# geopolars/geopolars

Measured on AMD Instinct MI355X. Metric: predicate evals/sec (10M pts x 1k polys point-in-polygon), higher is better.
Workload: dtype f64

## Files before the change

### geopolars_amd/_abi.py

```python
from __future__ import annotations

import ctypes as C
import os

HERE = os.path.dirname(os.path.abspath(__file__))
LIB_PATH = os.environ.get("GPK_LIB_PATH") or os.path.join(HERE, "libgeopolars_hip.so")

GPK_OK = 0
GPK_ERR_MISMATCHED_GEOMETRY = 1
GPK_ERR_INVALID_OFFSETS = 2
GPK_ERR_NULL_UNSUPPORTED = 3
GPK_ERR_DEVICE = 4
GPK_ERR_OOM = 5
GPK_ERR_INVALID_ARGUMENT = 6
GPK_ERR_CAPACITY = 7

GEOM_POINT = 0
GEOM_LINESTRING = 1
GEOM_POLYGON = 3
GEOM_MULTIPOINT = 4
GEOM_MULTILINESTRING = 5
GEOM_MULTIPOLYGON = 6
ARROW_WKB, ARROW_INTERLEAVED, ARROW_STRUCT = 0, 1, 2

MEM_HOST = 0
MEM_DEVICE = 1

PRED_INTERSECTS = 0
PRED_CONTAINS = 1
PRED_WITHIN = 2
INDEX_BBOX_GRID = 1
INDEX_PIP = 2
INDEX_PIP_LIGHT = 4
INDEX_PIP_FULL = 8
QUERY_CONTAINED, QUERY_INTERSECTING = 0, 1
PREDICATES = {"intersects": PRED_INTERSECTS, "contains": PRED_CONTAINS, "within": PRED_WITHIN}
LP_INTERIOR, LP_BOUNDARY, LP_EXTERIOR = 1, 2, 4
LP_PRED_INTERSECTS, LP_PRED_WITHIN, LP_PRED_COVERED_BY, LP_PRED_CROSSES, LP_PRED_TOUCHES = 0, 1, 2, 3, 4
TRI_OK, TRI_EMPTY, TRI_FAILED = 0, 1, 2
CLIP_INSIDE, CLIP_OUTSIDE, CLIP_DROP_EMPTY = 0, 1, 1
PCLIP_INTERSECTION, PCLIP_DIFFERENCE = 0, 1
PCLIP_OK, PCLIP_TOUCH, PCLIP_EMPTY, PCLIP_NULL, PCLIP_UNRESOLVED = 0, 1, 2, 3, 4
GEODESIC_AREA_SIGNED = 1
PUNION_UNION = 0
PP_INTERIORS, PP_BOUNDARIES, PP_A_OUTSIDE, PP_B_OUTSIDE = 1, 2, 4, 8
(PP_PRED_INTERSECTS, PP_PRED_WITHIN, PP_PRED_CONTAINS, PP_PRED_TOUCHES, PP_PRED_OVERLAPS, PP_PRED_EQUALS,
 PP_PRED_CONTAINS_PROPERLY) = range(7)
LL_INTERIORS, LL_SHARED_PIECE, LL_INT_BND, LL_BND_INT, LL_BND_BND, LL_A_OUTSIDE, LL_B_OUTSIDE = 1, 2, 4, 8, 16, 32, 64
(LL_PRED_INTERSECTS, LL_PRED_WITHIN, LL_PRED_CONTAINS, LL_PRED_COVERED_BY, LL_PRED_COVERS, LL_PRED_CROSSES, LL_PRED_TOUCHES, LL_PRED_OVERLAPS,
 LL_PRED_EQUALS) = range(9)
PT_INTERIOR, PT_BOUNDARY, PT_EXTERIOR, PT_B_OUTSIDE = 1, 2, 4, 8
GPK_KNN_MAX_K, GPK_KNN_EXCLUDE_SELF = 64, 1
(PT_PRED_INTERSECTS, PT_PRED_WITHIN, PT_PRED_CONTAINS, PT_PRED_COVERED_BY, PT_PRED_COVERS, PT_PRED_CROSSES, PT_PRED_TOUCHES, PT_PRED_OVERLAPS,
 PT_PRED_EQUALS) = range(9)


class GeopolarsHipError(RuntimeError):

    def __init__(self, code: int, message: str):
        super().__init__(f"[gpk status {code}] {message}")
        self.code = code


class MismatchedGeometry(GeopolarsHipError):
    """GeopolarsError::MismatchedGeometry (error.rs:12-16)."""


class GeoArrowDesc(C.Structure):
    _fields_ = [
        ("geom_type", C.c_int32),
        ("mem_space", C.c_int32),
        ("n_geoms", C.c_int64),
        ("n_coords", C.c_int64),
        ("xy", C.c_void_p),
        ("geom_offsets", C.c_void_p),
        ("part_offsets", C.c_void_p),
        ("ring_offsets", C.c_void_p),
        ("n_parts", C.c_int64),
        ("n_rings", C.c_int64),
        ("validity", C.c_void_p),
        ("x", C.c_void_p),
        ("y", C.c_void_p),
    ]


class ArrowSchema(C.Structure):
    """Arrow C Data Interface (what `pyarrow.Array._export_to_c` fills: py-geopolars/src/ffi.rs:12-32)"""


ArrowSchema._fields_ = [
    ("format", C.c_char_p),
    ("name", C.c_char_p),
    ("metadata", C.c_void_p),
    ("flags", C.c_int64),
    ("n_children", C.c_int64),
    ("children", C.POINTER(C.POINTER(ArrowSchema))),
    ("dictionary", C.POINTER(ArrowSchema)),
    ("release", C.CFUNCTYPE(None, C.POINTER(ArrowSchema))),
    ("private_data", C.c_void_p),
]


class ArrowArray(C.Structure):
    pass


ArrowArray._fields_ = [
    ("length", C.c_int64),
    ("null_count", C.c_int64),
    ("offset", C.c_int64),
    ("n_buffers", C.c_int64),
    ("n_children", C.c_int64),
    ("buffers", C.POINTER(C.c_void_p)),
    ("children", C.POINTER(C.POINTER(ArrowArray))),
    ("dictionary", C.POINTER(ArrowArray)),
    ("release", C.CFUNCTYPE(None, C.POINTER(ArrowArray))),
    ("private_data", C.c_void_p),
]


_VP = C.c_void_p
_PROTOS = {
    "gpk_version": (C.c_char_p, []),
    "gpk_last_error": (C.c_int32, [C.c_char_p, C.c_size_t]),
    "gpk_device_count": (C.c_int32, [C.POINTER(C.c_int32)]),
    "gpk_device_info": (C.c_int32, [C.c_char_p, C.c_size_t, C.POINTER(C.c_int32)]),
    "gpk_geoarray_upload": (C.c_int32, [C.POINTER(GeoArrowDesc), _VP, C.POINTER(_VP)]),
    "gpk_geoarray_from_arrow": (C.c_int32, [_VP, _VP, C.c_int32, _VP, C.POINTER(_VP), C.POINTER(C.c_int32)]),
    "gpk_geoarray_to_arrow": (C.c_int32, [_VP, C.c_int32, _VP, _VP, _VP]),
    "gpk_geoarray_free": (C.c_int32, [_VP]),
    "gpk_geoarray_invalidate": (C.c_int32, [_VP]),
    "gpk_geoarray_nbytes": (C.c_int32, [_VP, C.POINTER(C.c_int64)]),
    "gpk_wkb_decode": (C.c_int32, [_VP, _VP, C.c_int64, _VP, C.POINTER(C.c_int64), _VP, _VP, _VP, _VP]),
    "gpk_geoarray_from_wkb": (C.c_int32, [_VP, _VP, C.c_int64, _VP, C.c_int32, _VP, C.POINTER(_VP), C.POINTER(C.c_int32)]),
    "gpk_geoarray_download": (C.c_int32, [_VP, C.POINTER(C.c_int64), _VP, _VP, _VP, _VP, _VP]),
    "gpk_area": (C.c_int32, [_VP, _VP, C.c_int32, _VP]),
    "gpk_signed_area": (C.c_int32, [_VP, _VP, C.c_int32, _VP]),
    "gpk_centroid": (C.c_int32, [_VP, _VP, _VP, C.c_int32, _VP]),
    "gpk_representative_point": (C.c_int32, [_VP, _VP, _VP, _VP, C.c_int32, _VP]),
    "gpk_bounds": (C.c_int32, [_VP, _VP, C.c_int32, _VP]),
    "gpk_euclidean_length": (C.c_int32, [_VP, _VP, C.c_int32, _VP]),
    "gpk_affine_transform": (C.c_int32, [_VP, C.POINTER(C.c_double), _VP, C.c_int32, _VP]),
    "gpk_affine_transform_rows": (C.c_int32, [_VP, _VP, _VP, C.c_int32, _VP]),
    "gpk_affine_about_origin": (C.c_int32, [_VP, C.c_int32, C.c_double, C.c_double, C.c_int32, C.c_double, C.c_double, _VP, C.c_int32, _VP]),
    "gpk_crs_supported": (C.c_int32, [C.c_int32]),
    "gpk_reproject": (C.c_int32, [_VP, C.c_int32, C.c_int32, _VP, C.POINTER(C.c_int64), C.c_int32, _VP]),
    "gpk_envelope": (C.c_int32, [_VP, _VP, _VP, C.c_int32, _VP]),
    "gpk_exterior": (C.c_int32, [_VP, _VP, _VP, C.POINTER(C.c_int64), C.c_int32, _VP]),
    "gpk_explode": (C.c_int32, [_VP, _VP, C.c_int32, _VP, C.POINTER(_VP)]),
    "gpk_geoarray_validity": (C.c_int32, [_VP, _VP, C.POINTER(C.c_int32), _VP]),
    "gpk_geoarray_len": (C.c_int32, [_VP, C.POINTER(C.c_int64)]),
    "gpk_geom_type": (C.c_int32, [_VP, _VP, C.c_int32, _VP]),
    "gpk_is_empty": (C.c_int32, [_VP, _VP, C.c_int32, _VP]),
    "gpk_is_ring": (C.c_int32, [_VP, _VP, C.c_int32, _VP]),
    "gpk_point_xy": (C.c_int32, [_VP, _VP, _VP, C.c_int32, _VP]),
    "gpk_geodesic_length": (C.c_int32, [_VP, C.c_int32, _VP, C.c_int32, _VP]),
    "gpk_geodesic_area": (C.c_int32, [_VP, C.c_uint32, _VP, _VP, C.c_int32, _VP]),
    "gpk_geodesic_inverse": (C.c_int32, [_VP, _VP, _VP, _VP, _VP, _VP, C.c_int32, _VP]),
    "gpk_geodesic_direct": (C.c_int32, [_VP, _VP, C.c_int64, _VP, C.c_int64, _VP, _VP, C.c_int32, _VP]),
    "gpk_simplify": (C.c_int32, [_VP, C.c_double, _VP, _VP, C.POINTER(C.c_int64), C.c_int32, _VP]),
    "gpk_convex_hull": (C.c_int32, [_VP, _VP, _VP, C.c_int32, _VP]),
    "gpk_minimum_rotated_rectangle": (C.c_int32, [_VP, _VP, _VP, C.c_int32, _VP]),
    "gpk_minimum_bounding_circle": (C.c_int32, [_VP, _VP, _VP, _VP, C.c_int32, _VP]),
    "gpk_distance_rowwise": (C.c_int32, [_VP, _VP, _VP, _VP, C.c_int32, _VP]),
    "gpk_rowmap_build": (C.c_int32, [_VP, _VP, C.c_int64, C.c_int32, _VP, C.POINTER(_VP)]),
    "gpk_rowmap_free": (C.c_int32, [_VP]),
    "gpk_rowmap_nbytes": (C.c_int32, [_VP, C.POINTER(C.c_int64)]),
    "gpk_distance_rowmap": (C.c_int32, [_VP, _VP, _VP, _VP, C.c_int32, _VP]),
    "gpk_hausdorff_distance": (C.c_int32, [_VP, _VP, _VP, C.c_int32, _VP, C.c_int32, _VP]),
    "gpk_frechet_distance": (C.c_int32, [_VP, _VP, _VP, C.c_int32, _VP, C.POINTER(C.c_int64), C.c_int32, _VP]),
    "gpk_predicate_rowwise": (C.c_int32, [_VP, _VP, _VP, C.c_int32, _VP, C.c_int32, _VP]),
    "gpk_index_build": (C.c_int32, [_VP, _VP, C.POINTER(_VP)]),
    "gpk_index_build_ex": (C.c_int32, [_VP, C.c_int32, _VP, _VP, C.POINTER(_VP)]),
    "gpk_index_free": (C.c_int32, [_VP]),
    "gpk_index_nbytes": (C.c_int32, [_VP, C.POINTER(C.c_int64)]),
    "gpk_index_describe": (C.c_int32, [_VP, C.POINTER(C.c_int64)]),
    "gpk_index_query_envelope": (C.c_int32, [_VP, _VP, C.c_int64, C.c_int32, _VP, _VP, C.c_int64, C.POINTER(C.c_int64), C.c_int32, _VP]),
    "gpk_spatial_join": (
        C.c_int32,
        [_VP, _VP, _VP, C.c_int32, C.c_uint32, _VP, _VP, C.c_int64, C.POINTER(C.c_int64), C.c_int32, _VP],
    ),
    "gpk_spatial_join_async": (C.c_int32, [_VP, _VP, _VP, C.c_int32, C.c_uint32, _VP, _VP, C.c_int64, _VP, _VP]),
    "gpk_nearest_join": (
        C.c_int32,
        [_VP, _VP, _VP, C.c_double, C.c_uint32, _VP, _VP, _VP, C.c_int64, C.POINTER(C.c_int64), C.c_int32, _VP],
    ),
    "gpk_nearest_join_any": (
        C.c_int32,
        [_VP, _VP, _VP, C.c_double, C.c_uint32, _VP, _VP, _VP, C.c_int64, C.POINTER(C.c_int64), C.c_int32, _VP],
    ),
    "gpk_knn_join": (
        C.c_int32,
        [_VP, _VP, _VP, C.c_int32, C.c_double, C.c_uint32, C.c_uint32, _VP, _VP, _VP, C.c_int64, C.POINTER(C.c_int64), C.c_int32, _VP],
    ),
    "gpk_dwithin_join": (
        C.c_int32,
        [_VP, _VP, _VP, C.c_double, C.c_uint32, _VP, _VP, _VP, C.c_int64, C.POINTER(C.c_int64), C.c_int32, _VP],
    ),
    "gpk_dwithin_rowwise": (C.c_int32, [_VP, _VP, _VP, C.c_double, _VP, C.c_int32, _VP]),
    "gpk_line_polygon_relation": (C.c_int32, [_VP, _VP, _VP, _VP, C.c_int32, _VP]),
    "gpk_line_polygon_join": (
        C.c_int32,
        [_VP, _VP, _VP, C.c_int32, C.c_uint32, _VP, _VP, _VP, C.c_int64, C.POINTER(C.c_int64), C.c_int32, _VP],
    ),
    "gpk_polygon_relation": (C.c_int32, [_VP, _VP, _VP, _VP, C.c_int32, _VP]),
    "gpk_polygon_relation_join": (
        C.c_int32,
        [_VP, _VP, _VP, C.c_int32, C.c_uint32, _VP, _VP, _VP, C.c_int64, C.POINTER(C.c_int64), C.c_int32, _VP],
    ),
    "gpk_intersection_measure": (C.c_int32, [_VP, _VP, _VP, _VP, C.c_int32, _VP]),
    "gpk_line_clip": (C.c_int32, [_VP, _VP, _VP, _VP, C.c_int64, C.c_int32, C.c_int32, C.c_int32, _VP, C.c_int32, _VP, C.POINTER(_VP)]),
    "gpk_polygon_clip": (C.c_int32, [_VP, _VP, _VP, _VP, C.c_int64, C.c_int32, C.c_int32, C.c_int32, _VP, C.c_int32, _VP, C.c_int32, _VP, C.POINTER(_VP)]),
    "gpk_polygon_union": (C.c_int32, [_VP, _VP, _VP, _VP, C.c_int64, C.c_int32, C.c_int32, C.c_int32, _VP, C.c_int32, _VP, C.c_int32, _VP, C.POINTER(_VP)]),
    "gpk_union_all_pairs": (C.c_int32, [_VP, _VP, C.c_int64, C.c_int64, _VP, _VP, _VP, _VP, C.POINTER(C.c_int64), _VP]),
    "gpk_intersection_measure_join": (
        C.c_int32,
        [_VP, _VP, _VP, C.c_double, C.c_uint32, _VP, _VP, _VP, C.c_int64, C.POINTER(C.c_int64), C.c_int32, _VP],
    ),
    "gpk_line_relation": (C.c_int32, [_VP, _VP, _VP, _VP, C.c_int32, _VP]),
    "gpk_line_relation_join": (
        C.c_int32,
        [_VP, _VP, _VP, C.c_int32, C.c_uint32, _VP, _VP, _VP, C.c_int64, C.POINTER(C.c_int64), C.c_int32, _VP],
    ),
    "gpk_point_relation": (C.c_int32, [_VP, _VP, _VP, _VP, C.c_int32, _VP]),
    "gpk_point_relation_join": (
        C.c_int32,
        [_VP, _VP, _VP, C.c_int32, C.c_uint32, _VP, _VP, _VP, C.c_int64, C.POINTER(C.c_int64), C.c_int32, _VP],
    ),
    "gpk_validity": (C.c_int32, [_VP, _VP, _VP, C.c_int32, _VP]),
    "gpk_is_simple": (C.c_int32, [_VP, _VP, C.c_int32, _VP]),
    "gpk_triangulate": (C.c_int32, [_VP, _VP, C.c_int64, _VP, _VP, C.POINTER(C.c_int64), C.c_int32, _VP]),
    "gpk_closest_point_rowwise": (C.c_int32, [_VP, _VP, _VP, _VP, _VP, C.c_int32, _VP]),
    "gpk_line_locate_point": (C.c_int32, [_VP, _VP, _VP, C.c_int32, _VP, C.c_int32, _VP]),
    "gpk_line_interpolate_point": (C.c_int32, [_VP, _VP, C.c_int64, C.c_int32, _VP, _VP, C.c_int32, _VP]),
    "gpk_wkb_encode": (C.c_int32, [_VP, _VP, _VP, C.c_int64, C.POINTER(C.c_int64)]),
    "gpk_geoarray_to_wkb": (C.c_int32, [_VP, _VP, _VP, C.c_int64, C.POINTER(C.c_int64), C.c_int32, _VP]),
    "gpk_join_indices": (C.c_int32, [_VP, _VP, C.c_int64, C.c_int64, C.c_uint32, C.c_int32, _VP, _VP, C.c_int64, C.POINTER(C.c_int64), C.c_int32, _VP]),
    "gpk_take_fixed": (C.c_int32, [_VP, C.c_int32, _VP, C.c_int64, _VP, C.c_int64, _VP, _VP, C.c_int32, _VP]),
    "gpk_take_binary": (C.c_int32, [_VP, _VP, _VP, C.c_int64, _VP, C.c_int64, _VP, _VP, C.c_int64, C.POINTER(C.c_int64), _VP, C.c_int32, _VP]),
    "gpk_geoarray_take": (C.c_int32, [_VP, _VP, C.c_int64, C.c_int32, _VP, C.POINTER(_VP)]),
    "gpk_geoarray_filter": (C.c_int32, [_VP, _VP, C.c_int32, C.c_int32, _VP, C.POINTER(_VP), C.POINTER(C.c_int64)]),
    "gpk_segmentize": (C.c_int32, [_VP, C.c_double, _VP, C.c_int32, _VP, C.POINTER(_VP)]),
    "gpk_remove_repeated_points": (C.c_int32, [_VP, C.c_double, _VP, C.POINTER(_VP)]),
    "gpk_reverse": (C.c_int32, [_VP, _VP, C.POINTER(_VP)]),
    "gpk_orient_polygons": (C.c_int32, [_VP, C.c_int32, _VP, C.POINTER(_VP)]),
    "gpk_comm_unique_id":(C.c_int32, [C.POINTER(C.c_uint8)]),
    "gpk_comm_init": (C.c_int32, [C.c_int32, C.c_int32, C.POINTER(C.c_uint8), C.POINTER(_VP)]),
    "gpk_comm_free": (C.c_int32, [_VP]),
    "gpk_comm_mock_world": (C.c_int32, [C.c_int32, C.POINTER(_VP)]),
    "gpk_comm_init_mock": (C.c_int32, [C.c_int32, _VP, C.POINTER(_VP)]),
    "gpk_comm_mock_world_free": (C.c_int32, [_VP]),
    "gpk_comm_info": (C.c_int32, [_VP, C.POINTER(C.c_int32), C.POINTER(C.c_int32)]),
    "gpk_allgatherv_geoarray": (C.c_int32, [_VP, _VP, _VP, C.POINTER(_VP), C.POINTER(C.c_int64), C.POINTER(C.c_int64)]),
    "gpk_geoarray_concat": (C.c_int32, [C.POINTER(_VP), C.c_int32, _VP, C.POINTER(_VP), C.POINTER(C.c_int64), C.POINTER(C.c_int64)]),
    "gpk_allgatherv_rows_f64": (C.c_int32, [_VP, _VP, C.c_int64, C.c_int32, _VP, C.c_int64, C.POINTER(C.c_int64), C.POINTER(C.c_int64), _VP]),
    "gpk_device_cache_release": (C.c_int32, []),
    "gpk_join_stats_enable": (C.c_int32, [C.c_int32]),
    "gpk_join_stats": (C.c_int32, [C.POINTER(C.c_int64), C.c_int32]),
    "gpk_profile_enable": (C.c_int32, [C.c_int32]),
    "gpk_profile_filter": (C.c_int32, [C.c_char_p]),
    "gpk_profile_reset": (C.c_int32, []),
    "gpk_profile_query": (C.c_int32, [C.c_char_p, C.POINTER(C.c_double), C.POINTER(C.c_int64)]),
}
EXPORTED_SYMBOLS = tuple(_PROTOS)

_lib = None


def lib() -> C.CDLL:
    global _lib
    if _lib is not None:
        return _lib
    if not os.path.exists(LIB_PATH):
        raise GeopolarsHipError(
            GPK_ERR_DEVICE,
            f"{LIB_PATH} is missing: build it with `python -m geopolars_amd.build` "
            "(hipcc, gfx950).  geopolars_amd has no CPU fallback.",
        )
    try:
        import torch
    except Exception:
        pass
    handle = C.CDLL(LIB_PATH, mode=C.RTLD_GLOBAL)
    for name, (res, args) in _PROTOS.items():
        fn = getattr(handle, name)
        fn.restype = res
        fn.argtypes = args
    _lib = handle
    return _lib


def last_error() -> str:
    buf = C.create_string_buffer(512)
    lib().gpk_last_error(buf, 512)
    return buf.value.decode("utf-8", "replace")


def check(status: int) -> None:
    if status == GPK_OK:
        return
    msg = last_error()
    if status == GPK_ERR_MISMATCHED_GEOMETRY:
        raise MismatchedGeometry(status, msg)
    raise GeopolarsHipError(status, msg)


def device_count() -> int:
    n = C.c_int32(0)
    rc = lib().gpk_device_count(C.byref(n))
    return int(n.value) if rc == GPK_OK else 0


def device_info() -> tuple[str, int]:
    buf = C.create_string_buffer(256)
    cus = C.c_int32(0)
    check(lib().gpk_device_info(buf, 256, C.byref(cus)))
    return buf.value.decode(), int(cus.value)
```

### geopolars_amd/csrc/gpk_gridindex.hip

```cpp
#include <atomic>
#include <chrono>
#include <cmath>
#include <cstdlib>

#include "gpk_device.h"
#include "gpk_index.h"
#include "gpk_scan.h"

namespace gpk {

__global__ __launch_bounds__(256) void extent_partial_kernel(const double4* __restrict__ bbox, int64_t n, double4* __restrict__ part) {
    __shared__ double red[4][4];
    double mnx = INFINITY, mny = INFINITY, mxx = -INFINITY, mxy = -INFINITY;
    for (int64_t i = (int64_t)blockIdx.x * 256 + threadIdx.x; i < n; i += (int64_t)gridDim.x * 256) {
        const double4 b = bbox[i];
        if (b.x == b.x) {
            mnx = fmin(mnx, b.x);
            mny = fmin(mny, b.y);
            mxx = fmax(mxx, b.z);
            mxy = fmax(mxy, b.w);
        }
    }
    mnx = dev::wave_min(mnx);
    mny = dev::wave_min(mny);
    mxx = dev::wave_max(mxx);
    mxy = dev::wave_max(mxy);
    const int lane = threadIdx.x & 63, wave = threadIdx.x >> 6;
    if (lane == 0) {
        red[0][wave] = mnx;
        red[1][wave] = mny;
        red[2][wave] = mxx;
        red[3][wave] = mxy;
    }
    __syncthreads();
    if (threadIdx.x == 0) {
        for (int w = 1; w < 4; ++w) {
            mnx = fmin(mnx, red[0][w]);
            mny = fmin(mny, red[1][w]);
            mxx = fmax(mxx, red[2][w]);
            mxy = fmax(mxy, red[3][w]);
        }
        part[blockIdx.x] = mnx <= mxx ? make_double4(mnx, mny, mxx, mxy) : make_double4(NAN, NAN, NAN, NAN);
    }
}
__global__ __launch_bounds__(1024) void extent_kernel(const double4* __restrict__ bbox, int64_t n,
                                                      int gx, int gy, GridParams* __restrict__ out) {
    __shared__ double red[4][16];
    double mnx = INFINITY, mny = INFINITY, mxx = -INFINITY, mxy = -INFINITY;
    for (int64_t i = threadIdx.x; i < n; i += 1024) {
        const double4 b = bbox[i];
        if (b.x == b.x) {
            mnx = fmin(mnx, b.x);
            mny = fmin(mny, b.y);
            mxx = fmax(mxx, b.z);
            mxy = fmax(mxy, b.w);
        }
    }
    mnx = dev::wave_min(mnx);
    mny = dev::wave_min(mny);
    mxx = dev::wave_max(mxx);
    mxy = dev::wave_max(mxy);
    const int lane = threadIdx.x & 63, wave = threadIdx.x >> 6;
    if (lane == 0) {
        red[0][wave] = mnx;
        red[1][wave] = mny;
        red[2][wave] = mxx;
        red[3][wave] = mxy;
    }
    __syncthreads();
    if (threadIdx.x == 0) {
        for (int w = 1; w < 16; ++w) {
            mnx = fmin(mnx, red[0][w]);
            mny = fmin(mny, red[1][w]);
            mxx = fmax(mxx, red[2][w]);
            mxy = fmax(mxy, red[3][w]);
        }
        GridParams g;
        const bool any = mnx <= mxx;
        g.x0 = any ? mnx : 0.0;
        g.y0 = any ? mny : 0.0;
        const double w = any ? mxx - mnx : 0.0, h = any ? mxy - mny : 0.0;
        g.inv_w = w > 0.0 ? (double)gx / w : 0.0;
        g.inv_h = h > 0.0 ? (double)gy / h : 0.0;
        g.gx = gx;
        g.gy = gy;
        *out = g;
    }
}

template <bool FILL>
__global__ void grid_register_kernel(const double4* __restrict__ bbox, int64_t n,
                                     const GridParams* __restrict__ gp, int32_t* __restrict__ cell_cnt,
                                     int32_t* __restrict__ items) {
    const int64_t j = (int64_t)blockIdx.x * blockDim.x + threadIdx.x;
    if (j >= n) return;
    const double4 b = bbox[j];
    if (!(b.x == b.x)) return;
    const GridParams g = *gp;
    const int cx0 = dev::cell_of(b.x, g.x0, g.inv_w, g.gx), cx1 = dev::cell_of(b.z, g.x0, g.inv_w, g.gx);
    const int cy0 = dev::cell_of(b.y, g.y0, g.inv_h, g.gy), cy1 = dev::cell_of(b.w, g.y0, g.inv_h, g.gy);
    for (int cy = cy0; cy <= cy1; ++cy)
        for (int cx = cx0; cx <= cx1; ++cx) {
            const int c = cy * g.gx + cx;
            const int slot = atomicAdd(&cell_cnt[c], 1);
            if (FILL) items[slot] = (int32_t)j;
        }
}

__global__ void cell_sort_kernel(const int32_t* __restrict__ cell_off, int64_t n_cells, int32_t* __restrict__ items) {
    const int64_t c = (int64_t)blockIdx.x * blockDim.x + threadIdx.x;
    if (c >= n_cells) return;
    const int b = cell_off[c], e = cell_off[c + 1];
    for (int i = b + 1; i < e; ++i) {
        const int32_t key = items[i];
        int k = i - 1;
        while (k >= b && items[k] > key) {
            items[k + 1] = items[k];
            --k;
        }
        items[k + 1] = key;
    }
}

static inline dim3 grid_for(int64_t n, int block) {
    int64_t b = (n + block - 1) / block;
    return dim3((unsigned)(b > 0 ? b : 1));
}

}

using namespace gpk;

extern "C" {

int32_t gpk_index_free(gpk_index* idx) {
    if (!idx) return GPK_OK;
    (void)sync_device(idx->device);
    for (int i = 0; i < 24; ++i)
        if (idx->owned[i]) cached_free(idx->owned[i]);
    delete idx;
    return GPK_OK;
}

int32_t gpk_index_describe(const gpk_index* idx, int64_t out[8]) {
    if (!idx || !out) return fail(GPK_ERR_INVALID_ARGUMENT, "NULL argument");
    for (int i = 0; i < 8; ++i) out[i] = 0;
    out[0] = idx->pip.R;
    out[1] = idx->pip_lean;
    out[2] = idx->pip.chain_xy != nullptr;
    out[3] = idx->pip.route != nullptr;
    out[4] = idx->pip_list_heavy;
    out[5] = idx->route_own;
    out[6] = idx->route_single;
    return GPK_OK;
}

int32_t gpk_index_nbytes(const gpk_index* idx, int64_t* out_bytes) {
    if (!idx || !out_bytes) return fail(GPK_ERR_INVALID_ARGUMENT, "NULL argument");
    *out_bytes = idx->nbytes;
    return GPK_OK;
}

int32_t gpk_index_build(const gpk_geoarray* a, void* stream, gpk_index** out) {
    return gpk_index_build_ex(a, GPK_INDEX_BBOX_GRID | GPK_INDEX_PIP, nullptr, stream, out);
}

int32_t gpk_index_build_ex(const gpk_geoarray* a, int32_t parts, const double* bbox4_dev, void* stream, gpk_index** out) {
    if (!a || !out) return fail(GPK_ERR_INVALID_ARGUMENT, "NULL argument");
    *out = nullptr;
    GPK_TRY(require_device());
    hipStream_t s = (hipStream_t)stream;
    const int64_t n = a->d.n_geoms;

    gpk_index* ix = new gpk_index;
    memset(ix, 0, sizeof *ix);
    ix->device = a->device;
    ix->n_geoms = n;
    ix->geom_type = a->d.type;
    ix->n_coords = a->d.n_coords;
    ix->n_rings = a->d.n_rings;
    {
        static std::atomic<uint64_t> next_serial{1};
        ix->serial = next_serial.fetch_add(1);
    }

    int gdim = (int)ceil(2.0 * sqrt((double)(n > 0 ? n : 1)));
    if (gdim < 1) gdim = 1;
    if (gdim > 2048) gdim = 2048;
    const int64_t n_cells = (int64_t)gdim * gdim;

    auto cleanup = [&](int32_t rc) {
        gpk_index_free(ix);
        return rc;
    };
#define IX_HIP(expr)                                                                              \
    do {                                                                                          \
        hipError_t _e = (expr);                                                                   \
        if (_e != hipSuccess)                                                                     \
            return cleanup(fail(_e == hipErrorOutOfMemory ? GPK_ERR_OOM : GPK_ERR_DEVICE,         \
                                "%s failed: %s", #expr, hipGetErrorString(_e)));                  \
    } while (0)
#define IX_TRY(expr)                             \
    do {                                         \
        int32_t _rc = (expr);                    \
        if (_rc != GPK_OK) return cleanup(_rc);  \
    } while (0)

    const bool dbg_time = getenv("GPK_DEBUG_INDEX") != nullptr;
    auto t_last = std::chrono::steady_clock::now();
    auto stamp = [&](const char* what) {
        if (!dbg_time) return;
        (void)hipStreamSynchronize(s);
        const auto now = std::chrono::steady_clock::now();
        fprintf(stderr, "[gpk] index build: %-28s %8.3f ms\n", what, std::chrono::duration<double, std::milli>(now - t_last).count());
        t_last = now;
    };
    double4* bbox = nullptr;
    GridParams* grid = nullptr;
    int32_t* cell_off = nullptr;
    IX_HIP(cached_malloc((void**)&bbox, sizeof(double4) * (size_t)(n > 0 ? n : 1)));
    ix->owned[0] = bbox;
    IX_HIP(cached_malloc((void**)&grid, sizeof(GridParams)));
    ix->owned[1] = grid;
    IX_HIP(cached_malloc((void**)&cell_off, sizeof(int32_t) * (size_t)(n_cells + 1)));
    ix->owned[2] = cell_off;

    if (bbox4_dev)
        IX_HIP(hipMemcpyAsync(bbox, bbox4_dev, sizeof(double4) * (size_t)n, hipMemcpyDeviceToDevice, s));
    else
        IX_TRY(gpk_bounds(a, (double*)bbox, GPK_MEM_DEVICE, stream));

    stamp("boxes (gpk_bounds)");
    const int64_t n_blocks = (n_cells + 255) / 256;
    const int64_t ext_blocks = n > 65536 ? 1024 : 0;
    Scratch sc(workspace());
    int32_t *cell_cnt, *cursor;
    unsigned long long* btot;
    double4* ext_part;
    sc.add_n((size_t)(n_cells + 1), cell_cnt, cursor);
    sc.add(btot, (size_t)(n_blocks + 1));
    sc.add(ext_part, 1024);
    IX_TRY(sc.commit());
    if (ext_blocks) {
        GPK_LAUNCH_OR(cleanup, "gpk_index_extent_partial", extent_partial_kernel, dim3((unsigned)ext_blocks), dim3(256), 0, s, bbox, n, ext_part);
        GPK_LAUNCH_OR(cleanup, "gpk_index_extent", extent_kernel, dim3(1), dim3(1024), 0, s, (const double4*)ext_part, ext_blocks, gdim, gdim, grid);
    } else {
        GPK_LAUNCH_OR(cleanup, "gpk_index_extent", extent_kernel, dim3(1), dim3(1024), 0, s, bbox, n, gdim, gdim, grid);
    }

    stamp("extent");
    IX_HIP(hipMemsetAsync(cell_cnt, 0, sizeof(int32_t) * (size_t)(n_cells + 1), s));
    if (n > 0)
        GPK_LAUNCH_OR(cleanup, "gpk_index_count", grid_register_kernel<false>, grid_for(n, 256), dim3(256), 0, s, bbox, n, grid, cell_cnt, (int32_t*)nullptr);
    IX_TRY(exclusive_scan_i32(cell_cnt, n_cells, cell_off, cursor, btot, s));
    unsigned long long total = 0;
    IX_HIP(d2h_small(&total, btot + n_blocks, sizeof total, s));
    IX_HIP(d2h_small(&ix->host_grid, grid, sizeof(GridParams), s));
    IX_HIP(sync_small(s));
    if (total > (unsigned long long)INT32_MAX)
        return cleanup(fail(GPK_ERR_INVALID_OFFSETS, "spatial index directory overflows i32 (%llu entries)", total));
    int32_t* items = nullptr;
    IX_HIP(cached_malloc((void**)&items, sizeof(int32_t) * (size_t)(total > 0 ? total : 1)));
    ix->owned[3] = items;
    if (n > 0) {
        GPK_LAUNCH_OR(cleanup, "gpk_index_fill", grid_register_kernel<true>, grid_for(n, 256), dim3(256), 0, s, bbox, n, grid, cursor, items);
        GPK_LAUNCH_OR(cleanup, "gpk_index_sort", cell_sort_kernel, grid_for(n_cells, 256), dim3(256), 0, s, cell_off, n_cells, items);
    }
    IX_HIP(hipStreamSynchronize(s));
    stamp("directory");
#undef IX_HIP
#undef IX_TRY

    ix->v.bbox = bbox;
    ix->v.grid = grid;
    ix->v.cell_off = cell_off;
    ix->v.items = items;
    ix->v.gx = gdim;
    ix->v.gy = gdim;
    ix->nbytes = (int64_t)(sizeof(double4) * (size_t)n + sizeof(GridParams) + sizeof(int32_t) * (size_t)(n_cells + 1) +
                           sizeof(int32_t) * (size_t)total);
    if (parts & GPK_INDEX_PIP) {
        const int32_t rc = build_pip_index(a, ix, s, (parts & GPK_INDEX_PIP_LIGHT) ? 0 : ((parts & GPK_INDEX_PIP_FULL) ? 2 : 1));
        if (rc != GPK_OK) {
            gpk_index_free(ix);
            return rc;
        }
    }
    *out = ix;
    return GPK_OK;
}

}
```

### geopolars_amd/csrc/gpk_index.h

```cpp
#pragma once

#include "gpk_common.h"
#include "gpk_route.h"

namespace gpk {

struct GridParams {
    double x0, y0, inv_w, inv_h;
    int32_t gx, gy;
};

struct IndexView {
    const double4* bbox;
    const GridParams* grid;
    const int32_t* cell_off;
    const int32_t* items;
    int32_t gx, gy;
};

struct PartInfo {
    int32_t slab_base, row0 , nrows, n_rings;
};
constexpr int PIP_SUB = 8;
constexpr int PIP_SLAB_MUL = 2;
constexpr int PIP_FINE_LOG2 = 6;
__host__ __device__ inline int slab_row0_of(int32_t packed) { return packed & 0xFFFFFF; }
__host__ __device__ inline int slab_shift_of(int32_t packed) { return packed >> 24; }
constexpr uint32_t SUB_INDIRECT = 1u << 30;
struct SubCell {
    uint32_t part_flags;
    uint32_t e0, e1, e2;
    uint32_t labels[4];
};
struct SubCell2 {
    SubCell a;
    uint32_t b_part_flags;
    uint32_t b_e0, b_e1, b_e2;
    uint32_t pad[4];
};
constexpr uint32_t SUB2_BIT = 1u << 29;
constexpr int CHAIN_MAX = 12;
constexpr uint32_t HCHAIN_COUNT_MASK = 0xFu;
constexpr int HCHAIN_BASE_SHIFT = 4;
constexpr int HCHAIN_START_SHIFT = 8;
struct HalfCell {
    uint32_t lw[2];
    uint32_t part_flags;
    uint32_t aux_base;
};
static_assert(sizeof(HalfCell) * 2 == sizeof(SubCell), "two half-cell records overlay one SubCell");
static_assert(CHAIN_MAX <= (int)HCHAIN_COUNT_MASK, "the edge count of a chain is a 4-bit field");
struct PipView {
    int32_t R;
    double rx0, ry0, fw, fh, inv_fw, inv_fh;
    const uint32_t* cell;
    const uint32_t* list;
    const SubCell* sub;
    const SubCell2* sub2;
    const double2* chain_xy;
    const RouteWord* route;
    const SubCell* lrec;
    const uint32_t* part_geom;
    const PartInfo* part_info;
    const float4* part_box;
    const int32_t* ring_row0;
    const int32_t* ring_slab_base;
    const int32_t* slab_off;
    const double4* slab_edges;
    const int32_t* slab_vidx;
    const double2* slab_xy;
};
constexpr uint32_t CELL_TAG_EMPTY = 0u, CELL_TAG_SINGLE = 1u, CELL_TAG_LIST = 2u, CELL_TAG_SUB = 3u;

namespace dev {
__device__ __forceinline__ int cell_of(double v, double v0, double inv, int g) {
    return (int)fmin(fmax((v - v0) * inv, 0.0), (double)(g - 1));
}
}

}

struct gpk_index {
    gpk::IndexView v;
    gpk::PipView pip;
    gpk::GridParams host_grid;
    int device;
    int64_t n_geoms, n_coords, n_rings;
    int32_t geom_type;
    void* owned[24];
    int64_t nbytes;
    int32_t pip_lean;
    uint64_t serial;
    int32_t pip_list_heavy;
    int32_t route_own, route_single;
};

namespace gpk {
int32_t build_pip_index(const gpk_geoarray* a, gpk_index* ix, hipStream_t s, int list_records_mode = 1);
int32_t ring_bboxes(const gpk_geoarray* a, double4* out_dev, hipStream_t s);
int32_t affine_rows_impl(const gpk_geoarray* a, const double* matrices, int32_t mat_space, double* out_xy, int32_t out_space, hipStream_t s);
}
```

### geopolars_amd/csrc/gpk_pipindex.hip

```cpp
#include <cstdio>
#include <cstdlib>
#include <cstring>

#include <rocprim/rocprim.hpp>

#include <chrono>

#include "gpk_device.h"
#include "gpk_index.h"
#include "gpk_pip.h"
#include "gpk_scan.h"

namespace gpk {

struct FineGrid {
    int R;
    double rx0, ry0, fw, fh, inv_fw, inv_fh, pad_x, pad_y;
};
__device__ __forceinline__ int fcol(const FineGrid& f, double x) { return dev::cell_of(x, f.rx0, f.inv_fw, f.R); }
__device__ __forceinline__ int frow(const FineGrid& f, double y) { return dev::cell_of(y, f.ry0, f.inv_fh, f.R); }

__global__ void part_geom_kernel(DevGeo a, uint32_t* __restrict__ part_geom) {
    const int64_t g = (int64_t)blockIdx.x * blockDim.x + threadIdx.x;
    if (g >= a.n_geoms) return;
    for (int p = a.geom_off[g]; p < a.geom_off[g + 1]; ++p) part_geom[p] = (uint32_t)g;
}
__global__ void ring_part_kernel(DevGeo a, int64_t n_parts, int32_t* __restrict__ ring_part) {
    const int64_t p = (int64_t)blockIdx.x * blockDim.x + threadIdx.x;
    if (p >= n_parts) return;
    int r0, r1;
    dev::part_rings(a, (int)p, r0, r1);
    for (int r = r0; r < r1; ++r) ring_part[r] = (int32_t)p;
}

__global__ void part_info_kernel(DevGeo a, int64_t n_parts, const int32_t* __restrict__ row0, const int32_t* __restrict__ slab_base,
                                 PartInfo* __restrict__ info) {
    const int64_t p = (int64_t)blockIdx.x * blockDim.x + threadIdx.x;
    if (p >= n_parts) return;
    int r0, r1;
    dev::part_rings(a, (int)p, r0, r1);
    PartInfo pi{0, 0, 0, r1 - r0};
    if (r1 > r0) {
        pi.slab_base = slab_base[r0];
        pi.row0 = row0[r0];
        pi.nrows = slab_base[r0 + 1] - slab_base[r0];
    }
    info[p] = pi;
}

__global__ void part_box_kernel(DevGeo a, int64_t n_parts, const double4* __restrict__ ring_bbox, float4* __restrict__ box) {
    const int64_t p = (int64_t)blockIdx.x * blockDim.x + threadIdx.x;
    if (p >= n_parts) return;
    int r0, r1;
    dev::part_rings(a, (int)p, r0, r1);
    const float nan = __builtin_nanf("");
    float4 b = make_float4(nan, nan, nan, nan);
    if (r1 > r0) {
        const double4 d = ring_bbox[r0];
        auto down = [](double v) {
            float f = (float)v;
            return (double)f > v ? nextafterf(f, -INFINITY) : f;
        };
        auto up = [](double v) {
            float f = (float)v;
            return (double)f < v ? nextafterf(f, INFINITY) : f;
        };
        b = make_float4(down(d.x), down(d.y), up(d.z), up(d.w));
    }
    box[p] = b;
}

constexpr int SLAB_TARGET = 12;
__global__ void ring_rows_kernel(const double4* __restrict__ ring_bbox, int64_t n_rings, const int32_t* __restrict__ ring_off, FineGrid f,
                                 int max_shift, int32_t* __restrict__ row0, int32_t* __restrict__ nrows, int32_t* __restrict__ n_refined) {
    const int64_t r = (int64_t)blockIdx.x * blockDim.x + threadIdx.x;
    if (r >= n_rings) return;
    const double4 b = ring_bbox[r];
    if (!(b.x == b.x) || !(b.y == b.y) || !(b.w == b.w)) {
        row0[r] = 0;
        nrows[r] = 0;
        return;
    }
    const int f0 = frow(f, b.y), f1 = frow(f, b.w);
    const int64_t n_edges = (int64_t)ring_off[r + 1] - ring_off[r] - 1;
    const int64_t base_rows = (f1 >> PIP_FINE_LOG2) - (f0 >> PIP_FINE_LOG2) + 1;
    int sh = 0;
    while (sh < max_shift && n_edges > (int64_t)SLAB_TARGET * (base_rows << sh)) ++sh;
    const int j0 = f0 >> (PIP_FINE_LOG2 - sh), j1 = f1 >> (PIP_FINE_LOG2 - sh);
    if (sh > 0 && (int)(threadIdx.x & 63) == __ffsll((long long)__ballot(sh > 0)) - 1) *n_refined = 1;
    row0[r] = j0 | (sh << 24);
    nrows[r] = j1 - j0 + 1;
}

__device__ __forceinline__ bool edge_at(const DevGeo& a, const int32_t* __restrict__ coord_ring, int i, int& r, double2& s, double2& e) {
    r = coord_ring[i];
    const int c0 = a.ring_off[r], c1 = a.ring_off[r + 1];
    if (i >= c1) return false;
    s = a.xy[i];
    if (i + 1 < c1) {
        e = a.xy[i + 1];
        return true;
    }
    if (c1 - c0 == 1) {
        e = s;
        return true;
    }
    return false;
}

__global__ void ring_start_kernel(const int32_t* __restrict__ ring_off, int64_t n_rings, int64_t n_coords, int32_t* __restrict__ flag) {
    const int64_t r = (int64_t)blockIdx.x * blockDim.x + threadIdx.x;
    if (r < 1 || r >= n_rings) return;
    const int32_t o = ring_off[r];
    if (o >= 0 && (int64_t)o < n_coords) atomicAdd(&flag[o], 1);
}

template <bool FILL>
__global__ void slab_register_kernel(DevGeo a, const int32_t* __restrict__ coord_ring, FineGrid f, const int32_t* __restrict__ row0,
                                     const int32_t* __restrict__ slab_base, int32_t* __restrict__ cnt_or_cursor,
                                     double4* __restrict__ edges, int32_t* __restrict__ vidx = nullptr) {
    const int64_t i = (int64_t)blockIdx.x * blockDim.x + threadIdx.x;
    const int lane = (int)(threadIdx.x & 63);
    int r = 0;
    double2 s = make_double2(0, 0), e = s;
    bool live = i < a.n_coords && edge_at(a, coord_ring, (int)i, r, s, e);
    if (live) live = slab_base[r + 1] != slab_base[r];
    const double ylo = s.y < e.y ? s.y : e.y, yhi = s.y > e.y ? s.y : e.y;
    if (!(ylo == ylo) || !(yhi == yhi)) live = false;
    int j0 = 0, j1 = -1, sl0 = -1 - lane;
    int rr = 0;
    if (live) {
        rr = row0[r];
        const int down = PIP_FINE_LOG2 - slab_shift_of(rr);
        j0 = frow(f, ylo) >> down;
        j1 = frow(f, yhi) >> down;
        sl0 = slab_base[r] + (j0 - slab_row0_of(rr));
    }
    const int prev = __shfl_up(sl0, 1, 64);
    const unsigned long long heads = __ballot(lane == 0 || sl0 != prev);
    const int head = 63 - __clzll((long long)(heads & (~0ull >> (63 - lane))));
    const unsigned long long above = lane == 63 ? 0ull : heads >> (lane + 1);
    const int run = above ? __ffsll((long long)above) : 64 - lane;
    int base = 0;
    if (live && head == lane) base = atomicAdd(&cnt_or_cursor[sl0], run);
    base = __shfl(base, head, 64);
    if (!live) return;
    const bool degenerate = FILL && a.ring_off[r + 1] - a.ring_off[r] == 1;
    auto put = [&](int slot) {
        if (edges) edges[slot] = make_double4(s.x, s.y, e.x, e.y);
        if (vidx) vidx[slot] = degenerate ? ~(int32_t)i : (int32_t)i;
    };
    if (FILL) put(base + (lane - head));
    for (int j = j0 + 1; j <= j1; ++j) {
        const int sl = slab_base[r] + (j - slab_row0_of(rr));
        const int slot = atomicAdd(&cnt_or_cursor[sl], 1);
        if (FILL) put(slot);
    }
}

__device__ __forceinline__ bool line_clear_of_rect(double sx, double sy, double ex, double ey, double xl, double yl, double xh, double yh) {
    const bool x_up = sy > ey, y_up = ex > sx;
    const double max_x = x_up ? xh : xl, min_x = x_up ? xl : xh, max_y = y_up ? yh : yl, min_y = y_up ? yl : yh;
    return dev::orient2d(sx, sy, ex, ey, min_x, min_y) > 0 || dev::orient2d(sx, sy, ex, ey, max_x, max_y) < 0;
}
template <typename F>
__device__ __forceinline__ void for_each_touched_cell(const FineGrid& g, double2 s, double2 e, F&& f) {
    const double xlo = s.x < e.x ? s.x : e.x, xhi = s.x > e.x ? s.x : e.x;
    const double ylo = s.y < e.y ? s.y : e.y, yhi = s.y > e.y ? s.y : e.y;
    if (!(xlo == xlo) || !(xhi == xhi) || !(ylo == ylo) || !(yhi == yhi)) return;
    const int i0 = fcol(g, xlo - g.pad_x), i1 = fcol(g, xhi + g.pad_x);
    const int j0 = frow(g, ylo - g.pad_y), j1 = frow(g, yhi + g.pad_y);
    if (i0 == i1 && j0 == j1) {
        f(i0, j0);
        return;
    }
    for (int j = j0; j <= j1; ++j)
        for (int i = i0; i <= i1; ++i) {
            if (i == 0 || j == 0 || i == g.R - 1 || j == g.R - 1) {
                f(i, j);
                continue;
            }
            const double xl = g.rx0 + (double)i * g.fw - g.pad_x, xh = g.rx0 + (double)(i + 1) * g.fw + g.pad_x;
            const double yl = g.ry0 + (double)j * g.fh - g.pad_y, yh = g.ry0 + (double)(j + 1) * g.fh + g.pad_y;
            if (!line_clear_of_rect(s.x, s.y, e.x, e.y, xl, yl, xh, yh)) f(i, j);
        }
}

template <bool FILL>
__global__ void mark_kernel(DevGeo a, const int32_t* __restrict__ coord_ring, FineGrid g, const int32_t* __restrict__ ring_part,
                            int32_t* __restrict__ cnt_or_off, unsigned long long* __restrict__ keys) {
    const int64_t i = (int64_t)blockIdx.x * blockDim.x + threadIdx.x;
    const int lane = (int)(threadIdx.x & 63);
    int r = 0;
    double2 s = make_double2(0, 0), e = s;
    const bool live = i < a.n_coords && edge_at(a, coord_ring, (int)i, r, s, e);
    const unsigned long long none = ~0ull;
    unsigned long long first = none;
    const int64_t o0 = FILL && i < a.n_coords ? (int64_t)cnt_or_off[i] : 0;
    int64_t n = 0;
    if (live) {
        const unsigned long long part = (unsigned long long)ring_part[r];
        for_each_touched_cell(g, s, e, [&](int ci, int cj) {
            const unsigned long long key = ((unsigned long long)(cj * g.R + ci) << 32) | part;
            if (n == 0) {
                first = key;
            } else if (FILL) {
                if (n == 1) keys[o0] = first;
                keys[o0 + n] = key;
            }
            ++n;
        });
    }
    const unsigned long long single = n == 1 ? first : none;
    const unsigned long long prev = __shfl_up(single, 1, 64);
    const bool repeat = lane > 0 && single != none && single == prev;
    if (i >= a.n_coords) return;
    if (!FILL) {
        cnt_or_off[i] = repeat ? 0 : (int32_t)(n < 0x7FFFFFFF ? n : 0x7FFFFFFF);
    } else if (n == 1 && !repeat) {
        keys[o0] = first;
    }
}

__global__ void unique_flags_kernel(const unsigned long long* __restrict__ sorted, int64_t n, int32_t* __restrict__ flag) {
    const int64_t i = (int64_t)blockIdx.x * blockDim.x + threadIdx.x;
    if (i >= n) return;
    flag[i] = (i == 0 || sorted[i] != sorted[i - 1]) ? 1 : 0;
}
__global__ void unique_compact_kernel(const unsigned long long* __restrict__ sorted, int64_t n, const int32_t* __restrict__ pos,
                                      unsigned long long* __restrict__ out, int32_t* __restrict__ cell_marks) {
    const int64_t i = (int64_t)blockIdx.x * blockDim.x + threadIdx.x;
    if (i >= n) return;
    const unsigned long long key = sorted[i];
    if (i == 0 || key != sorted[i - 1]) {
        out[pos[i]] = key;
        atomicAdd(&cell_marks[key >> 32], 1);
    }
}

constexpr int CELL_SCRATCH = 8;
template <bool FILL>
__global__ void cell_build_kernel(DevGeo a, IndexView ix, PipView pv, FineGrid g,
                                  const unsigned long long* __restrict__ marks, const int32_t* __restrict__ mark_start,
                                  int32_t* __restrict__ need, const int32_t* __restrict__ list_off,
                                  uint32_t* __restrict__ cell, uint32_t* __restrict__ list, uint32_t* __restrict__ scratch,
                                  const double4* __restrict__ ring_bbox) {
    const int64_t c = (int64_t)blockIdx.x * blockDim.x + threadIdx.x;
    const int64_t n_cells = (int64_t)g.R * g.R;
    if (c >= n_cells) return;
    if (FILL && need[c] == 0) return;
    if (FILL && scratch && need[c] - 1 <= CELL_SCRATCH) {
        const int m = need[c] - 1;
        uint32_t* out = list + list_off[c];
        out[0] = (uint32_t)m;
        for (int k = 0; k < m; ++k) out[1 + k] = scratch[(int64_t)k * n_cells + c];
        cell[c] = (CELL_TAG_LIST << 30) | (uint32_t)list_off[c];
        return;
    }
    const int ci = (int)(c % g.R), cj = (int)(c / g.R);
    const double cx = g.rx0 + ((double)ci + 0.5) * g.fw, cy = g.ry0 + ((double)cj + 0.5) * g.fh;
    const bool border = ci == 0 || cj == 0 || ci == g.R - 1 || cj == g.R - 1;
    const bool centre_ok = !border && fcol(g, cx) == ci && frow(g, cy) == cj;
    int64_t m = mark_start[c];
    const int64_t m_end = mark_start[c + 1];

    int n = 0;
    uint32_t first_entry = 0;
    uint32_t* out = nullptr;
    if (FILL && need[c] > 0) {
        out = list + list_off[c];
        out[0] = (uint32_t)(need[c] - 1);
        ++out;
    }
    auto emit = [&](uint32_t part, uint32_t boundary) {
        const uint32_t e = (part << 1) | boundary;
        if (n == 0) first_entry = e;
        if (out) out[n] = e;
        if (!FILL && scratch && n < CELL_SCRATCH) scratch[(int64_t)n * n_cells + c] = e;
        ++n;
    };
    auto flush_marks_below = [&](unsigned long long part_limit) {
        while (m < m_end && (marks[m] & 0xFFFFFFFFull) < part_limit) {
            emit((uint32_t)(marks[m] & 0xFFFFFFFFull), 1u);
            ++m;
        }
    };

    const GridParams cg = *ix.grid;
    const int gx = dev::cell_of(cx, cg.x0, cg.inv_w, cg.gx), gy = dev::cell_of(cy, cg.y0, cg.inv_h, cg.gy);
    const int gc = gy * cg.gx + gx;
    for (int k = ix.cell_off[gc]; k < ix.cell_off[gc + 1]; ++k) {
        const int j = ix.items[k];
        const double4 bb = ix.bbox[j];
        if (!(cx >= bb.x && cx <= bb.z && cy >= bb.y && cy <= bb.w)) continue;
        if (!dev::valid_row(a.validity, j)) continue;
        int p0, p1;
        dev::geom_parts(a, j, p0, p1);
        for (int p = p0; p < p1; ++p) {
            flush_marks_below((unsigned long long)p);
            if (m < m_end && (marks[m] & 0xFFFFFFFFull) == (unsigned long long)p) {
                emit((uint32_t)p, 1u);
                ++m;
                continue;
            }
            if (p1 - p0 > 1) {
                int r0, r1;
                dev::part_rings(a, p, r0, r1);
                if (r1 <= r0) continue;
                const double4 rb = ring_bbox[r0];
                if (!(cx >= rb.x && cx <= rb.z && cy >= rb.y && cy <= rb.w)) continue;
            }
            const int pos = pip::part_pos_single(pv, a, p, cx, cy);
            if (pos == dev::POS_OUTSIDE) continue;
            emit((uint32_t)p, (centre_ok && pos == dev::POS_INSIDE) ? 0u : 1u);
        }
    }
    flush_marks_below(~0ull);

    if (!FILL) {
        need[c] = n >= 2 ? n + 1 : 0;
        if (n <= 1) cell[c] = n == 1 ? ((CELL_TAG_SINGLE << 30) | first_entry) : 0u;
        return;
    }
    cell[c] = (CELL_TAG_LIST << 30) | (uint32_t)list_off[c];
}

__device__ __forceinline__ int64_t sub_slot(int64_t c, int route_logR) { return route_logR ? (int64_t)route_order((uint32_t)c, route_logR) : c; }
__global__ void sub_flag_kernel(const uint32_t* __restrict__ cell, const uint32_t* __restrict__ list, int64_t n_cells, int route_logR,
                                int32_t* __restrict__ flag, int32_t* __restrict__ flag2) {
    const int64_t c = (int64_t)blockIdx.x * blockDim.x + threadIdx.x;
    if (c >= n_cells) return;
    const uint32_t w = cell[c];
    const uint32_t tag = w >> 30;
    flag[sub_slot(c, route_logR)] = (tag == CELL_TAG_SINGLE && (w & 1u)) ? 1 : 0;
    int f2 = 0;
    if (tag == CELL_TAG_LIST) {
        const uint32_t off = w & 0x3FFFFFFFu;
        if (list[off] == 2u) f2 = (list[off + 1] & list[off + 2] & 1u) ? 1 : 0;
    }
    flag2[c] = f2;
}

__device__ __forceinline__ void record_slabs(const PipView& pv, int p, int cj, uint32_t& flags, uint32_t& e0, uint32_t& e1, uint32_t& e2) {
    const PartInfo pi = pv.part_info[p];
    e0 = e1 = e2 = 0;
    flags = (uint32_t)p | (pi.n_rings > 1 ? 0x80000000u : 0u);
    if (slab_shift_of(pi.row0) != 0) {
        flags |= SUB_INDIRECT;
        return;
    }
    const int j0 = PIP_SLAB_MUL * cj - slab_row0_of(pi.row0), j1 = j0 + 1;
    const bool lo_ok = j0 >= 0 && j0 < pi.nrows, hi_ok = j1 >= 0 && j1 < pi.nrows;
    if (lo_ok) {
        e0 = (uint32_t)pv.slab_off[pi.slab_base + j0];
        e1 = (uint32_t)pv.slab_off[pi.slab_base + j0 + 1];
        e2 = e1;
    }
    if (hi_ok) {
        if (!lo_ok) e0 = e1 = (uint32_t)pv.slab_off[pi.slab_base + j1];
        e2 = (uint32_t)pv.slab_off[pi.slab_base + j1 + 1];
    }
}
__global__ void sub_head_kernel(PipView pv, FineGrid g, const int32_t* __restrict__ work_cell, const uint32_t* __restrict__ work_part,
                                int64_t n_work, SubCell* __restrict__ sub) {
    const int64_t i = (int64_t)blockIdx.x * blockDim.x + threadIdx.x;
    if (i >= n_work) return;
    uint32_t flags, e0, e1, e2;
    record_slabs(pv, (int)work_part[i], (int)(work_cell[i] / g.R), flags, e0, e1, e2);
    *reinterpret_cast<uint4*>(&sub[i].part_flags) = make_uint4(flags, e0, e1, e2);
}

constexpr int SUB_EDGE_CAP = 48;
template <int NP, bool WORK = false, int MODE = 0>
__global__ __launch_bounds__(256) __attribute__((amdgpu_waves_per_eu(MODE == 1 ? 8 : 5))) void sub_build_kernel(DevGeo a, PipView pv, FineGrid g, const int32_t* __restrict__ flag,
                                                        const int32_t* __restrict__ pos, int64_t n_cells, const uint32_t* __restrict__ cell,
                                                        const uint32_t* __restrict__ list, SubCell* __restrict__ sub,
                                                        SubCell2* __restrict__ sub2, const int32_t* __restrict__ work_cell = nullptr,
                                                        const uint32_t* __restrict__ work_part = nullptr, int64_t n_work = 0) {
    static_assert(!WORK || NP == 1, "work items carry one part");
    constexpr int S = PIP_SUB, SS = PIP_SUB * PIP_SUB;
    const int64_t t = (int64_t)blockIdx.x * blockDim.x + threadIdx.x;
    const int64_t item = t / SS;
    const int k = (int)(t % SS);
    if (WORK ? item >= n_work : (item >= n_cells || !flag[item])) return;
    const int64_t c = WORK ? (int64_t)work_cell[item] : item;
    const uint32_t w = cell[c];
    int part[2] = {0, 0};
    bool crosses[2] = {true, true};
    if (WORK) {
        part[0] = (int)work_part[item];
    } else if (NP == 1) {
        part[0] = (int)((w & 0x3FFFFFFFu) >> 1);
    } else {
        const uint32_t off = w & 0x3FFFFFFFu;
        const uint32_t ea = list[off + 1], eb = list[off + 2];
        part[0] = (int)(ea >> 1);
        part[1] = (int)(eb >> 1);
    }
    const int ci = (int)(c % g.R), cj = (int)(c / g.R);
    const int si = S * ci + (k % S), sj = S * cj + (k / S);
    const double fw2 = g.fw / S, fh2 = g.fh / S, px2 = g.pad_x / S, py2 = g.pad_y / S;
    const double xl = g.rx0 + (double)si * fw2 - px2, xh = g.rx0 + (double)(si + 1) * fw2 + px2;
    const double yl = g.ry0 + (double)sj * fh2 - py2, yh = g.ry0 + (double)(sj + 1) * fh2 + py2;
    __shared__ double4 s_edges[256 / 64][SUB_EDGE_CAP];
    __shared__ double4 s_edges_all[WORK ? 256 / 64 : 1][WORK ? 64 : 1];
    const int wave = threadIdx.x >> 6, lane64 = threadIdx.x & 63;
    const double cxl = g.rx0 + (double)(S * ci) * fw2 - px2, cxh = g.rx0 + (double)(S * ci + S) * fw2 + px2;
    const double cyl = g.ry0 + (double)(S * cj) * fh2 - py2, cyh = g.ry0 + (double)(S * cj + S) * fh2 + py2;
    auto edge_touches = [&](const double4 ed) {
        if (fmax(ed.x, ed.z) < xl || fmin(ed.x, ed.z) > xh || fmax(ed.y, ed.w) < yl || fmin(ed.y, ed.w) > yh) return false;
        return !line_clear_of_rect(ed.x, ed.y, ed.z, ed.w, xl, yl, xh, yh);
    };
    auto store_labels = [&](SubCell* rec, uint32_t label) {
        const unsigned long long lo = __ballot((label & 1u) != 0), hi = __ballot((label & 2u) != 0);
        if (k < 4) {
            auto spread16 = [](uint32_t x) {
                x = (x | (x << 8)) & 0x00FF00FFu;
                x = (x | (x << 4)) & 0x0F0F0F0Fu;
                x = (x | (x << 2)) & 0x33333333u;
                x = (x | (x << 1)) & 0x55555555u;
                return x;
            };
            rec->labels[k] = spread16((uint32_t)(lo >> (16 * k)) & 0xFFFFu) | (spread16((uint32_t)(hi >> (16 * k)) & 0xFFFFu) << 1);
        }
    };
    if (WORK) {
        const uint4 head = *reinterpret_cast<const uint4*>(&sub[item].part_flags);
        const uint32_t n_all = head.w - head.y;
        const bool fast = !(head.x & (SUB_INDIRECT | 0x80000000u)) && n_all <= 64u;
        if (MODE == 1 && !fast) return;
        if (MODE == 2 && fast) return;
        if (MODE != 2 && fast) {
            if ((uint32_t)lane64 < n_all) s_edges_all[wave][lane64] = pip::slab_edge(pv, (int)(head.y + (uint32_t)lane64));
            __builtin_amdgcn_fence(__ATOMIC_RELEASE, "wavefront");
            __builtin_amdgcn_wave_barrier();
            __builtin_amdgcn_fence(__ATOMIC_ACQUIRE, "wavefront");
            bool touched = false;
            for (uint32_t e = 0; e < n_all && !touched; ++e) touched = edge_touches(s_edges_all[wave][e]);
            uint32_t label = 2u;
            if (!touched) {
                const double cx = g.rx0 + ((double)si + 0.5) * fw2, cy = g.ry0 + ((double)sj + 0.5) * fh2;
                const bool ok = dev::cell_of(cx, g.rx0, g.inv_fw * S, g.R * S) == si && dev::cell_of(cy, g.ry0, g.inv_fh * S, g.R * S) == sj;
                if (ok) {
                    const uint32_t mid = head.z - head.y;
                    const uint32_t a0 = (k / S) >= S / 2 ? mid : 0u, a1 = (k / S) >= S / 2 ? n_all : mid;
                    int wn = 0;
                    bool on = false;
                    for (uint32_t e = a0; e < a1; ++e) {
                        const double4 ed = s_edges_all[wave][e];
                        on |= dev::ring_edge(ed.x, ed.y, ed.z, ed.w, cx, cy, wn);
                    }
                    label = on ? 2u : (wn != 0 ? 1u : 0u);
                }
            }
            store_labels(sub + item, label);
            return;
        }
        if (MODE == 1) return;
    }
    __shared__ int s_span_e0[256 / 64][64], s_span_at[256 / 64][64];
    int n_list = 0;
    bool touched = false;
    auto wave_min = [&](double v) {
#pragma unroll
        for (int o = 1; o < 64; o <<= 1) v = fmin(v, __shfl_xor(v, o, 64));
        return v;
    };
    auto drain = [&](bool boxed = false) {
        __builtin_amdgcn_fence(__ATOMIC_RELEASE, "wavefront");
        __builtin_amdgcn_wave_barrier();
        __builtin_amdgcn_fence(__ATOMIC_ACQUIRE, "wavefront");
        bool skip = false;
        if (boxed) {
            const double inf = __builtin_inf();
            double4 b = make_double4(inf, inf, inf, inf);
            bool odd = false;
            if (lane64 < n_list) {
                const double4 ed = s_edges[wave][lane64];
                b = make_double4(fmin(ed.x, ed.z), fmin(ed.y, ed.w), -fmax(ed.x, ed.z), -fmax(ed.y, ed.w));
                odd = !(ed.x == ed.x) || !(ed.y == ed.y) || !(ed.z == ed.z) || !(ed.w == ed.w);
            }
            if (!__ballot(odd)) {
                const double bx0 = wave_min(b.x), by0 = wave_min(b.y), bx1 = -wave_min(b.z), by1 = -wave_min(b.w);
                skip = bx1 < xl || bx0 > xh || by1 < yl || by0 > yh;
            }
        }
        for (int e = 0; e < n_list && !touched && !skip; ++e) touched = edge_touches(s_edges[wave][e]);
        __builtin_amdgcn_fence(__ATOMIC_RELEASE, "wavefront");
        __builtin_amdgcn_wave_barrier();
        __builtin_amdgcn_fence(__ATOMIC_ACQUIRE, "wavefront");
        n_list = 0;
    };
    for (int q = 0; q < NP; ++q) {
        if (!crosses[q]) continue;
        int r0, r1;
        dev::part_rings(a, part[q], r0, r1);
        for (int rb = r0; rb < r1; rb += 64) {
            const int n_r = r1 - rb < 64 ? r1 - rb : 64;
            int e0 = 0, cnt = 0;
            if (lane64 < n_r) {
                int a0, a1;
                if (pip::slab_span_of_raster_row(pv, rb + lane64, cj, a0, a1)) {
                    e0 = a0;
                    cnt = a1 - a0;
                }
            }
            const int incl = dev::wave_inclusive_scan(cnt);
            const int total = __shfl(incl, 63, 64);
            s_span_e0[wave][lane64] = e0;
            s_span_at[wave][lane64] = incl - cnt;
            __builtin_amdgcn_fence(__ATOMIC_RELEASE, "wavefront");
            __builtin_amdgcn_wave_barrier();
            __builtin_amdgcn_fence(__ATOMIC_ACQUIRE, "wavefront");
            for (int base = 0; base < total; base += 64) {
                const int t = base + lane64;
                bool keep = false;
                double4 ed = make_double4(0, 0, 0, 0);
                if (t < total) {
                    int lo = 0, hi = n_r;
                    while (hi - lo > 1) {
                        const int mid = (lo + hi) >> 1;
                        if (s_span_at[wave][mid] <= t)
                            lo = mid;
                        else
                            hi = mid;
                    }
                    ed = pip::slab_edge(pv, s_span_e0[wave][lo] + (t - s_span_at[wave][lo]));
                    keep = !(fmax(ed.x, ed.z) < cxl || fmin(ed.x, ed.z) > cxh || fmax(ed.y, ed.w) < cyl || fmin(ed.y, ed.w) > cyh);
                }
                unsigned long long pending = __ballot(keep);
                while (pending) {
                    const int rank = __popcll(pending & ((1ull << lane64) - 1ull));
                    const bool put = keep && rank < SUB_EDGE_CAP - n_list;
                    if (put) {
                        s_edges[wave][n_list + rank] = ed;
                        keep = false;
                    }
                    const unsigned long long taken = __ballot(put);
                    n_list += __popcll(taken);
                    pending &= ~taken;
                    if (pending) drain(true);
                }
            }
            __builtin_amdgcn_fence(__ATOMIC_RELEASE, "wavefront");
            __builtin_amdgcn_wave_barrier();
            __builtin_amdgcn_fence(__ATOMIC_ACQUIRE, "wavefront");
        }
    }
    drain();
    const uint32_t test_label = NP == 2 ? 3u : 2u;
    uint32_t label = test_label;
    if (!touched) {
        const double cx = g.rx0 + ((double)si + 0.5) * fw2, cy = g.ry0 + ((double)sj + 0.5) * fh2;
        const bool ok = dev::cell_of(cx, g.rx0, g.inv_fw * S, g.R * S) == si && dev::cell_of(cy, g.ry0, g.inv_fh * S, g.R * S) == sj;
        if (ok) {
            if (NP == 1) {
                const int p = pip::part_pos_single(pv, a, part[0], cx, cy);
                label = p == dev::POS_INSIDE ? 1u : (p == dev::POS_OUTSIDE ? 0u : 2u);
            } else {
                const int pa = pip::part_pos_single(pv, a, part[0], cx, cy), pb = pip::part_pos_single(pv, a, part[1], cx, cy);
                if (pa == dev::POS_BOUNDARY || pb == dev::POS_BOUNDARY)
                    label = 3u;
                else if (pa == dev::POS_INSIDE && pb == dev::POS_INSIDE)
                    label = 3u;
                else
                    label = pa == dev::POS_INSIDE ? 1u : (pb == dev::POS_INSIDE ? 2u : 0u);
            }
        }
    }
    auto slabs_of = [&](int p, uint32_t& flags, uint32_t& e0, uint32_t& e1, uint32_t& e2) { record_slabs(pv, p, cj, flags, e0, e1, e2); };
    SubCell* rec = WORK ? sub + item : (NP == 1 ? sub + pos[c] : &sub2[pos[c]].a);
    if (k == 0) {
        slabs_of(part[0], rec->part_flags, rec->e0, rec->e1, rec->e2);
        if (NP == 2) {
            SubCell2* r2 = sub2 + pos[c];
            slabs_of(part[1], r2->b_part_flags, r2->b_e0, r2->b_e1, r2->b_e2);
        }
    }
    store_labels(rec, label);
}
__global__ void sub_commit_kernel(const int32_t* __restrict__ flag, const int32_t* __restrict__ pos, const int32_t* __restrict__ flag2,
                                  const int32_t* __restrict__ pos2, int64_t n_cells, int route_logR, uint32_t* __restrict__ cell) {
    const int64_t c = (int64_t)blockIdx.x * blockDim.x + threadIdx.x;
    if (c >= n_cells) return;
    const int64_t o = sub_slot(c, route_logR);
    if (flag[o])
        cell[c] = (CELL_TAG_SUB << 30) | (uint32_t)pos[o];
    else if (flag2 && flag2[c])
        cell[c] = (CELL_TAG_SUB << 30) | SUB2_BIT | (uint32_t)pos2[c];
}

__global__ void lrec_count_kernel(const uint32_t* __restrict__ cell, const uint32_t* __restrict__ list, int64_t n_cells,
                                  int32_t* __restrict__ cnt) {
    const int64_t c = (int64_t)blockIdx.x * blockDim.x + threadIdx.x;
    if (c >= n_cells) return;
    const uint32_t w = cell[c];
    int n = 0;
    if ((w >> 30) == CELL_TAG_LIST) {
        const uint32_t off = w & 0x3FFFFFFFu, m = list[off];
        for (uint32_t t = 0; t < m; ++t) n += (int)(list[off + 1 + t] & 1u);
    }
    cnt[c] = n;
}
__device__ __forceinline__ int test_labels_of(uint32_t w) { return __popc((w >> 1) & ~w & 0x55555555u); }
__global__ void chain_xy_kernel(DevGeo a, double2* __restrict__ ext) {
    const int64_t k = (int64_t)blockIdx.x * blockDim.x + threadIdx.x;
    const int64_t n_ext = a.n_coords + a.n_rings * CHAIN_MAX;
    if (k >= n_ext) return;
    int lo = 0, hi = (int)a.n_rings - 1;
    while (lo < hi) {
        const int mid = (lo + hi + 1) >> 1;
        if ((int64_t)a.ring_off[mid] + (int64_t)mid * CHAIN_MAX <= k)
            lo = mid;
        else
            hi = mid - 1;
    }
    const int c0 = a.ring_off[lo], n = a.ring_off[lo + 1] - c0;
    const int j = (int)(k - ((int64_t)c0 + (int64_t)lo * CHAIN_MAX));
    const int ne = n - 1;
    ext[k] = n <= 0 ? make_double2(0.0, 0.0) : (ne >= 1 ? a.xy[c0 + j % ne] : a.xy[c0]);
}
__global__ __launch_bounds__(256) void half_chain_kernel(DevGeo a, PipView pv, FineGrid g, const int32_t* __restrict__ work_cell,
                                                         const uint32_t* __restrict__ work_part, int64_t n_work,
                                                         const int32_t* __restrict__ slab_vidx, const SubCell* __restrict__ sub,
                                                         uint32_t* __restrict__ hword) {
    constexpr int S = PIP_SUB;
    static_assert(S == 8 && PIP_SLAB_MUL == 2, "a record is two halves of four sub-cell rows, one base slab row each");
    const int64_t t = (int64_t)blockIdx.x * blockDim.x + threadIdx.x;
    const int64_t item = t >> 1;
    const int half = (int)(t & 1);
    if (item >= n_work) return;
    const int64_t c = work_cell[item];
    const int part = (int)work_part[item];
    const uint32_t lw0 = sub[item].labels[2 * half], lw1 = sub[item].labels[2 * half + 1];
    uint32_t word = 0u;
    int r0, r1;
    dev::part_rings(a, part, r0, r1);
    if (test_labels_of(lw0) + test_labels_of(lw1) > 0 && r1 - r0 == 1) {
        const int ci = (int)(c % g.R), cj = (int)(c / g.R);
        const double fw2 = g.fw / S, fh2 = g.fh / S, px2 = g.pad_x / S, py2 = g.pad_y / S;
        const int sj0 = S * cj + (S / 2) * half;
        const double xl = g.rx0 + (double)(S * ci) * fw2 - px2, xh = g.rx0 + (double)(S * ci + S) * fw2 + px2;
        const double yl = g.ry0 + (double)sj0 * fh2 - py2, yh = g.ry0 + (double)(sj0 + S / 2) * fh2 + py2;
        const int c0 = a.ring_off[r0], ne = a.ring_off[r0 + 1] - c0 - 1;
        bool closed = false;
        if (ne >= 1) {
            const double2 f = a.xy[c0], l = a.xy[c0 + ne];
            closed = f.x == l.x && f.y == l.y;
        }
        const double cy = g.ry0 + ((double)sj0 + 0.25 * S) * fh2;
        const int row_c = pip::row_of(pv, cy);
        const int step = 1 << PIP_FINE_LOG2;
        int e0 = 0, e1 = 0;
        bool have = false;
        int lo = 0, len = 0;
        bool ok = closed;
        int n_touched = 0;
        int touched[CHAIN_MAX + 1];
        for (int dr = -1; dr <= 1 && ok; ++dr) {
            if (!pip::slab_range(pv, r0, row_c + dr * step, e0, e1)) continue;
            have = true;
            for (int e = e0; e < e1 && ok; ++e) {
                const double4 ed = pip::slab_edge(pv, e);
                if (fmax(ed.x, ed.z) < xl || fmin(ed.x, ed.z) > xh || fmax(ed.y, ed.w) < yl || fmin(ed.y, ed.w) > yh) continue;
                if (line_clear_of_rect(ed.x, ed.y, ed.z, ed.w, xl, yl, xh, yh)) continue;
                const int ei = pip::slab_vertex(slab_vidx[e]) - c0;
                bool seen = false;
                for (int q = 0; q < n_touched; ++q) seen = seen || touched[q] == ei;
                if (seen) continue;
                if (n_touched >= CHAIN_MAX) {
                    ok = false;
                    break;
                }
                touched[n_touched++] = ei;
            }
        }
        ok = ok && have && n_touched > 0;
        if (ok) {
            int best_gap = -1, best_next = 0;
            for (int p = 0; p < n_touched; ++p) {
                const int ea = touched[p];
                int nd = ne, nb = ea;
                for (int q = 0; q < n_touched; ++q) {
                    int dd = touched[q] - ea;
                    if (dd < 0) dd += ne;
                    if (dd > 0 && dd < nd) {
                        nd = dd;
                        nb = touched[q];
                    }
                }
                if (nd > best_gap) {
                    best_gap = nd;
                    best_next = nb;
                }
            }
            lo = best_next;
            len = ne - best_gap + 1;
            ok = len >= 1 && len <= CHAIN_MAX;
        }
        while (ok && len < ne) {
            int hv = lo + len;
            if (hv >= ne) hv -= ne;
            const double y = a.xy[c0 + hv].y;
            if (!(y >= yl && y <= yh)) break;
            ++len;
            ok = len <= CHAIN_MAX;
        }
        while (ok && len < ne) {
            const double y = a.xy[c0 + lo].y;
            if (!(y >= yl && y <= yh)) break;
            lo = lo == 0 ? ne - 1 : lo - 1;
            ++len;
            ok = len <= CHAIN_MAX;
        }
        if (ok) {
            const double cx = g.rx0 + ((double)(S * ci) + 0.5 * S) * fw2;
            int wn = 0;
            bool on = false;
            if (pip::slab_range(pv, r0, row_c, e0, e1)) {
                for (int e = e0; e < e1; ++e) {
                    int dd = pip::slab_vertex(slab_vidx[e]) - c0 - lo;
                    if (dd < 0) dd += ne;
                    if (dd < len) continue;
                    const double4 ed = pip::slab_edge(pv, e);
                    on |= dev::ring_edge(ed.x, ed.y, ed.z, ed.w, cx, cy, wn);
                }
            }
            const int64_t start = (int64_t)c0 + (int64_t)r0 * CHAIN_MAX + lo;
            if (!on && wn >= -8 && wn <= 7 && start < ((int64_t)1 << (32 - HCHAIN_START_SHIFT)))
                word = (uint32_t)len | ((uint32_t)(wn & 15) << HCHAIN_BASE_SHIFT) | ((uint32_t)start << HCHAIN_START_SHIFT);
        }
    }
    hword[2 * item + half] = word;
}
__global__ void half_chain_commit_kernel(SubCell* __restrict__ sub, int64_t n_sub, const uint32_t* __restrict__ hword) {
    const int64_t i = (int64_t)blockIdx.x * blockDim.x + threadIdx.x;
    if (i >= n_sub) return;
    const SubCell rc = sub[i];
    HalfCell* h = reinterpret_cast<HalfCell*>(sub + i);
    h[0] = HalfCell{{rc.labels[0], rc.labels[1]}, rc.part_flags & ~SUB_INDIRECT, hword[2 * i]};
    h[1] = HalfCell{{rc.labels[2], rc.labels[3]}, rc.part_flags & ~SUB_INDIRECT, hword[2 * i + 1]};
}
__global__ void route_build_kernel(const uint32_t* __restrict__ cell, int64_t n_words, int logR, RouteWord* __restrict__ route,
                                   uint32_t* __restrict__ counters) {
    const int64_t w = (int64_t)blockIdx.x * blockDim.x + threadIdx.x;
    if (w >= n_words) return;
    const uint32_t bx = (uint32_t)w & ((1u << (logR - 3)) - 1u), by = (uint32_t)w >> (logR - 3);
    uint32_t cw[32];
#pragma unroll
    for (int i = 0; i < 32; ++i) cw[i] = cell[((int64_t)((by << 2) | (uint32_t)(i >> 3)) << logR) + ((bx << 3) | (uint32_t)(i & 7))];
    uint32_t rec = 0u, other = 0u, inside = 0u, rec0 = 0u;
#pragma unroll
    for (int i = 31; i >= 0; --i) {
        const uint32_t tag = cw[i] >> 30, payload = cw[i] & 0x3FFFFFFFu;
        if (tag == CELL_TAG_SUB && !(payload & SUB2_BIT)) {
            rec |= 1u << i;
            rec0 = payload;
        } else if ((cw[i] & 0xC0000001u) == (CELL_TAG_SINGLE << 30)) {
            inside |= 1u << i;
        } else if (cw[i] != 0u) {
            other |= 1u << i;
        }
    }
    uint32_t owner = ROUTE_NO_OWNER, own = 0u;
    if (inside) {
        uint32_t left = inside;
#pragma unroll
        for (int i = 0; i < 32; ++i) {
            if (!((left >> i) & 1u)) continue;
            const uint32_t p = (cw[i] >> 1) & 0x1FFFFFFFu;
            uint32_t m = 0u;
#pragma unroll
            for (int j = i; j < 32; ++j) m |= (uint32_t)(((cw[j] >> 1) & 0x1FFFFFFFu) == p) << j;
            m &= left;
            left &= ~m;
            if (p < ROUTE_OWNER_MAX && (__popc(m) > __popc(own) || (__popc(m) == __popc(own) && p < owner))) {
                owner = p;
                own = m;
            }
        }
    }
    route[w] = RouteWord{rec | own, other | inside, route_pack(rec0, owner), 0u};
    if (inside) {
        if (own) atomicAdd(&counters[0], (uint32_t)__popc(own));
        atomicAdd(&counters[1], (uint32_t)__popc(inside));
    }
}

__global__ void sub_work_kernel(const uint32_t* __restrict__ cell, const int32_t* __restrict__ flag, const int32_t* __restrict__ pos,
                                int64_t n_cells, int route_logR, int32_t* __restrict__ work_cell, uint32_t* __restrict__ work_part) {
    const int64_t c = (int64_t)blockIdx.x * blockDim.x + threadIdx.x;
    if (c >= n_cells) return;
    const int64_t o = sub_slot(c, route_logR);
    if (!flag[o]) return;
    work_cell[pos[o]] = (int32_t)c;
    work_part[pos[o]] = (cell[c] & 0x3FFFFFFFu) >> 1;
}
__global__ void lrec_assign_kernel(const uint32_t* __restrict__ cell, uint32_t* __restrict__ list, int64_t n_cells,
                                   const int32_t* __restrict__ pos, int32_t* __restrict__ work_cell, uint32_t* __restrict__ work_part) {
    const int64_t c = (int64_t)blockIdx.x * blockDim.x + threadIdx.x;
    if (c >= n_cells) return;
    const uint32_t w = cell[c];
    if ((w >> 30) != CELL_TAG_LIST) return;
    const uint32_t off = w & 0x3FFFFFFFu, m = list[off];
    int32_t o = pos[c];
    for (uint32_t t = 0; t < m; ++t) {
        const uint32_t e = list[off + 1 + t];
        if (!(e & 1u)) continue;
        work_cell[o] = (int32_t)c;
        work_part[o] = e >> 1;
        list[off + 1 + t] = ((uint32_t)o << 1) | 1u;
        ++o;
    }
}

}

using namespace gpk;

namespace {
struct Temps {
    void* p[48] = {nullptr};
    int n = 0;
    double malloc_ms = 0.0;
    size_t malloc_bytes = 0;
    template <typename T>
    int32_t alloc(T** out, size_t count) {
        const size_t bytes = sizeof(T) * (count ? count : 1);
        void* q = gpk::ScratchEstimate::try_carve(gpk::workspace_aux(1), bytes);
        if (!q) {
            const auto t0 = std::chrono::steady_clock::now();
            hipError_t e = cached_malloc(&q, bytes);
            malloc_ms += std::chrono::duration<double, std::milli>(std::chrono::steady_clock::now() - t0).count();
            malloc_bytes += bytes;
            if (e != hipSuccess) return fail(GPK_ERR_OOM, "index build: device_malloc(%zu) failed: %s", bytes, hipGetErrorString(e));
            if (n < 48) p[n++] = q;
        }
        *out = (T*)q;
        return GPK_OK;
    }
    ~Temps() {
        const auto t0 = std::chrono::steady_clock::now();
        if (n) (void)hipDeviceSynchronize();
        for (int i = 0; i < n; ++i) cached_free(p[i]);
        if (getenv("GPK_DEBUG_INDEX"))
            fprintf(stderr, "[gpk] index build: %d temporaries beyond the arena (%.2f GB): hipMalloc %.3f ms, hipFree %.3f ms\n", n, (double)malloc_bytes / 1e9,
                    malloc_ms, std::chrono::duration<double, std::milli>(std::chrono::steady_clock::now() - t0).count());
    }
};
inline dim3 blocks_for(int64_t n) { return dim3((unsigned)((n + 255) / 256 > 0 ? (n + 255) / 256 : 1)); }
}

namespace gpk {

int32_t build_pip_index(const gpk_geoarray* a, gpk_index* ix, hipStream_t s, int list_records_mode) {
    memset(&ix->pip, 0, sizeof ix->pip);
    const DevGeo& d = a->d;
    if (!is_polygonal(d.type) || d.n_geoms == 0 || d.n_coords == 0 || d.n_rings == 0) return GPK_OK;
    const GridParams hg = ix->host_grid;
    const double w = hg.inv_w > 0.0 ? (double)hg.gx / hg.inv_w : 0.0, h = hg.inv_h > 0.0 ? (double)hg.gy / hg.inv_h : 0.0;
    if (!(w > 0.0) || !(h > 0.0) || !std::isfinite(w) || !std::isfinite(h)) return GPK_OK;

    int R = 64;
    while (R < 2048 && (double)R < 2.0 * sqrt((double)d.n_coords)) R <<= 1;
    bool many_parts = false;
    if (R == 2048 && d.n_parts > (int64_t)R * R / 2) {
        R = 4096;
        many_parts = true;
    }
    const bool list_records = list_records_mode == 2 || (list_records_mode == 1 && !many_parts);
    FineGrid g;
    g.R = R;
    g.fw = w / (double)(R - 3);
    g.fh = h / (double)(R - 3);
    g.rx0 = hg.x0 - 1.5 * g.fw;
    g.ry0 = hg.y0 - 1.5 * g.fh;
    g.inv_fw = 1.0 / g.fw;
    g.inv_fh = 1.0 / g.fh;
    g.pad_x = g.fw * (1.0 / 65536.0);
    g.pad_y = g.fh * (1.0 / 65536.0);
    const double max_abs = fmax(fmax(fabs(hg.x0), fabs(hg.x0 + w)), fmax(fabs(hg.y0), fabs(hg.y0 + h)));
    const double ulp64 = max_abs * 1.4210854715202004e-14;
    if (!(g.pad_x > ulp64) || !(g.pad_y > ulp64)) return GPK_OK;

    const int64_t n_rings = d.n_rings, n_parts = d.n_parts, n_cells = (int64_t)R * R;
    {
        size_t est = (size_t)n_rings * 64 + (size_t)n_cells * 96 + (size_t)d.n_coords * 168 + (8u << 20);
        if (est > (size_t(256) << 20)) est = size_t(256) << 20;
        ScratchEstimate::reserve(workspace_aux(1), est);
    }
    Temps t;
    const bool dbg_time = getenv("GPK_DEBUG_INDEX") != nullptr;
    auto t_last = std::chrono::steady_clock::now();
    auto stamp = [&](const char* what) {
        if (!dbg_time) return;
        (void)hipStreamSynchronize(s);
        const auto now = std::chrono::steady_clock::now();
        fprintf(stderr, "[gpk] index build: %-28s %8.3f ms\n", what, std::chrono::duration<double, std::milli>(now - t_last).count());
        t_last = now;
    };
    int slot = 4;
    auto keep = [&](void* p) {
        if (slot < 24) ix->owned[slot++] = p;
    };

    uint32_t* part_geom = nullptr;
    if (d.type == GPK_GEOM_MULTIPOLYGON) {
        GPK_HIP(cached_malloc((void**)&part_geom, sizeof(uint32_t) * (size_t)(n_parts ? n_parts : 1)));
        keep(part_geom);
        GPK_LAUNCH("gpk_pipidx_part_geom", part_geom_kernel, blocks_for(d.n_geoms), dim3(256), 0, s, d, part_geom);
    }
    int32_t* ring_part;
    GPK_TRY(t.alloc(&ring_part, (size_t)n_rings));
    GPK_LAUNCH("gpk_pipidx_ring_part", ring_part_kernel, blocks_for(n_parts), dim3(256), 0, s, d, n_parts, ring_part);

    double4* ring_bbox;
    GPK_TRY(t.alloc(&ring_bbox, (size_t)n_rings));
    GPK_TRY(ring_bboxes(a, ring_bbox, s));
    stamp("ring maps + ring boxes");
    int32_t *row0 = nullptr, *nrows, *slab_base = nullptr;
    GPK_HIP(cached_malloc((void**)&row0, sizeof(int32_t) * (size_t)n_rings));
    keep(row0);
    GPK_HIP(cached_malloc((void**)&slab_base, sizeof(int32_t) * (size_t)(n_rings + 1)));
    keep(slab_base);
    GPK_TRY(t.alloc(&nrows, (size_t)n_rings));
    unsigned long long* btot;
    int64_t max_scan = n_cells > d.n_coords ? n_cells : d.n_coords;
    if (n_rings > max_scan) max_scan = n_rings;
    GPK_TRY(t.alloc(&btot, (size_t)((max_scan + 255) / 256 + 4)));
    int32_t* ring_starts;
    GPK_TRY(t.alloc(&ring_starts, (size_t)d.n_coords + 2));
    GPK_HIP(hipMemsetAsync(ring_starts, 0, sizeof(int32_t) * (size_t)(d.n_coords + 2), s));
    GPK_LAUNCH("gpk_pipidx_ring_start", ring_start_kernel, blocks_for(n_rings), dim3(256), 0, s, d.ring_off, n_rings, d.n_coords, ring_starts);
    GPK_TRY(exclusive_scan_i32(ring_starts, d.n_coords + 1, ring_starts, nullptr, btot, s));
    const int32_t* coord_ring = ring_starts + 1;
    FineGrid gs = g;
    gs.R = g.R * (PIP_SLAB_MUL << PIP_FINE_LOG2);
    gs.fw = g.fw / (PIP_SLAB_MUL << PIP_FINE_LOG2);
    gs.fh = g.fh / (PIP_SLAB_MUL << PIP_FINE_LOG2);
    gs.inv_fw = g.inv_fw * (double)(PIP_SLAB_MUL << PIP_FINE_LOG2);
    gs.inv_fh = g.inv_fh * (double)(PIP_SLAB_MUL << PIP_FINE_LOG2);
    int32_t n_slabs = 0, n_edges = 0;
    int32_t *slab_cnt = nullptr, *slab_off = nullptr, *cursor = nullptr;
    const int slab_off_slot = slot++;
    int32_t n_refined = 0, *n_refined_dev;
    GPK_TRY(t.alloc(&n_refined_dev, 64));
    for (int max_shift = PIP_FINE_LOG2;; max_shift = 0) {
        GPK_HIP(hipMemsetAsync(n_refined_dev, 0, sizeof(int32_t), s));
        GPK_LAUNCH("gpk_pipidx_ring_rows", ring_rows_kernel, blocks_for(n_rings), dim3(256), 0, s, ring_bbox, n_rings, d.ring_off, gs, max_shift,
                   row0, nrows, n_refined_dev);
        GPK_TRY(exclusive_scan_i32(nrows, n_rings, slab_base, nullptr, btot, s));
        GPK_HIP(d2h_small(&n_slabs, slab_base + n_rings, sizeof n_slabs, s));
        GPK_HIP(d2h_small(&n_refined, n_refined_dev, sizeof n_refined, s));
        GPK_HIP(sync_small(s));
        if ((int64_t)n_slabs > max_scan) {
            max_scan = n_slabs;
            GPK_TRY(t.alloc(&btot, (size_t)((max_scan + 255) / 256 + 4)));
        }
        GPK_TRY(t.alloc(&slab_cnt, (size_t)n_slabs + 1));
        GPK_TRY(t.alloc(&cursor, (size_t)n_slabs + 1));
        if (slab_off) cached_free(slab_off);
        ix->owned[slab_off_slot] = slab_off = nullptr;
        GPK_HIP(cached_malloc((void**)&slab_off, sizeof(int32_t) * (size_t)(n_slabs + 1)));
        ix->owned[slab_off_slot] = slab_off;
        GPK_HIP(hipMemsetAsync(slab_cnt, 0, sizeof(int32_t) * (size_t)(n_slabs + 1), s));
        GPK_HIP(hipMemsetAsync(slab_off, 0, sizeof(int32_t) * (size_t)(n_slabs + 1), s));
        GPK_LAUNCH("gpk_pipidx_slab_count", slab_register_kernel<false>, blocks_for(d.n_coords), dim3(256), 0, s, d, coord_ring, gs, row0, slab_base,
                   slab_cnt, (double4*)nullptr);
        n_edges = 0;
        if (n_slabs > 0) {
            GPK_TRY(exclusive_scan_i32(slab_cnt, n_slabs, slab_off, cursor, btot, s));
            GPK_HIP(d2h_small(&n_edges, slab_off + n_slabs, sizeof n_edges, s));
            GPK_HIP(sync_small(s));
        }
        if (max_shift == 0 || (int64_t)n_edges <= 8 * d.n_coords + (1 << 20)) break;
    }
    stamp("slab rows + counts");
    double4* edges = nullptr;
    int32_t* slab_vidx = nullptr;
    const bool edge_copies = sizeof(double4) * (size_t)n_edges <= (size_t(256) << 20);
    if (edge_copies) {
        GPK_HIP(cached_malloc((void**)&edges, sizeof(double4) * (size_t)(n_edges ? n_edges : 1)));
        keep(edges);
        if ((int64_t)n_edges <= ((int64_t)64 << 20)) GPK_TRY(t.alloc(&slab_vidx, (size_t)(n_edges ? n_edges : 1)));
    } else {
        GPK_HIP(cached_malloc((void**)&slab_vidx, sizeof(int32_t) * (size_t)n_edges));
        keep(slab_vidx);
    }
    GPK_LAUNCH("gpk_pipidx_slab_fill", slab_register_kernel<true>, blocks_for(d.n_coords), dim3(256), 0, s, d, coord_ring, gs, row0, slab_base,
               cursor, edges, slab_vidx);

    stamp("slab fill (+ edges malloc)");
    PartInfo* part_info = nullptr;
    GPK_HIP(cached_malloc((void**)&part_info, sizeof(PartInfo) * (size_t)(n_parts ? n_parts : 1)));
    keep(part_info);
    GPK_LAUNCH("gpk_pipidx_part_info", part_info_kernel, blocks_for(n_parts), dim3(256), 0, s, d, n_parts, row0, slab_base, part_info);

    PipView pv;
    memset(&pv, 0, sizeof pv);
    pv.R = R;
    pv.rx0 = g.rx0;
    pv.ry0 = g.ry0;
    pv.fw = g.fw;
    pv.fh = g.fh;
    pv.inv_fw = g.inv_fw;
    pv.inv_fh = g.inv_fh;
    pv.part_geom = part_geom;
    pv.part_info = part_info;
    pv.ring_row0 = row0;
    pv.ring_slab_base = slab_base;
    pv.slab_off = slab_off;
    pv.slab_edges = edges;
    pv.slab_vidx = edge_copies ? nullptr : slab_vidx;
    pv.slab_xy = d.xy;

    stamp("part info");
    int32_t *mark_cnt, *mark_off;
    GPK_TRY(t.alloc(&mark_cnt, (size_t)d.n_coords + 1));
    GPK_TRY(t.alloc(&mark_off, (size_t)d.n_coords + 1));
    GPK_LAUNCH("gpk_pipidx_mark_count", mark_kernel<false>, blocks_for(d.n_coords), dim3(256), 0, s, d, coord_ring, g, ring_part, mark_cnt,
               (unsigned long long*)nullptr);
    GPK_TRY(exclusive_scan_i32(mark_cnt, d.n_coords, mark_off, nullptr, btot, s));
    unsigned long long n_marks_raw = 0;
    GPK_HIP(d2h_small(&n_marks_raw, btot + (d.n_coords + 255) / 256, sizeof n_marks_raw, s));
    GPK_HIP(sync_small(s));
    if (n_marks_raw >= (1ull << 31))
        return GPK_OK;
    stamp("mark count + scan");
    unsigned long long *keys, *sorted, *marks;
    GPK_TRY(t.alloc(&keys, (size_t)n_marks_raw));
    GPK_TRY(t.alloc(&sorted, (size_t)n_marks_raw));
    marks = keys;
    int64_t n_marks = 0;
    int32_t* mark_start;
    GPK_TRY(t.alloc(&mark_start, (size_t)n_cells + 2));
    GPK_HIP(hipMemsetAsync(mark_start, 0, sizeof(int32_t) * (size_t)(n_cells + 2), s));
    if (n_marks_raw > 0) {
        GPK_LAUNCH("gpk_pipidx_mark_fill", mark_kernel<true>, blocks_for(d.n_coords), dim3(256), 0, s, d, coord_ring, g, ring_part, mark_off, keys);
        size_t tmp_bytes = 0;
        unsigned cell_bits = 1;
        while (cell_bits < 32 && (1ll << cell_bits) < n_cells) ++cell_bits;
        const unsigned sort_end = 32 + cell_bits;
        GPK_HIP(rocprim::radix_sort_keys(nullptr, tmp_bytes, keys, sorted, (size_t)n_marks_raw, 0, sort_end, s));
        char* tmp;
        GPK_TRY(t.alloc(&tmp, tmp_bytes));
        GPK_HIP(rocprim::radix_sort_keys(tmp, tmp_bytes, keys, sorted, (size_t)n_marks_raw, 0, sort_end, s));
        int32_t *flag, *pos;
        GPK_TRY(t.alloc(&flag, (size_t)n_marks_raw + 1));
        GPK_TRY(t.alloc(&pos, (size_t)n_marks_raw + 1));
        unsigned long long* btot2;
        GPK_TRY(t.alloc(&btot2, (size_t)((n_marks_raw + 255) / 256 + 4)));
        GPK_LAUNCH("gpk_pipidx_unique_flags", unique_flags_kernel, blocks_for((int64_t)n_marks_raw), dim3(256), 0, s, sorted,
                   (int64_t)n_marks_raw, flag);
        GPK_TRY(exclusive_scan_i32(flag, (int64_t)n_marks_raw, pos, nullptr, btot2, s));
        GPK_LAUNCH("gpk_pipidx_unique_compact", unique_compact_kernel, blocks_for((int64_t)n_marks_raw), dim3(256), 0, s, sorted,
                   (int64_t)n_marks_raw, pos, marks, mark_start);
        GPK_TRY(exclusive_scan_i32(mark_start, n_cells, mark_start, nullptr, btot, s));
        int32_t nu = 0;
        GPK_HIP(d2h_small(&nu, pos + n_marks_raw, sizeof nu, s));
        GPK_HIP(sync_small(s));
        n_marks = nu;
    }

    stamp("mark fill + sort + unique");
    uint32_t* cell = nullptr;
    GPK_HIP(cached_malloc((void**)&cell, sizeof(uint32_t) * (size_t)n_cells));
    keep(cell);
    int32_t *need, *list_off;
    GPK_TRY(t.alloc(&need, (size_t)n_cells + 1));
    GPK_TRY(t.alloc(&list_off, (size_t)n_cells + 1));
    uint32_t* cell_scratch = nullptr;
    GPK_TRY(t.alloc(&cell_scratch, (size_t)n_cells * CELL_SCRATCH));
    GPK_LAUNCH("gpk_pipidx_cell_count", cell_build_kernel<false>, blocks_for(n_cells), dim3(256), 0, s, d, ix->v, pv, g, marks, mark_start,
               need, (const int32_t*)nullptr, cell, (uint32_t*)nullptr, cell_scratch, (const double4*)ring_bbox);
    GPK_TRY(exclusive_scan_i32(need, n_cells, list_off, nullptr, btot, s));
    int32_t list_len = 0;
    GPK_HIP(d2h_small(&list_len, list_off + n_cells, sizeof list_len, s));
    GPK_HIP(sync_small(s));
    if ((unsigned)list_len >= (1u << 30)) return GPK_OK;
    uint32_t* list = nullptr;
    GPK_HIP(cached_malloc((void**)&list, sizeof(uint32_t) * (size_t)(list_len ? list_len : 1)));
    keep(list);
    GPK_LAUNCH("gpk_pipidx_cell_fill", cell_build_kernel<true>, blocks_for(n_cells), dim3(256), 0, s, d, ix->v, pv, g, marks, mark_start,
               need, list_off, cell, list, cell_scratch, (const double4*)ring_bbox);
    GPK_HIP(hipStreamSynchronize(s));
    pv.cell = cell;
    pv.list = list;
    ix->pip_list_heavy = (int64_t)list_len * 4 > n_cells ? 1 : 0;

    stamp("cells");
    int32_t n_sub = 0, n_sub2 = 0;
    bool sub_overflow = false;
    int32_t* swork_cell = nullptr;
    uint32_t* swork_part = nullptr;
    SubCell* sub = nullptr;
    SubCell2* sub2 = nullptr;
    static_assert(PIP_SLAB_MUL == 2, "SubCell stores exactly two adjacent slab ranges");
    int route_logR = 0;
    if (R <= PIP_ROUTE_RMAX)
        while ((1 << route_logR) < R) ++route_logR;
    const bool level2_ok = g.pad_x / PIP_SUB > ulp64 && g.pad_y / PIP_SUB > ulp64 && R * PIP_SUB <= 32768;
    if (level2_ok) {
        int32_t *sflag, *spos, *sflag2, *spos2;
        GPK_TRY(t.alloc(&sflag, (size_t)n_cells + 1));
        GPK_TRY(t.alloc(&spos, (size_t)n_cells + 1));
        GPK_TRY(t.alloc(&sflag2, (size_t)n_cells + 1));
        GPK_TRY(t.alloc(&spos2, (size_t)n_cells + 1));
        GPK_LAUNCH("gpk_pipidx_sub_flag", sub_flag_kernel, blocks_for(n_cells), dim3(256), 0, s, cell, (const uint32_t*)list, n_cells, route_logR, sflag,
                   sflag2);
        GPK_TRY(exclusive_scan_i32(sflag, n_cells, spos, nullptr, btot, s));
        GPK_TRY(exclusive_scan_i32(sflag2, n_cells, spos2, nullptr, btot, s));
        GPK_HIP(d2h_small(&n_sub, spos + n_cells, sizeof n_sub, s));
        GPK_HIP(d2h_small(&n_sub2, spos2 + n_cells, sizeof n_sub2, s));
        GPK_HIP(sync_small(s));
        if ((unsigned)n_sub >= SUB2_BIT || (unsigned)n_sub2 >= SUB2_BIT) {
            n_sub = n_sub2 = 0;
            sub_overflow = true;
        }
        if (getenv("GPK_DEBUG_INDEX")) fprintf(stderr, "[gpk] level 2: %d one-part cells, %d two-part cells of %lld\n", n_sub, n_sub2, (long long)n_cells);
        if ((int64_t)n_sub2 < 4 * (int64_t)n_sub) n_sub2 = 0;
        if (n_sub > 0) {
            GPK_HIP(cached_malloc((void**)&sub, sizeof(SubCell) * (size_t)n_sub));
            keep(sub);
            GPK_HIP(hipMemsetAsync(sub, 0, sizeof(SubCell) * (size_t)n_sub, s));
            GPK_TRY(t.alloc(&swork_cell, (size_t)n_sub));
            GPK_TRY(t.alloc(&swork_part, (size_t)n_sub));
            GPK_LAUNCH("gpk_pipidx_sub_work", sub_work_kernel, blocks_for(n_cells), dim3(256), 0, s, (const uint32_t*)cell, (const int32_t*)sflag,
                       (const int32_t*)spos, n_cells, route_logR, swork_cell, swork_part);
            GPK_LAUNCH("gpk_pipidx_sub_head", sub_head_kernel, blocks_for(n_sub), dim3(256), 0, s, pv, g, (const int32_t*)swork_cell,
                       (const uint32_t*)swork_part, (int64_t)n_sub, sub);
            if (n_refined == 0) {
                GPK_LAUNCH("gpk_pipidx_sub_build_fast", (sub_build_kernel<1, true, 1>), blocks_for((int64_t)n_sub * PIP_SUB * PIP_SUB), dim3(256), 0, s, d, pv, g,
                           (const int32_t*)nullptr, (const int32_t*)nullptr, n_cells, (const uint32_t*)cell, (const uint32_t*)list, sub, (SubCell2*)nullptr,
                           (const int32_t*)swork_cell, (const uint32_t*)swork_part, (int64_t)n_sub);
                GPK_LAUNCH("gpk_pipidx_sub_build_rest", (sub_build_kernel<1, true, 2>), blocks_for((int64_t)n_sub * PIP_SUB * PIP_SUB), dim3(256), 0, s, d, pv, g,
                           (const int32_t*)nullptr, (const int32_t*)nullptr, n_cells, (const uint32_t*)cell, (const uint32_t*)list, sub, (SubCell2*)nullptr,
                           (const int32_t*)swork_cell, (const uint32_t*)swork_part, (int64_t)n_sub);
            } else {
                GPK_LAUNCH("gpk_pipidx_sub_build", (sub_build_kernel<1, true, 0>), blocks_for((int64_t)n_sub * PIP_SUB * PIP_SUB), dim3(256), 0, s, d, pv, g,
                           (const int32_t*)nullptr, (const int32_t*)nullptr, n_cells, (const uint32_t*)cell, (const uint32_t*)list, sub, (SubCell2*)nullptr,
                           (const int32_t*)swork_cell, (const uint32_t*)swork_part, (int64_t)n_sub);
            }
        }
        if (n_sub2 > 0) {
            GPK_HIP(cached_malloc((void**)&sub2, sizeof(SubCell2) * (size_t)n_sub2));
            keep(sub2);
            GPK_HIP(hipMemsetAsync(sub2, 0, sizeof(SubCell2) * (size_t)n_sub2, s));
            GPK_LAUNCH("gpk_pipidx_sub2_build", sub_build_kernel<2>, blocks_for(n_cells * PIP_SUB * PIP_SUB), dim3(256), 0, s, d, pv, g, sflag2, spos2,
                       n_cells, (const uint32_t*)cell, (const uint32_t*)list, (SubCell*)nullptr, sub2);
        }
        if (n_sub > 0 || n_sub2 > 0) {
            GPK_LAUNCH("gpk_pipidx_sub_commit", sub_commit_kernel, blocks_for(n_cells), dim3(256), 0, s, sflag, spos, n_sub2 > 0 ? sflag2 : nullptr,
                       spos2, n_cells, route_logR, cell);
            GPK_HIP(hipStreamSynchronize(s));
        }
    }
    stamp("level-2 records");
    pv.sub = sub;
    pv.sub2 = sub2;
    int32_t n_lrec = 0;
    SubCell* lrec = nullptr;
    if (level2_ok && list_len > 0 && list_records) {
        int32_t *lcnt, *lpos;
        GPK_TRY(t.alloc(&lcnt, (size_t)n_cells + 1));
        GPK_TRY(t.alloc(&lpos, (size_t)n_cells + 1));
        GPK_LAUNCH("gpk_pipidx_lrec_count", lrec_count_kernel, blocks_for(n_cells), dim3(256), 0, s, (const uint32_t*)cell, (const uint32_t*)list, n_cells,
                   lcnt);
        GPK_TRY(exclusive_scan_i32(lcnt, n_cells, lpos, nullptr, btot, s));
        GPK_HIP(d2h_small(&n_lrec, lpos + n_cells, sizeof n_lrec, s));
        GPK_HIP(sync_small(s));
        if (getenv("GPK_DEBUG_INDEX")) fprintf(stderr, "[gpk] level 2: %d boundary entries in list cells (list length %d)\n", n_lrec, list_len);
        if (n_lrec > 0 && (int64_t)n_lrec < (int64_t)1 << 28) {
            int32_t* work_cell;
            uint32_t* work_part;
            GPK_TRY(t.alloc(&work_cell, (size_t)n_lrec));
            GPK_TRY(t.alloc(&work_part, (size_t)n_lrec));
            GPK_HIP(cached_malloc((void**)&lrec, sizeof(SubCell) * (size_t)n_lrec));
            keep(lrec);
            GPK_HIP(hipMemsetAsync(lrec, 0, sizeof(SubCell) * (size_t)n_lrec, s));
            GPK_LAUNCH("gpk_pipidx_lrec_assign", lrec_assign_kernel, blocks_for(n_cells), dim3(256), 0, s, (const uint32_t*)cell, list, n_cells,
                       (const int32_t*)lpos, work_cell, work_part);
            GPK_LAUNCH("gpk_pipidx_lrec_head", sub_head_kernel, blocks_for(n_lrec), dim3(256), 0, s, pv, g, (const int32_t*)work_cell,
                       (const uint32_t*)work_part, (int64_t)n_lrec, lrec);
            if (n_refined == 0) {
                GPK_LAUNCH("gpk_pipidx_lrec_build", (sub_build_kernel<1, true, 1>), blocks_for((int64_t)n_lrec * PIP_SUB * PIP_SUB), dim3(256), 0, s, d, pv, g,
                           (const int32_t*)nullptr, (const int32_t*)nullptr, n_cells, (const uint32_t*)cell, (const uint32_t*)list, lrec, (SubCell2*)nullptr,
                           (const int32_t*)work_cell, (const uint32_t*)work_part, (int64_t)n_lrec);
                GPK_LAUNCH("gpk_pipidx_lrec_build", (sub_build_kernel<1, true, 2>), blocks_for((int64_t)n_lrec * PIP_SUB * PIP_SUB), dim3(256), 0, s, d, pv, g,
                           (const int32_t*)nullptr, (const int32_t*)nullptr, n_cells, (const uint32_t*)cell, (const uint32_t*)list, lrec, (SubCell2*)nullptr,
                           (const int32_t*)work_cell, (const uint32_t*)work_part, (int64_t)n_lrec);
            } else {
                GPK_LAUNCH("gpk_pipidx_lrec_build", (sub_build_kernel<1, true, 0>), blocks_for((int64_t)n_lrec * PIP_SUB * PIP_SUB), dim3(256), 0, s, d, pv, g,
                           (const int32_t*)nullptr, (const int32_t*)nullptr, n_cells, (const uint32_t*)cell, (const uint32_t*)list, lrec, (SubCell2*)nullptr,
                           (const int32_t*)work_cell, (const uint32_t*)work_part, (int64_t)n_lrec);
            }
            GPK_HIP(hipStreamSynchronize(s));
        } else {
            n_lrec = 0;
        }
    }
    stamp("list-cell records");
    pv.lrec = lrec;
    if (list_len > 0 && !lrec) {
        float4* part_box = nullptr;
        GPK_HIP(cached_malloc((void**)&part_box, sizeof(float4) * (size_t)(n_parts ? n_parts : 1)));
        keep(part_box);
        GPK_LAUNCH("gpk_pipidx_part_box", part_box_kernel, blocks_for(n_parts), dim3(256), 0, s, d, n_parts, (const double4*)ring_bbox, part_box);
        pv.part_box = part_box;
        ix->nbytes += (int64_t)(sizeof(float4) * (size_t)n_parts);
    }
    const bool boundary_cells_have_records = level2_ok && !sub_overflow && n_sub2 == 0;
    ix->pip_lean = (int64_t)list_len * 8 <= (int64_t)n_sub && n_refined == 0 && boundary_cells_have_records ? 1 : 0;
    if (getenv("GPK_DEBUG_INDEX")) fprintf(stderr, "[gpk] lean join kernel eligible: %d (list %d, refined rings: %s, one-part records %d)\n", ix->pip_lean, list_len, n_refined ? "some" : "none", n_sub);
    if (ix->pip_lean && slab_vidx && n_sub > 0 && swork_cell && d.n_coords + d.n_rings * CHAIN_MAX < ((int64_t)1 << (32 - HCHAIN_START_SHIFT))) {
        const int64_t n_ext = d.n_coords + d.n_rings * CHAIN_MAX;
        double2* cxy = nullptr;
        GPK_HIP(cached_malloc((void**)&cxy, sizeof(double2) * (size_t)n_ext));
        keep(cxy);
        uint32_t* hword;
        GPK_TRY(t.alloc(&hword, (size_t)n_sub * 2 + 2));
        pv.sub = sub;
        GPK_LAUNCH("gpk_pipidx_chain_xy", chain_xy_kernel, blocks_for(n_ext), dim3(256), 0, s, d, cxy);
        GPK_LAUNCH("gpk_pipidx_half_chain", half_chain_kernel, blocks_for((int64_t)n_sub * 2), dim3(256), 0, s, d, pv, g,
                   (const int32_t*)swork_cell, (const uint32_t*)swork_part, (int64_t)n_sub, (const int32_t*)slab_vidx, (const SubCell*)sub, hword);
        GPK_LAUNCH("gpk_pipidx_chain_commit", half_chain_commit_kernel, blocks_for(n_sub), dim3(256), 0, s, sub, (int64_t)n_sub, (const uint32_t*)hword);
        pv.chain_xy = cxy;
        ix->nbytes += (int64_t)(sizeof(double2) * (size_t)n_ext);
        uint32_t route_host[2] = {0u, 0u};
        if (R <= PIP_ROUTE_RMAX) {
            RouteWord* route = nullptr;
            const int64_t n_words = n_cells / 32;
            GPK_HIP(cached_malloc((void**)&route, sizeof(RouteWord) * (size_t)n_words));
            keep(route);
            uint32_t* route_counts;
            GPK_TRY(t.alloc(&route_counts, 2));
            GPK_HIP(hipMemsetAsync(route_counts, 0, 2 * sizeof(uint32_t), s));
            GPK_LAUNCH("gpk_pipidx_route", route_build_kernel, blocks_for(n_words), dim3(256), 0, s, (const uint32_t*)cell, n_words, route_logR, route,
                       route_counts);
            GPK_HIP(d2h_small(route_host, route_counts, sizeof route_host, s));
            pv.route = route;
            ix->nbytes += (int64_t)(sizeof(RouteWord) * (size_t)n_words);
        }
        GPK_HIP(sync_small(s));
        ix->route_own = (int32_t)route_host[0];
        ix->route_single = (int32_t)route_host[1];
        if (getenv("GPK_DEBUG_INDEX")) fprintf(stderr, "[gpk] half-cell chains: %d records, %lld extended coordinates%s\n", n_sub, (long long)n_ext, pv.route ? ", routing image" : "");
        stamp("local chains");
    }
    ix->nbytes += (int64_t)(sizeof(SubCell) * (size_t)n_sub + sizeof(SubCell2) * (size_t)n_sub2 + sizeof(SubCell) * (size_t)n_lrec);
    ix->pip = pv;
    ix->nbytes += (int64_t)(sizeof(uint32_t) * (size_t)n_cells + sizeof(uint32_t) * (size_t)list_len + (pv.slab_edges ? sizeof(double4) : sizeof(int32_t)) * (size_t)n_edges +
                            sizeof(int32_t) * (size_t)(n_slabs + 1) + sizeof(int32_t) * (size_t)(2 * n_rings + 1) +
                            (part_geom ? sizeof(uint32_t) * (size_t)n_parts : 0) + sizeof(PartInfo) * (size_t)n_parts);
    return GPK_OK;
}

}
```

### geopolars_amd/spatial_index.py

```python
from __future__ import annotations

import ctypes as C
from dataclasses import dataclass
from typing import Optional

import numpy as np

from . import _abi
from ._abi import MEM_DEVICE, MEM_HOST, PREDICATES
from .geoarrow import DeviceGeoArray, GeoArrowArray
from .geoseries import (
    LINEAL,
    POLYGONAL,
    GeoSeries,
    _abi_name,
    _mismatch,
    dwithin_distance_arg,
    intersection_families_arg,
    intersection_min_measure_arg,
    line_clip_call,
    point_relation_sides,
    polygon_clip_call,
    predicate_route,
    relation_sides,
)


def _ptr(t):
    return t.data_ptr() if t is not None else None


def _index_parts(for_points: bool, full: bool, light: bool) -> int:
    parts = _abi.INDEX_BBOX_GRID | (_abi.INDEX_PIP if for_points else 0) | (_abi.INDEX_PIP_FULL if for_points and full else 0)
    if for_points and light and not full:
        parts |= _abi.INDEX_PIP_LIGHT
    return parts


class SpatialIndex:

    def __init__(self, series: GeoSeries, stream: int = 0, for_points: bool = True, full: bool = False, light: bool = False):
        self.series = series
        h = C.c_void_p()
        parts = _index_parts(for_points, full, light)
        _abi.check(_abi.lib().gpk_index_build_ex(series.device().handle, parts, None, stream, C.byref(h)))
        self._h = h

    @staticmethod
    def from_device(dev: DeviceGeoArray, stream: int = 0, for_points: bool = True, bboxes=None, full: bool = False, light: bool = False) -> "SpatialIndex":
        self = SpatialIndex.__new__(SpatialIndex)
        self.series = None
        self._dev = dev
        h = C.c_void_p()
        parts = _index_parts(for_points, full, light)
        _abi.check(_abi.lib().gpk_index_build_ex(dev.handle, parts, _ptr(bboxes), stream, C.byref(h)))
        self._h = h
        return self

    @property
    def handle(self) -> C.c_void_p:
        return self._h

    def nbytes(self) -> int:
        n = C.c_int64(0)
        _abi.check(_abi.lib().gpk_index_nbytes(self._h, C.byref(n)))
        return int(n.value)

    def describe(self) -> dict:
        out = (C.c_int64 * 8)()
        _abi.check(_abi.lib().gpk_index_describe(self._h, out))
        return {"R": int(out[0]), "lean": bool(out[1]), "chains": bool(out[2]), "route": bool(out[3]), "list_heavy": bool(out[4])}

    def query_envelopes(self, boxes, mode: str = "contained", stream: int = 0) -> tuple[np.ndarray, np.ndarray]:
        lib = _abi.lib()
        b = np.ascontiguousarray(np.asarray(boxes, dtype=np.float64).reshape(-1, 4))
        n = len(b)
        m = {"contained": _abi.QUERY_CONTAINED, "intersecting": _abi.QUERY_INTERSECTING}[mode]
        counts = np.zeros(n, dtype=np.uint32)
        n_pairs = C.c_int64(0)
        _abi.check(lib.gpk_index_query_envelope(self._h, b.ctypes.data, n, m, counts.ctypes.data, None, 0, C.byref(n_pairs), MEM_HOST, stream))
        pairs = np.zeros((int(n_pairs.value), 2), dtype=np.uint32)
        if len(pairs):
            _abi.check(lib.gpk_index_query_envelope(self._h, b.ctypes.data, n, m, counts.ctypes.data, pairs.ctypes.data, len(pairs), C.byref(n_pairs), MEM_HOST, stream))
        return pairs, counts

    def locate_in_envelope(self, lower, upper) -> np.ndarray:
        pairs, _ = self.query_envelopes([[lower[0], lower[1], upper[0], upper[1]]], "contained")
        return pairs[:, 1].astype(np.int64)

    def locate_in_envelope_intersecting(self, lower, upper) -> np.ndarray:
        pairs, _ = self.query_envelopes([[lower[0], lower[1], upper[0], upper[1]]], "intersecting")
        return pairs[:, 1].astype(np.int64)

    def free(self) -> None:
        if self._h:
            _abi.lib().gpk_index_free(self._h)
            self._h = C.c_void_p()

    def __del__(self):
        try:
            self.free()
        except Exception:
            pass


@dataclass
class SpatialJoinArgs:

    join_type: str = "inner"
    predicate: str = "intersects"
    l_suffix: Optional[str] = "_left"
    r_suffix: Optional[str] = "_right"
    l_index: Optional[SpatialIndex] = None
    r_index: Optional[SpatialIndex] = None
    l_geom_type: int = -1
    r_geom_type: int = -1
    geometry_encoding: str = "wkb"


GEOMETRY_ENCODINGS = ("wkb", "geoarrow")


def _pairs_with_retry(n: int, call, want_dist: bool = False, payload=np.float64):
    n_pairs = C.c_int64(0)
    capacity = max(1024, 4 * n)
    while True:
        pairs = np.empty((capacity, 2), dtype=np.uint32)
        dist = np.empty(capacity, dtype=payload) if want_dist else None
        rc = call(pairs.ctypes.data, dist.ctypes.data if want_dist else None, capacity, C.byref(n_pairs))
        if rc == _abi.GPK_ERR_CAPACITY and int(n_pairs.value) > capacity:
            capacity = int(n_pairs.value)
            continue
        _abi.check(rc)
        h = int(n_pairs.value)
        return pairs[:h].copy(), (dist[:h].copy() if want_dist else None)


def join_pairs(
    left: GeoSeries,
    right: GeoSeries,
    predicate: str = "intersects",
    r_index: Optional[SpatialIndex] = None,
    left_row_base: int = 0,
) -> tuple[np.ndarray, np.ndarray]:
    lib = _abi.lib()
    n = len(left)
    counts = np.empty(n, dtype=np.uint32)
    rh = r_index.handle if r_index is not None else None
    pred = PREDICATES[predicate]
    call = lambda pairs_ptr, _dist, capacity, n_pairs: lib.gpk_spatial_join(
        left.device().handle, right.device().handle, rh, pred, left_row_base, counts.ctypes.data, pairs_ptr, capacity, n_pairs, MEM_HOST, None)
    return _pairs_with_retry(n, call)[0], counts


def join_pairs_device(left: DeviceGeoArray, right: DeviceGeoArray, r_index: SpatialIndex, predicate: str, out_counts, out_pairs, left_row_base: int = 0, stream: int = 0) -> int:
    n_pairs = C.c_int64(0)
    rh, cap = r_index.handle if r_index is not None else None, out_pairs.shape[0] if out_pairs is not None else 0
    _abi.check(_abi.lib().gpk_spatial_join(
        left.handle, right.handle, rh, PREDICATES[predicate], left_row_base, _ptr(out_counts), _ptr(out_pairs), cap, C.byref(n_pairs), MEM_DEVICE, stream))
    return int(n_pairs.value)


def join_pairs_enqueue(left: DeviceGeoArray, right: DeviceGeoArray, r_index: SpatialIndex, predicate: str, out_counts, out_pairs, n_pairs_out, left_row_base: int = 0, stream: int = 0) -> None:
    cap = out_pairs.shape[0] if out_pairs is not None else 0
    _abi.check(_abi.lib().gpk_spatial_join_async(
        left.handle, right.handle, r_index.handle, PREDICATES[predicate], left_row_base, _ptr(out_counts), _ptr(out_pairs), cap, _ptr(n_pairs_out), stream))


JOIN_TYPES = {"inner": 0, "left": 1}


def join_indices(counts: np.ndarray, pairs: np.ndarray, join_type: str = "inner", left_row_base: int = 0) -> tuple[np.ndarray, np.ndarray]:
    lib = _abi.lib()
    counts = np.ascontiguousarray(counts, dtype=np.uint32)
    pairs = np.ascontiguousarray(pairs, dtype=np.uint32).reshape(-1, 2)
    n_rows = C.c_int64(0)
    jt = JOIN_TYPES[join_type]
    args = (counts.ctypes.data, pairs.ctypes.data if len(pairs) else None, len(counts), len(pairs), left_row_base, jt)
    _abi.check(lib.gpk_join_indices(*args, None, None, 0, C.byref(n_rows), MEM_HOST, None))
    n = int(n_rows.value)
    li, ri = np.empty(n, dtype=np.int64), np.empty(n, dtype=np.int64)
    if n:
        _abi.check(lib.gpk_join_indices(*args, li.ctypes.data, ri.ctypes.data, n, C.byref(n_rows), MEM_HOST, None))
    return li, ri


def take_column(column, idx: np.ndarray):
    import pyarrow as pa

    lib = _abi.lib()
    arr = column.combine_chunks() if isinstance(column, pa.ChunkedArray) else column
    if arr.offset != 0:
        arr = pa.concat_arrays([arr])
    t = arr.type
    idx = np.ascontiguousarray(idx, dtype=np.int64)
    n_idx, n = len(idx), len(arr)
    bufs = arr.buffers()
    validity = np.frombuffer(bufs[0], dtype=np.uint8) if bufs[0] is not None else None
    vptr = validity.ctypes.data if validity is not None else None
    out_valid = np.zeros((n_idx + 7) // 8, dtype=np.uint8)
    if pa.types.is_binary(t) or pa.types.is_string(t):
        offsets = np.frombuffer(bufs[1], dtype=np.int32)[: n + 1] if bufs[1] is not None else np.zeros(1, np.int32)
        values = np.frombuffer(bufs[2], dtype=np.uint8) if bufs[2] is not None and bufs[2].size else np.zeros(1, np.uint8)
        n_bytes = C.c_int64(0)
        out_off = np.zeros(n_idx + 1, dtype=np.int32)
        args = (values.ctypes.data, offsets.ctypes.data, vptr, n, idx.ctypes.data, n_idx, out_off.ctypes.data)
        _abi.check(lib.gpk_take_binary(*args, None, 0, C.byref(n_bytes), out_valid.ctypes.data, MEM_HOST, None))
        out_vals = np.empty(max(int(n_bytes.value), 1), dtype=np.uint8)
        if n_bytes.value:
            _abi.check(lib.gpk_take_binary(*args, out_vals.ctypes.data, int(n_bytes.value), C.byref(n_bytes), out_valid.ctypes.data, MEM_HOST, None))
        return pa.Array.from_buffers(t, n_idx, [pa.py_buffer(out_valid.tobytes()), pa.py_buffer(out_off.tobytes()), pa.py_buffer(out_vals[: int(n_bytes.value)].tobytes())])
    if pa.types.is_boolean(t):
        bits = 1
    elif pa.types.is_primitive(t):
        bits = t.bit_width
    else:
        raise _abi.GeopolarsHipError(_abi.GPK_ERR_INVALID_ARGUMENT, f"join assembly: column type {t} is not supported")
    data = np.frombuffer(bufs[1], dtype=np.uint8) if bufs[1] is not None else np.zeros(16, np.uint8)
    out = np.zeros((n_idx + 7) // 8 if bits == 1 else n_idx * (bits // 8), dtype=np.uint8)
    _abi.check(lib.gpk_take_fixed(data.ctypes.data, bits, vptr, n, idx.ctypes.data, n_idx, out.ctypes.data if len(out) else None, out_valid.ctypes.data, MEM_HOST, None))
    return pa.Array.from_buffers(t, n_idx, [pa.py_buffer(out_valid.tobytes()), pa.py_buffer(out.tobytes())])


def _geometry_type_of(table, hint: int, hint_name: str) -> int:
    import pyarrow as pa

    if hint >= 0:
        return hint
    t = table.schema.field("geometry").type
    ext = (table.schema.field("geometry").metadata or {}).get(b"ARROW:extension:name")
    if isinstance(t, pa.BaseExtensionType):
        ext, t = t.extension_name.encode(), t.storage_type
    depth = 0
    while pa.types.is_list(t) or pa.types.is_large_list(t):
        depth, t = depth + 1, t.value_type
    if depth in (1, 2) and not ext:
        kinds = "LineString or MultiPoint" if depth == 1 else "Polygon or MultiLineString"
        raise _abi.GeopolarsHipError(
            _abi.GPK_ERR_INVALID_ARGUMENT,
            f"spatial_join: a GeoArrow geometry column of {depth} list level(s) without an ARROW:extension:name is a {kinds} column: "
            f"name the type in SpatialJoinArgs.{hint_name}",
        )
    return -1


def _as_wkb(column, geo: GeoSeries):
    import pyarrow as pa

    if pa.types.is_binary(column.type) or pa.types.is_large_binary(column.type):
        return column
    return geo.device().to_arrow("wkb")


def _assemble(lhs, rhs, lgeo: GeoSeries, rgeo: GeoSeries, li: np.ndarray, ri: np.ndarray, l_suffix, r_suffix, distance_col=None, dist=None,
              geometry_encoding: str = "wkb"):
    import pyarrow as pa

    cols, names = [], []
    for table, geo, idx, suffix in ((lhs, lgeo, li, l_suffix), (rhs, rgeo, ri, r_suffix)):
        for name in table.column_names:
            if name == "geometry" and geometry_encoding == "geoarrow":
                cols.append(geo.device().take(idx).to_arrow("struct"))
            else:
                cols.append(take_column(_as_wkb(table.column(name), geo) if name == "geometry" else table.column(name), idx))
            names.append(name + (suffix or ""))
    if distance_col is not None:
        matched = ri >= 0
        d = np.zeros(len(ri), dtype=np.float64)
        d[matched] = dist
        cols.append(pa.array(d, type=pa.float64(), mask=~matched))
        names.append(distance_col)
    return pa.table(cols, names=names)


def spatial_join(lhs, rhs, options: Optional[SpatialJoinArgs] = None):
    options = options or SpatialJoinArgs()
    if options.join_type not in ("inner", "left"):
        raise _abi.GeopolarsHipError(_abi.GPK_ERR_INVALID_ARGUMENT, "Failed to generate the spatial index for the left dataframe")
    if options.geometry_encoding not in GEOMETRY_ENCODINGS:
        raise _abi.GeopolarsHipError(
            _abi.GPK_ERR_INVALID_ARGUMENT, f"spatial_join: geometry_encoding {options.geometry_encoding!r}: one of {', '.join(GEOMETRY_ENCODINGS)}")
    lgeo = GeoSeries.from_arrow(lhs.column("geometry"), _geometry_type_of(lhs, options.l_geom_type, "l_geom_type"))
    rgeo = GeoSeries.from_arrow(rhs.column("geometry"), _geometry_type_of(rhs, options.r_geom_type, "r_geom_type"))
    r_index = options.r_index or SpatialIndex(rgeo)
    pairs, counts = join_pairs(lgeo, rgeo, options.predicate, r_index)
    li, ri = join_indices(counts, pairs, options.join_type)
    return _assemble(lhs, rhs, lgeo, rgeo, li, ri, options.l_suffix, options.r_suffix, geometry_encoding=options.geometry_encoding)




@dataclass
class SpatialJoinNearestArgs:

    join_type: str = "inner"
    max_distance: Optional[float] = None
    distance_col: Optional[str] = None
    l_suffix: Optional[str] = "_left"
    r_suffix: Optional[str] = "_right"
    r_index: Optional[SpatialIndex] = None
    l_geom_type: int = -1
    r_geom_type: int = -1


def _max_distance_arg(max_distance: Optional[float]) -> float:
    if max_distance is None:
        return float("inf")
    d = float(max_distance)
    if not d >= 0.0:
        raise _abi.GeopolarsHipError(_abi.GPK_ERR_INVALID_ARGUMENT, f"nearest join: max_distance must be >= 0 (None: no limit), got {max_distance!r}")
    return d


def _require_point_series(left: GeoSeries) -> None:
    t = left._array.geom_type if left._array is not None else left._dev.geom_type
    if t != _abi.GEOM_POINT:
        raise _abi.MismatchedGeometry(_abi.GPK_ERR_MISMATCHED_GEOMETRY, f"nearest join: the left side must be POINT (found type {t})")


def nearest_pairs(
    left: GeoSeries,
    right: GeoSeries,
    r_index: Optional[SpatialIndex] = None,
    max_distance: Optional[float] = None,
    left_row_base: int = 0,
) -> tuple[np.ndarray, np.ndarray, np.ndarray]:
    md = _max_distance_arg(max_distance)
    _require_point_series(left)
    lib = _abi.lib()
    n = len(left)
    counts = np.empty(n, dtype=np.uint32)
    rh = r_index.handle if r_index is not None else None
    call = lambda pairs_ptr, dist_ptr, capacity, n_pairs: lib.gpk_nearest_join(
        left.device().handle, right.device().handle, rh, md, left_row_base, counts.ctypes.data, pairs_ptr, dist_ptr, capacity, n_pairs, MEM_HOST, None)
    pairs, dist = _pairs_with_retry(n, call, want_dist=True)
    return pairs, counts, dist


def nearest_pairs_device(
    left: DeviceGeoArray,
    right: DeviceGeoArray,
    r_index: Optional[SpatialIndex],
    out_counts,
    out_pairs,
    out_dist=None,
    max_distance: Optional[float] = None,
    left_row_base: int = 0,
    stream: int = 0,
) -> int:
    md = _max_distance_arg(max_distance)
    if left.geom_type != _abi.GEOM_POINT:
        raise _abi.MismatchedGeometry(_abi.GPK_ERR_MISMATCHED_GEOMETRY, f"nearest join: the left side must be POINT (found type {left.geom_type})")
    n_pairs = C.c_int64(0)
    rh, cap = r_index.handle if r_index is not None else None, out_pairs.shape[0] if out_pairs is not None else 0
    _abi.check(_abi.lib().gpk_nearest_join(
        left.handle, right.handle, rh, md, left_row_base, _ptr(out_counts), _ptr(out_pairs), _ptr(out_dist), cap, C.byref(n_pairs), MEM_DEVICE, stream))
    return int(n_pairs.value)


NEAREST_FAMILIES = (_abi.GEOM_POINT, _abi.GEOM_MULTIPOINT, _abi.GEOM_LINESTRING, _abi.GEOM_MULTILINESTRING, _abi.GEOM_POLYGON, _abi.GEOM_MULTIPOLYGON)


def _require_nearest_families(left_family: int, right_family: int) -> None:
    for side, t in (("left", left_family), ("right", right_family)):
        if t not in NEAREST_FAMILIES:
            raise _mismatch(f"nearest join: the {side} side must be Point, MultiPoint, LineString, MultiLineString, Polygon or MultiPolygon (found {_abi_name(t)})")


def nearest_pairs_any(
    left: GeoSeries,
    right: GeoSeries,
    r_index: Optional[SpatialIndex] = None,
    max_distance: Optional[float] = None,
    left_row_base: int = 0,
# ... 691 lines not shown
```

### include/geopolars_hip.h

```cpp
#ifndef GEOPOLARS_HIP_H
#define GEOPOLARS_HIP_H

#include <stddef.h>
#include <stdint.h>

#ifdef __cplusplus
extern "C" {
#endif

#define GPK_OK                        0
#define GPK_ERR_MISMATCHED_GEOMETRY   1
#define GPK_ERR_INVALID_OFFSETS       2
#define GPK_ERR_NULL_UNSUPPORTED      3
#define GPK_ERR_DEVICE                4
#define GPK_ERR_OOM                   5
#define GPK_ERR_INVALID_ARGUMENT      6
#define GPK_ERR_CAPACITY              7

#define GPK_GEOM_POINT             0
#define GPK_GEOM_LINESTRING        1
#define GPK_GEOM_POLYGON           3
#define GPK_GEOM_MULTIPOINT        4
#define GPK_GEOM_MULTILINESTRING   5
#define GPK_GEOM_MULTIPOLYGON      6

#define GPK_MEM_HOST    0
#define GPK_MEM_DEVICE  1

#define GPK_PRED_INTERSECTS  0
#define GPK_PRED_CONTAINS    1
#define GPK_PRED_WITHIN      2

typedef struct gpk_geoarrow_desc {
    int32_t        geom_type;
    int32_t        mem_space;
    int64_t        n_geoms;
    int64_t        n_coords;
    const double*  xy;
    const int32_t* geom_offsets;
    const int32_t* part_offsets;
    const int32_t* ring_offsets;
    int64_t        n_parts;
    int64_t        n_rings;
    const uint8_t* validity;
    const double*  x;
    const double*  y;
} gpk_geoarrow_desc;

typedef struct gpk_geoarray gpk_geoarray;
typedef struct gpk_index    gpk_index;

const char* gpk_version(void);
int32_t gpk_last_error(char* buf, size_t cap);
int32_t gpk_device_count(int32_t* out_n);
int32_t gpk_device_info(char* name_buf, size_t cap, int32_t* out_cus);
int32_t gpk_device_cache_release(void);

int32_t gpk_geoarray_upload(const gpk_geoarrow_desc* desc, void* stream, gpk_geoarray** out);
int32_t gpk_geoarray_free(gpk_geoarray* a);
int32_t gpk_geoarray_invalidate(gpk_geoarray* a);
int32_t gpk_geoarray_nbytes(const gpk_geoarray* a, int64_t* out_bytes);

int32_t gpk_wkb_decode(const uint8_t* wkb_values, const int32_t* wkb_offsets, int64_t n_rows,
                       const uint8_t* validity, int64_t counts[5], double* xy,
                       int32_t* geom_offsets, int32_t* part_offsets, int32_t* ring_offsets);

int32_t gpk_geoarray_from_wkb(const uint8_t* wkb_values, const int32_t* wkb_offsets, int64_t n_rows,
                              const uint8_t* validity, int32_t mem_space, void* stream,
                              gpk_geoarray** out, int32_t* out_geom_type);
int32_t gpk_wkb_encode(const gpk_geoarrow_desc* desc, int32_t* out_offsets, uint8_t* out_values,
                       int64_t capacity, int64_t* n_bytes);
int32_t gpk_geoarray_to_wkb(const gpk_geoarray* a, int32_t* out_offsets, uint8_t* out_values,
                            int64_t capacity, int64_t* n_bytes, int32_t out_space, void* stream);
#ifndef ARROW_C_DATA_INTERFACE
#define ARROW_C_DATA_INTERFACE
struct ArrowSchema {
    const char* format;
    const char* name;
    const char* metadata;
    int64_t flags;
    int64_t n_children;
    struct ArrowSchema** children;
    struct ArrowSchema* dictionary;
    void (*release)(struct ArrowSchema*);
    void* private_data;
};
struct ArrowArray {
    int64_t length;
    int64_t null_count;
    int64_t offset;
    int64_t n_buffers;
    int64_t n_children;
    const void** buffers;
    struct ArrowArray** children;
    struct ArrowArray* dictionary;
    void (*release)(struct ArrowArray*);
    void* private_data;
};
#endif
int32_t gpk_geoarray_from_arrow(const struct ArrowArray* array, const struct ArrowSchema* schema, int32_t geom_type_hint,
                                void* stream, gpk_geoarray** out, int32_t* out_geom_type);
#define GPK_ARROW_WKB 0
#define GPK_ARROW_INTERLEAVED 1
#define GPK_ARROW_STRUCT 2
int32_t gpk_geoarray_to_arrow(const gpk_geoarray* a, int32_t layout, void* stream, struct ArrowArray* out_array, struct ArrowSchema* out_schema);
int32_t gpk_geoarray_download(const gpk_geoarray* a, int64_t sizes[4], double* xy, int32_t* geom_offsets,
                              int32_t* part_offsets, int32_t* ring_offsets, void* stream);

int32_t gpk_geoarray_validity(const gpk_geoarray* a, uint8_t* out_bitmap, int32_t* out_has_validity, void* stream);

int32_t gpk_area(const gpk_geoarray* a, double* out, int32_t out_space, void* stream);
int32_t gpk_signed_area(const gpk_geoarray* a, double* out, int32_t out_space, void* stream);
int32_t gpk_centroid(const gpk_geoarray* a, double* out_xy, uint8_t* out_valid, int32_t out_space,
                     void* stream);
int32_t gpk_representative_point(const gpk_geoarray* a, double* out_xy, uint8_t* out_valid, double* out_width, int32_t out_space, void* stream);
int32_t gpk_bounds(const gpk_geoarray* a, double* out4, int32_t out_space, void* stream);
int32_t gpk_euclidean_length(const gpk_geoarray* a, double* out, int32_t out_space, void* stream);
int32_t gpk_affine_transform(const gpk_geoarray* a, const double m[6], double* out_xy,
                             int32_t out_space, void* stream);
int32_t gpk_affine_transform_rows(const gpk_geoarray* a, const double* matrices, double* out_xy,
                                  int32_t out_space, void* stream);
#define GPK_AFFINE_ROTATE 0
#define GPK_AFFINE_SCALE  1
#define GPK_AFFINE_SKEW   2
#define GPK_ORIGIN_CENTROID 0
#define GPK_ORIGIN_CENTER   1
#define GPK_ORIGIN_POINT    2
int32_t gpk_affine_about_origin(const gpk_geoarray* a, int32_t kind, double p0, double p1, int32_t origin,
                                double ox, double oy, double* out_xy, int32_t out_space, void* stream);
int32_t gpk_crs_supported(int32_t epsg);
int32_t gpk_reproject(const gpk_geoarray* a, int32_t src_epsg, int32_t dst_epsg, double* out_xy, int64_t* n_failed,
                      int32_t out_space, void* stream);
int32_t gpk_envelope(const gpk_geoarray* a, double* out_xy, uint8_t* out_valid, int32_t out_space, void* stream);
int32_t gpk_exterior(const gpk_geoarray* a, double* out_xy, int32_t* out_geom_offsets, int64_t* n_out_coords,
                     int32_t out_space, void* stream);
int32_t gpk_explode(const gpk_geoarray* a, int32_t* out_parent, int32_t parent_space, void* stream, gpk_geoarray** out);
int32_t gpk_geoarray_len(const gpk_geoarray* a, int64_t* out_n);
int32_t gpk_geom_type(const gpk_geoarray* a, int8_t* out, int32_t out_space, void* stream);
int32_t gpk_is_empty(const gpk_geoarray* a, uint8_t* out, int32_t out_space, void* stream);
int32_t gpk_is_ring(const gpk_geoarray* a, uint8_t* out, int32_t out_space, void* stream);
int32_t gpk_point_xy(const gpk_geoarray* a, double* out_x, double* out_y, int32_t out_space, void* stream);
#define GPK_GEODESIC_KARNEY    0
#define GPK_GEODESIC_HAVERSINE 1
#define GPK_GEODESIC_VINCENTY  2
int32_t gpk_geodesic_length(const gpk_geoarray* a, int32_t method, double* out, int32_t out_space, void* stream);
#define GPK_GEODESIC_AREA_SIGNED 1u
int32_t gpk_geodesic_area(const gpk_geoarray* a, uint32_t flags, double* out_area, double* out_perimeter, int32_t out_space,
                          void* stream);
int32_t gpk_geodesic_inverse(const gpk_geoarray* a, const gpk_geoarray* b, const uint32_t* b_rows, double* out_s12, double* out_azi1,
                             double* out_azi2, int32_t out_space, void* stream);
int32_t gpk_geodesic_direct(const gpk_geoarray* a, const double* azi1, int64_t n_azi, const double* s12, int64_t n_s12, double* out_xy,
                            double* out_azi2, int32_t out_space, void* stream);
int32_t gpk_simplify(const gpk_geoarray* a, double epsilon, double* out_xy, int32_t* out_seq_offsets,
                     int64_t* n_out_coords, int32_t out_space, void* stream);
int32_t gpk_convex_hull(const gpk_geoarray* a, double* out_xy, int32_t* out_ring_offsets,
                        int32_t out_space, void* stream);
#define MBG_CIRCLE_ITERS 64
int32_t gpk_minimum_rotated_rectangle(const gpk_geoarray* a, double* out_xy, uint8_t* out_valid, int32_t out_space, void* stream);
int32_t gpk_minimum_bounding_circle(const gpk_geoarray* a, double* out_center_xy, double* out_radius, uint8_t* out_valid, int32_t out_space,
                                    void* stream);

int32_t gpk_distance_rowwise(const gpk_geoarray* a, const gpk_geoarray* b, const uint32_t* b_rows,
                             double* out, int32_t out_space, void* stream);
typedef struct gpk_rowmap gpk_rowmap;
int32_t gpk_rowmap_build(const gpk_geoarray* b, const uint32_t* b_rows, int64_t n_rows, int32_t rows_space,
                         void* stream, gpk_rowmap** out);
int32_t gpk_rowmap_free(gpk_rowmap* map);
int32_t gpk_rowmap_nbytes(const gpk_rowmap* map, int64_t* out_bytes);
int32_t gpk_distance_rowmap(const gpk_geoarray* a, const gpk_geoarray* b, const gpk_rowmap* map, double* out,
                            int32_t out_space, void* stream);
#define GPK_FRECHET_MAX_SHORT 16384
#define GPK_MAX_SUBDIVISIONS 4096
int32_t gpk_hausdorff_distance(const gpk_geoarray* a, const gpk_geoarray* b, const uint32_t* b_rows, int32_t subdivisions,
                               double* out, int32_t out_space, void* stream);
int32_t gpk_frechet_distance(const gpk_geoarray* a, const gpk_geoarray* b, const uint32_t* b_rows, int32_t subdivisions,
                             double* out, int64_t* n_over, int32_t out_space, void* stream);
int32_t gpk_predicate_rowwise(const gpk_geoarray* a, const gpk_geoarray* b, const uint32_t* b_rows,
                              int32_t predicate, uint8_t* out, int32_t out_space, void* stream);

int32_t gpk_index_build(const gpk_geoarray* a, void* stream, gpk_index** out);
#define GPK_INDEX_BBOX_GRID 1
#define GPK_INDEX_PIP       2
#define GPK_INDEX_PIP_LIGHT 4
#define GPK_INDEX_PIP_FULL  8
int32_t gpk_index_build_ex(const gpk_geoarray* a, int32_t parts, const double* bbox4_dev, void* stream,
                           gpk_index** out);
int32_t gpk_index_free(gpk_index* idx);
#define GPK_QUERY_CONTAINED    0
#define GPK_QUERY_INTERSECTING 1
int32_t gpk_index_query_envelope(const gpk_index* idx, const double* boxes4, int64_t n_boxes, int32_t mode,
                                 uint32_t* out_counts, uint32_t* out_pairs, int64_t pair_capacity, int64_t* n_pairs,
                                 int32_t space, void* stream);
int32_t gpk_index_nbytes(const gpk_index* idx, int64_t* out_bytes);
int32_t gpk_index_describe(const gpk_index* idx, int64_t out[8]);

int32_t gpk_spatial_join(const gpk_geoarray* left, const gpk_geoarray* right,
                         const gpk_index* right_index, int32_t predicate, uint32_t left_row_base,
                         uint32_t* out_counts, uint32_t* out_pairs, int64_t pair_capacity,
                         int64_t* n_pairs, int32_t out_space, void* stream);

int32_t gpk_nearest_join(const gpk_geoarray* left, const gpk_geoarray* right, const gpk_index* right_index, double max_distance,
                         uint32_t left_row_base, uint32_t* out_counts, uint32_t* out_pairs, double* out_dist, int64_t pair_capacity,
                         int64_t* n_pairs, int32_t out_space, void* stream);

int32_t gpk_nearest_join_any(const gpk_geoarray* left, const gpk_geoarray* right, const gpk_index* right_index, double max_distance,
                             uint32_t left_row_base, uint32_t* out_counts, uint32_t* out_pairs, double* out_dist, int64_t pair_capacity,
                             int64_t* n_pairs, int32_t out_space, void* stream);

#define GPK_KNN_MAX_K 64
#define GPK_KNN_EXCLUDE_SELF 1u
int32_t gpk_knn_join(const gpk_geoarray* left, const gpk_geoarray* right, const gpk_index* right_index, int32_t k, double max_distance,
                     uint32_t flags, uint32_t left_row_base, uint32_t* out_counts, uint32_t* out_pairs, double* out_dist,
                     int64_t pair_capacity, int64_t* n_pairs, int32_t out_space, void* stream);

int32_t gpk_dwithin_join(const gpk_geoarray* left, const gpk_geoarray* right, const gpk_index* right_index, double distance,
                         uint32_t left_row_base, uint32_t* out_counts, uint32_t* out_pairs, double* out_dist, int64_t pair_capacity,
                         int64_t* n_pairs, int32_t out_space, void* stream);
int32_t gpk_dwithin_rowwise(const gpk_geoarray* a, const gpk_geoarray* b, const uint32_t* b_rows, double distance, uint8_t* out,
                            int32_t out_space, void* stream);

#define GPK_LP_INTERIOR 1
#define GPK_LP_BOUNDARY 2
#define GPK_LP_EXTERIOR 4
int32_t gpk_line_polygon_relation(const gpk_geoarray* lines, const gpk_geoarray* polys, const uint32_t* poly_rows, uint8_t* out_mask,
                                  int32_t out_space, void* stream);
#define GPK_LP_PRED_INTERSECTS 0
#define GPK_LP_PRED_WITHIN 1
#define GPK_LP_PRED_COVERED_BY 2
#define GPK_LP_PRED_CROSSES 3
#define GPK_LP_PRED_TOUCHES 4
int32_t gpk_line_polygon_join(const gpk_geoarray* left, const gpk_geoarray* right, const gpk_index* right_index, int32_t predicate,
                              uint32_t left_row_base, uint32_t* out_counts, uint32_t* out_pairs, uint8_t* out_mask, int64_t pair_capacity,
                              int64_t* n_pairs, int32_t out_space, void* stream);

#define GPK_PP_INTERIORS 1
#define GPK_PP_BOUNDARIES 2
#define GPK_PP_A_OUTSIDE 4
#define GPK_PP_B_OUTSIDE 8
int32_t gpk_polygon_relation(const gpk_geoarray* a, const gpk_geoarray* b, const uint32_t* b_rows, uint8_t* out_mask, int32_t out_space,
                             void* stream);
#define GPK_PP_PRED_INTERSECTS 0
#define GPK_PP_PRED_WITHIN 1
#define GPK_PP_PRED_CONTAINS 2
#define GPK_PP_PRED_TOUCHES 3
#define GPK_PP_PRED_OVERLAPS 4
#define GPK_PP_PRED_EQUALS 5
#define GPK_PP_PRED_CONTAINS_PROPERLY 6
int32_t gpk_polygon_relation_join(const gpk_geoarray* left, const gpk_geoarray* right, const gpk_index* right_index, int32_t predicate,
                                  uint32_t left_row_base, uint32_t* out_counts, uint32_t* out_pairs, uint8_t* out_mask,
                                  int64_t pair_capacity, int64_t* n_pairs, int32_t out_space, void* stream);

int32_t gpk_intersection_measure(const gpk_geoarray* a, const gpk_geoarray* b, const uint32_t* b_rows, double* out, int32_t out_space,
                                 void* stream);
int32_t gpk_intersection_measure_join(const gpk_geoarray* left, const gpk_geoarray* right, const gpk_index* right_index, double min_measure,
                                      uint32_t left_row_base, uint32_t* out_counts, uint32_t* out_pairs, double* out_measure,
                                      int64_t pair_capacity, int64_t* n_pairs, int32_t out_space, void* stream);

#define GPK_CLIP_INSIDE  0
#define GPK_CLIP_OUTSIDE 1
#define GPK_CLIP_DROP_EMPTY 1
int32_t gpk_line_clip(const gpk_geoarray* lines, const gpk_geoarray* polys, const uint32_t* line_rows, const uint32_t* poly_rows,
                      int64_t n_rows, int32_t rows_space, int32_t mode, int32_t flags, int32_t* out_src, int32_t src_space, void* stream,
                      gpk_geoarray** out);

#define GPK_PCLIP_INTERSECTION 0
#define GPK_PCLIP_DIFFERENCE   1
int32_t gpk_polygon_clip(const gpk_geoarray* a, const gpk_geoarray* b, const uint32_t* a_rows, const uint32_t* b_rows, int64_t n_rows,
                         int32_t rows_space, int32_t mode, int32_t flags, int32_t* out_src, int32_t src_space, uint8_t* out_status,
                         int32_t status_space, void* stream, gpk_geoarray** out);

#define GPK_PUNION_UNION 0
int32_t gpk_polygon_union(const gpk_geoarray* a, const gpk_geoarray* b, const uint32_t* a_rows, const uint32_t* b_rows, int64_t n_rows,
                          int32_t rows_space, int32_t mode, int32_t flags, int32_t* out_src, int32_t src_space, uint8_t* out_status,
                          int32_t status_space, void* stream, gpk_geoarray** out);
int32_t gpk_union_all_pairs(const int32_t* group, const uint32_t* rows, int64_t n, int64_t base, uint32_t* a_rows, uint32_t* b_rows,
                            int32_t* next_group, uint32_t* next_rows, int64_t* out_counts, void* stream);

#define GPK_LL_INTERIORS 1
#define GPK_LL_SHARED_PIECE 2
#define GPK_LL_INT_BND 4
#define GPK_LL_BND_INT 8
#define GPK_LL_BND_BND 16
#define GPK_LL_A_OUTSIDE 32
#define GPK_LL_B_OUTSIDE 64
int32_t gpk_line_relation(const gpk_geoarray* a, const gpk_geoarray* b, const uint32_t* b_rows, uint8_t* out_mask, int32_t out_space,
                          void* stream);
#define GPK_LL_PRED_INTERSECTS 0
#define GPK_LL_PRED_WITHIN 1
#define GPK_LL_PRED_CONTAINS 2
#define GPK_LL_PRED_COVERED_BY 3
#define GPK_LL_PRED_COVERS 4
#define GPK_LL_PRED_CROSSES 5
#define GPK_LL_PRED_TOUCHES 6
#define GPK_LL_PRED_OVERLAPS 7
#define GPK_LL_PRED_EQUALS 8
int32_t gpk_line_relation_join(const gpk_geoarray* left, const gpk_geoarray* right, const gpk_index* right_index, int32_t predicate,
                               uint32_t left_row_base, uint32_t* out_counts, uint32_t* out_pairs, uint8_t* out_mask, int64_t pair_capacity,
                               int64_t* n_pairs, int32_t out_space, void* stream);

#define GPK_PT_INTERIOR 1
#define GPK_PT_BOUNDARY 2
#define GPK_PT_EXTERIOR 4
#define GPK_PT_B_OUTSIDE 8
int32_t gpk_point_relation(const gpk_geoarray* points, const gpk_geoarray* other, const uint32_t* other_rows, uint8_t* out_mask,
                           int32_t out_space, void* stream);
#define GPK_PT_PRED_INTERSECTS 0
#define GPK_PT_PRED_WITHIN 1
#define GPK_PT_PRED_CONTAINS 2
#define GPK_PT_PRED_COVERED_BY 3
#define GPK_PT_PRED_COVERS 4
#define GPK_PT_PRED_CROSSES 5
#define GPK_PT_PRED_TOUCHES 6
#define GPK_PT_PRED_OVERLAPS 7
#define GPK_PT_PRED_EQUALS 8
int32_t gpk_point_relation_join(const gpk_geoarray* left, const gpk_geoarray* right, const gpk_index* right_index, int32_t predicate,
                                uint32_t left_row_base, uint32_t* out_counts, uint32_t* out_pairs, uint8_t* out_mask, int64_t pair_capacity,
                                int64_t* n_pairs, int32_t out_space, void* stream);

#define GPK_VALID 0
#define GPK_INVALID_COORDINATE 1
#define GPK_INVALID_RING_SHAPE 2
#define GPK_INVALID_RING_SELF_INTERSECTION 3
#define GPK_INVALID_RINGS_CROSS 4
#define GPK_INVALID_HOLE_OUTSIDE_SHELL 5
#define GPK_INVALID_NESTED_HOLES 6
#define GPK_INVALID_NESTED_MEMBERS 7
#define GPK_INVALID_DISCONNECTED_INTERIOR 8
#define GPK_INVALID_NULL 9
int32_t gpk_validity(const gpk_geoarray* a, uint8_t* out_code, int32_t* out_where, int32_t out_space, void* stream);
int32_t gpk_is_simple(const gpk_geoarray* a, uint8_t* out, int32_t out_space, void* stream);

#define GPK_TRI_OK     0
#define GPK_TRI_EMPTY  1
#define GPK_TRI_FAILED 2
int32_t gpk_triangulate(const gpk_geoarray* a, uint32_t* out_index, int64_t tri_capacity, int32_t* out_tri_offsets, uint8_t* out_status,
                        int64_t* n_triangles, int32_t out_space, void* stream);

int32_t gpk_closest_point_rowwise(const gpk_geoarray* a, const gpk_geoarray* b, const uint32_t* b_rows, double* out_xy, int32_t* out_seg,
                                  int32_t out_space, void* stream);
int32_t gpk_line_locate_point(const gpk_geoarray* pts, const gpk_geoarray* lines, const uint32_t* line_rows, int32_t normalized, double* out,
                              int32_t out_space, void* stream);
int32_t gpk_line_interpolate_point(const gpk_geoarray* lines, const double* distances, int64_t n_distances, int32_t normalized,
                                   double* out_xy, uint8_t* out_valid, int32_t out_space, void* stream);

int32_t gpk_spatial_join_async(const gpk_geoarray* left, const gpk_geoarray* right,
                               const gpk_index* right_index, int32_t predicate, uint32_t left_row_base,
                               uint32_t* out_counts, uint32_t* out_pairs, int64_t pair_capacity,
                               int64_t* n_pairs_dev, void* stream);

#define GPK_JOIN_INNER 0
#define GPK_JOIN_LEFT  1
int32_t gpk_join_indices(const uint32_t* counts, const uint32_t* pairs, int64_t n_left, int64_t n_pairs,
                         uint32_t left_row_base, int32_t join_type, int64_t* out_l, int64_t* out_r,
                         int64_t capacity, int64_t* n_rows, int32_t space, void* stream);
int32_t gpk_take_fixed(const void* values, int32_t elem_bits, const uint8_t* validity, int64_t n_values,
                       const int64_t* idx, int64_t n_idx, void* out_values, uint8_t* out_validity,
                       int32_t space, void* stream);
int32_t gpk_take_binary(const uint8_t* values, const int32_t* offsets, const uint8_t* validity, int64_t n_values,
                        const int64_t* idx, int64_t n_idx, int32_t* out_offsets, uint8_t* out_values,
                        int64_t capacity, int64_t* n_bytes, uint8_t* out_validity, int32_t space, void* stream);

int32_t gpk_geoarray_take(const gpk_geoarray* a, const int64_t* idx, int64_t n_idx, int32_t idx_space, void* stream, gpk_geoarray** out);
int32_t gpk_geoarray_filter(const gpk_geoarray* a, const uint8_t* mask, int32_t mask_bits, int32_t mask_space, void* stream, gpk_geoarray** out, int64_t* n_kept);

int32_t gpk_segmentize(const gpk_geoarray* a, double max_segment_length, const double* per_row, int32_t per_row_space, void* stream, gpk_geoarray** out);
int32_t gpk_remove_repeated_points(const gpk_geoarray* a, double tolerance, void* stream, gpk_geoarray** out);
int32_t gpk_reverse(const gpk_geoarray* a, void* stream, gpk_geoarray** out);
int32_t gpk_orient_polygons(const gpk_geoarray* a, int32_t exterior_cw, void* stream, gpk_geoarray** out);

int32_t gpk_geoarray_concat(const gpk_geoarray* const* chunks, int32_t n_chunks, void* stream, gpk_geoarray** out,
                            int64_t* out_row_bases, int64_t* out_bytes);

typedef struct gpk_comm gpk_comm;
int32_t gpk_comm_unique_id(uint8_t out_id[128]);
int32_t gpk_comm_init(int32_t rank, int32_t world, const uint8_t id[128], gpk_comm** out);
int32_t gpk_comm_free(gpk_comm* comm);
int32_t gpk_comm_info(const gpk_comm* comm, int32_t* out_rank, int32_t* out_world);
int32_t gpk_comm_mock_world(int32_t world, void** out_world);
int32_t gpk_comm_init_mock(int32_t rank, void* world, gpk_comm** out);
int32_t gpk_comm_mock_world_free(void* world);
int32_t gpk_allgatherv_geoarray(gpk_comm* comm, const gpk_geoarray* shard, void* stream, gpk_geoarray** out,
                                int64_t* out_row_base, int64_t* out_bytes);
int32_t gpk_allgatherv_rows_f64(gpk_comm* comm, const double* local_dev, int64_t n_local, int32_t width, double* out_dev,
                                int64_t out_capacity_rows, int64_t* out_total_rows, int64_t* out_counts, void* stream);

int32_t gpk_join_stats_enable(int32_t on);
int32_t gpk_join_stats(int64_t out[4], int32_t reset);

int32_t gpk_profile_enable(int32_t on);
int32_t gpk_profile_filter(const char* substr);
int32_t gpk_profile_reset(void);
int32_t gpk_profile_query(const char* substr, double* out_ms, int64_t* out_launches);

#ifdef __cplusplus
}
#endif
#endif
```

Measured before the change: 127800 billion.

## Add speculative single-sync PIP index build path for small polygon sets

Adds a speculative build path for the point-in-polygon index, used when the coordinate count is small. Device-side capacity checks and stop flags let the kernels run back-to-back with preallocated buffers, replacing many host round-trips that read back sizes. Per-cell mark deduplication now uses bucket scatter and insertion sort instead of a global sort. If a capacity is exceeded the path aborts and falls back to the exact build, which adds redundant work in that case. It also adds debug table export and build-path reporting.

```diff
diff --git a/geopolars_amd/_abi.py b/geopolars_amd/_abi.py
--- a/geopolars_amd/_abi.py
+++ b/geopolars_amd/_abi.py
@@ -33,6 +33,10 @@
 INDEX_PIP = 2
 INDEX_PIP_LIGHT = 4
 INDEX_PIP_FULL = 8
+INDEX_PIP_EXACT_BUILD = 16
+INDEX_PIP_SMALL_BUILD = 32
+INDEX_TABLES = {"cell": 0, "list": 1, "sub": 2, "sub2": 3, "lrec": 4, "chain_xy": 5, "route": 6, "part_info": 7, "part_box": 8, "slab_off": 9,
+                "slab_edges": 10, "ring_row0": 11, "ring_slab_base": 12, "part_geom": 13}
 QUERY_CONTAINED, QUERY_INTERSECTING = 0, 1
 PREDICATES = {"intersects": PRED_INTERSECTS, "contains": PRED_CONTAINS, "within": PRED_WITHIN}
 LP_INTERIOR, LP_BOUNDARY, LP_EXTERIOR = 1, 2, 4
@@ -175,6 +179,7 @@
     "gpk_index_free": (C.c_int32, [_VP]),
     "gpk_index_nbytes": (C.c_int32, [_VP, C.POINTER(C.c_int64)]),
     "gpk_index_describe": (C.c_int32, [_VP, C.POINTER(C.c_int64)]),
+    "gpk_index_debug_table": (C.c_int32, [_VP, C.c_int32, _VP, C.c_int64, C.POINTER(C.c_int64), _VP]),
     "gpk_index_query_envelope": (C.c_int32, [_VP, _VP, C.c_int64, C.c_int32, _VP, _VP, C.c_int64, C.POINTER(C.c_int64), C.c_int32, _VP]),
     "gpk_spatial_join": (
         C.c_int32,
diff --git a/geopolars_amd/csrc/gpk_gridindex.hip b/geopolars_amd/csrc/gpk_gridindex.hip
--- a/geopolars_amd/csrc/gpk_gridindex.hip
+++ b/geopolars_amd/csrc/gpk_gridindex.hip
@@ -152,6 +152,43 @@
     out[4] = idx->pip_list_heavy;
     out[5] = idx->route_own;
     out[6] = idx->route_single;
+    out[7] = idx->pip_build_path;
+    return GPK_OK;
+}
+
+int32_t gpk_index_debug_table(const gpk_index* idx, int32_t which, void* dst_dev, int64_t capacity, int64_t* nbytes, void* stream) {
+    if (!idx || !nbytes) return fail(GPK_ERR_INVALID_ARGUMENT, "NULL argument");
+    const PipView& pv = idx->pip;
+    const int64_t* c = idx->pip_counts;
+    const int64_t n_cells = (int64_t)pv.R * pv.R;
+    const void* src = nullptr;
+    int64_t bytes = 0;
+    switch (which) {
+        case GPK_INDEX_TABLE_CELL: src = pv.cell, bytes = 4 * n_cells; break;
+        case GPK_INDEX_TABLE_LIST: src = pv.list, bytes = 4 * c[2]; break;
+        case GPK_INDEX_TABLE_SUB: src = pv.sub, bytes = (int64_t)sizeof(SubCell) * c[3]; break;
+        case GPK_INDEX_TABLE_SUB2: src = pv.sub2, bytes = (int64_t)sizeof(SubCell2) * c[4]; break;
+        case GPK_INDEX_TABLE_LREC: src = pv.lrec, bytes = (int64_t)sizeof(SubCell) * c[5]; break;
+        case GPK_INDEX_TABLE_CHAIN_XY: src = pv.chain_xy, bytes = (int64_t)sizeof(double2) * c[6]; break;
+        case GPK_INDEX_TABLE_ROUTE: src = pv.route, bytes = (int64_t)sizeof(RouteWord) * (n_cells / 32); break;
+        case GPK_INDEX_TABLE_PART_INFO: src = pv.part_info, bytes = (int64_t)sizeof(PartInfo) * c[7]; break;
+        case GPK_INDEX_TABLE_PART_BOX: src = pv.part_box, bytes = (int64_t)sizeof(float4) * c[7]; break;
+        case GPK_INDEX_TABLE_SLAB_OFF: src = pv.slab_off, bytes = 4 * (c[0] + 1); break;
+        case GPK_INDEX_TABLE_SLAB_EDGES:
+            src = pv.slab_edges ? (const void*)pv.slab_edges : (const void*)pv.slab_vidx;
+            bytes = (pv.slab_edges ? (int64_t)sizeof(double4) : 4) * c[1];
+            break;
+        case GPK_INDEX_TABLE_RING_ROW0: src = pv.ring_row0, bytes = 4 * idx->n_rings; break;
+        case GPK_INDEX_TABLE_RING_SLAB: src = pv.ring_slab_base, bytes = 4 * (idx->n_rings + 1); break;
+        case GPK_INDEX_TABLE_PART_GEOM: src = pv.part_geom, bytes = 4 * c[7]; break;
+        default: return fail(GPK_ERR_INVALID_ARGUMENT, "gpk_index_debug_table: no table %d", which);
+    }
+    if (!pv.R || !src) bytes = 0;
+    *nbytes = bytes;
+    if (!dst_dev || bytes == 0) return GPK_OK;
+    if (bytes > capacity) return fail(GPK_ERR_CAPACITY, "gpk_index_debug_table: table %d holds %lld bytes, capacity %lld", which, (long long)bytes, (long long)capacity);
+    const hipError_t e = hipMemcpyAsync(dst_dev, src, (size_t)bytes, hipMemcpyDeviceToDevice, (hipStream_t)stream);
+    if (e != hipSuccess) return fail(GPK_ERR_DEVICE, "gpk_index_debug_table: copy failed: %s", hipGetErrorString(e));
     return GPK_OK;
 }
 
@@ -280,7 +317,8 @@
     ix->nbytes = (int64_t)(sizeof(double4) * (size_t)n + sizeof(GridParams) + sizeof(int32_t) * (size_t)(n_cells + 1) +
                            sizeof(int32_t) * (size_t)total);
     if (parts & GPK_INDEX_PIP) {
-        const int32_t rc = build_pip_index(a, ix, s, (parts & GPK_INDEX_PIP_LIGHT) ? 0 : ((parts & GPK_INDEX_PIP_FULL) ? 2 : 1));
+        const int32_t rc = build_pip_index(a, ix, s, (parts & GPK_INDEX_PIP_LIGHT) ? 0 : ((parts & GPK_INDEX_PIP_FULL) ? 2 : 1),
+                                           (parts & GPK_INDEX_PIP_EXACT_BUILD) ? 1 : ((parts & GPK_INDEX_PIP_SMALL_BUILD) ? 2 : 0));
         if (rc != GPK_OK) {
             gpk_index_free(ix);
             return rc;
diff --git a/geopolars_amd/csrc/gpk_index.h b/geopolars_amd/csrc/gpk_index.h
--- a/geopolars_amd/csrc/gpk_index.h
+++ b/geopolars_amd/csrc/gpk_index.h
@@ -93,10 +93,12 @@
     uint64_t serial;
     int32_t pip_list_heavy;
     int32_t route_own, route_single;
+    int32_t pip_build_path;
+    int64_t pip_counts[8];
 };
 
 namespace gpk {
-int32_t build_pip_index(const gpk_geoarray* a, gpk_index* ix, hipStream_t s, int list_records_mode = 1);
+int32_t build_pip_index(const gpk_geoarray* a, gpk_index* ix, hipStream_t s, int list_records_mode = 1, int path_mode = 0);
 int32_t ring_bboxes(const gpk_geoarray* a, double4* out_dev, hipStream_t s);
 int32_t affine_rows_impl(const gpk_geoarray* a, const double* matrices, int32_t mat_space, double* out_xy, int32_t out_space, hipStream_t s);
 }
diff --git a/geopolars_amd/csrc/gpk_pipindex.hip b/geopolars_amd/csrc/gpk_pipindex.hip
--- a/geopolars_amd/csrc/gpk_pipindex.hip
+++ b/geopolars_amd/csrc/gpk_pipindex.hip
@@ -17,6 +17,30 @@
     int R;
     double rx0, ry0, fw, fh, inv_fw, inv_fh, pad_x, pad_y;
 };
+struct SpecCtl {
+    const unsigned long long* n64;
+    const int32_t* n32;
+    int64_t cap;
+    uint32_t* stop;
+    const uint32_t* go;
+};
+__device__ __forceinline__ bool spec_enter(const SpecCtl& sc, int64_t& n) {
+    if (!sc.stop) return true;
+    if (*sc.stop) return false;
+    if (sc.go && !*sc.go) return false;
+    if (sc.n64 || sc.n32) {
+        const unsigned long long v = sc.n64 ? *sc.n64 : (unsigned long long)(uint32_t)*sc.n32;
+        if (v > (unsigned long long)sc.cap) {
+            *sc.stop = 1u;
+            return false;
+        }
+        n = (int64_t)v;
+    }
+    return true;
+}
+enum { SC_STOP = 0, SC_GO_CHAIN, SC_GO_REST, SC_N_FLAG2, SC_N_SLABS, SC_N_EDGES, SC_N_MARKS_RAW, SC_LIST_LEN, SC_N_SUB, SC_N_SUB2, SC_N_LREC, SC_N_REFINED,
+       SC_ROUTE_OWN, SC_ROUTE_SINGLE, SC_WORDS = 16 };
+
 __device__ __forceinline__ int fcol(const FineGrid& f, double x) { return dev::cell_of(x, f.rx0, f.inv_fw, f.R); }
 __device__ __forceinline__ int frow(const FineGrid& f, double y) { return dev::cell_of(y, f.ry0, f.inv_fh, f.R); }
 
@@ -118,9 +142,11 @@
 template <bool FILL>
 __global__ void slab_register_kernel(DevGeo a, const int32_t* __restrict__ coord_ring, FineGrid f, const int32_t* __restrict__ row0,
                                      const int32_t* __restrict__ slab_base, int32_t* __restrict__ cnt_or_cursor,
-                                     double4* __restrict__ edges, int32_t* __restrict__ vidx = nullptr) {
+                                     double4* __restrict__ edges, int32_t* __restrict__ vidx = nullptr, SpecCtl sc = SpecCtl{}) {
     const int64_t i = (int64_t)blockIdx.x * blockDim.x + threadIdx.x;
     const int lane = (int)(threadIdx.x & 63);
+    int64_t n_checked = 0;
+    if (!spec_enter(sc, n_checked)) return;
     int r = 0;
     double2 s = make_double2(0, 0), e = s;
     bool live = i < a.n_coords && edge_at(a, coord_ring, (int)i, r, s, e);
@@ -188,9 +214,11 @@
 
 template <bool FILL>
 __global__ void mark_kernel(DevGeo a, const int32_t* __restrict__ coord_ring, FineGrid g, const int32_t* __restrict__ ring_part,
-                            int32_t* __restrict__ cnt_or_off, unsigned long long* __restrict__ keys) {
+                            int32_t* __restrict__ cnt_or_off, unsigned long long* __restrict__ keys, SpecCtl sc = SpecCtl{}) {
     const int64_t i = (int64_t)blockIdx.x * blockDim.x + threadIdx.x;
     const int lane = (int)(threadIdx.x & 63);
+    int64_t n_checked = 0;
+    if (!spec_enter(sc, n_checked)) return;
     int r = 0;
     double2 s = make_double2(0, 0), e = s;
     const bool live = i < a.n_coords && edge_at(a, coord_ring, (int)i, r, s, e);
@@ -238,16 +266,57 @@
     }
 }
 
+constexpr int MARK_BUCKET_MAX = 64;
+__global__ void mark_hist_kernel(const unsigned long long* __restrict__ keys, int32_t* __restrict__ cell_cnt, SpecCtl sc) {
+    const int64_t i = (int64_t)blockIdx.x * blockDim.x + threadIdx.x;
+    int64_t n = 0;
+    if (!spec_enter(sc, n) || i >= n) return;
+    atomicAdd(&cell_cnt[keys[i] >> 32], 1);
+}
+__global__ void mark_scatter_kernel(const unsigned long long* __restrict__ keys, int32_t* __restrict__ cursor, unsigned long long* __restrict__ bucket,
+                                    SpecCtl sc) {
+    const int64_t i = (int64_t)blockIdx.x * blockDim.x + threadIdx.x;
+    int64_t n = 0;
+    if (!spec_enter(sc, n) || i >= n) return;
+    const unsigned long long key = keys[i];
+    bucket[atomicAdd(&cursor[key >> 32], 1)] = key;
+}
+__global__ void cell_marks_sort_kernel(unsigned long long* __restrict__ bucket, const int32_t* __restrict__ off, int64_t n_cells,
+                                       int32_t* __restrict__ uniq, SpecCtl sc) {
+    const int64_t c = (int64_t)blockIdx.x * blockDim.x + threadIdx.x;
+    int64_t n_checked = 0;
+    if (!spec_enter(sc, n_checked) || c >= n_cells) return;
+    const int lo = off[c], k = off[c + 1] - lo;
+    if (k > MARK_BUCKET_MAX) {
+        *sc.stop = 1u;
+        return;
+    }
+    unsigned long long* b = bucket + lo;
+    for (int i = 1; i < k; ++i) {
+        const unsigned long long v = b[i];
+        int j = i;
+        for (; j > 0 && b[j - 1] > v; --j) b[j] = b[j - 1];
+        b[j] = v;
+    }
+    int u = 0;
+    for (int i = 0; i < k; ++i)
+        if (i == 0 || b[i] != b[u - 1]) b[u++] = b[i];
+    uniq[c] = u;
+}
+
 constexpr int CELL_SCRATCH = 8;
 template <bool FILL>
 __global__ void cell_build_kernel(DevGeo a, IndexView ix, PipView pv, FineGrid g,
                                   const unsigned long long* __restrict__ marks, const int32_t* __restrict__ mark_start,
                                   int32_t* __restrict__ need, const int32_t* __restrict__ list_off,
                                   uint32_t* __restrict__ cell, uint32_t* __restrict__ list, uint32_t* __restrict__ scratch,
-                                  const double4* __restrict__ ring_bbox) {
+                                  const double4* __restrict__ ring_bbox, SpecCtl sc = SpecCtl{},
+                                  const int32_t* __restrict__ mark_uniq = nullptr) {
     const int64_t c = (int64_t)blockIdx.x * blockDim.x + threadIdx.x;
     const int64_t n_cells = (int64_t)g.R * g.R;
     if (c >= n_cells) return;
+    int64_t n_checked = 0;
+    if (!spec_enter(sc, n_checked)) return;
     if (FILL && need[c] == 0) return;
     if (FILL && scratch && need[c] - 1 <= CELL_SCRATCH) {
         const int m = need[c] - 1;
@@ -262,7 +331,7 @@
     const bool border = ci == 0 || cj == 0 || ci == g.R - 1 || cj == g.R - 1;
     const bool centre_ok = !border && fcol(g, cx) == ci && frow(g, cy) == cj;
     int64_t m = mark_start[c];
-    const int64_t m_end = mark_start[c + 1];
+    const int64_t m_end = mark_uniq ? m + mark_uniq[c] : (int64_t)mark_start[c + 1];
 
     int n = 0;
     uint32_t first_entry = 0;
@@ -327,9 +396,11 @@
 
 __device__ __forceinline__ int64_t sub_slot(int64_t c, int route_logR) { return route_logR ? (int64_t)route_order((uint32_t)c, route_logR) : c; }
 __global__ void sub_flag_kernel(const uint32_t* __restrict__ cell, const uint32_t* __restrict__ list, int64_t n_cells, int route_logR,
-                                int32_t* __restrict__ flag, int32_t* __restrict__ flag2) {
+                                int32_t* __restrict__ flag, int32_t* __restrict__ flag2, SpecCtl sc = SpecCtl{}, uint32_t* __restrict__ n_flag2 = nullptr) {
     const int64_t c = (int64_t)blockIdx.x * blockDim.x + threadIdx.x;
     if (c >= n_cells) return;
+    int64_t n_checked = 0;
+    if (!spec_enter(sc, n_checked)) return;
     const uint32_t w = cell[c];
     const uint32_t tag = w >> 30;
     flag[sub_slot(c, route_logR)] = (tag == CELL_TAG_SINGLE && (w & 1u)) ? 1 : 0;
@@ -338,7 +409,11 @@
         const uint32_t off = w & 0x3FFFFFFFu;
         if (list[off] == 2u) f2 = (list[off + 1] & list[off + 2] & 1u) ? 1 : 0;
     }
-    flag2[c] = f2;
+    if (flag2) flag2[c] = f2;
+    if (n_flag2) {
+        const unsigned long long m = __ballot(f2 != 0);
+        if (m && (int)(threadIdx.x & 63) == __ffsll((long long)m) - 1) atomicAdd(n_flag2, (uint32_t)__popcll(m));
+    }
 }
 
 __device__ __forceinline__ void record_slabs(const PipView& pv, int p, int cj, uint32_t& flags, uint32_t& e0, uint32_t& e1, uint32_t& e2) {
@@ -362,11 +437,13 @@
     }
 }
 __global__ void sub_head_kernel(PipView pv, FineGrid g, const int32_t* __restrict__ work_cell, const uint32_t* __restrict__ work_part,
-                                int64_t n_work, SubCell* __restrict__ sub) {
+                                int64_t n_work, SubCell* __restrict__ sub, SpecCtl sc = SpecCtl{}, uint32_t* __restrict__ rest_any = nullptr) {
     const int64_t i = (int64_t)blockIdx.x * blockDim.x + threadIdx.x;
+    if (!spec_enter(sc, n_work)) return;
     if (i >= n_work) return;
     uint32_t flags, e0, e1, e2;
     record_slabs(pv, (int)work_part[i], (int)(work_cell[i] / g.R), flags, e0, e1, e2);
+    if (rest_any && ((flags & (SUB_INDIRECT | 0x80000000u)) || e2 - e0 > 64u)) *rest_any = 1u;
     *reinterpret_cast<uint4*>(&sub[i].part_flags) = make_uint4(flags, e0, e1, e2);
 }
 
@@ -376,8 +453,10 @@
                                                         const int32_t* __restrict__ pos, int64_t n_cells, const uint32_t* __restrict__ cell,
                                                         const uint32_t* __restrict__ list, SubCell* __restrict__ sub,
                                                         SubCell2* __restrict__ sub2, const int32_t* __restrict__ work_cell = nullptr,
-                                                        const uint32_t* __restrict__ work_part = nullptr, int64_t n_work = 0) {
+                                                        const uint32_t* __restrict__ work_part = nullptr, int64_t n_work = 0,
+                                                        SpecCtl sc = SpecCtl{}) {
     static_assert(!WORK || NP == 1, "work items carry one part");
+    if (!spec_enter(sc, n_work)) return;
     constexpr int S = PIP_SUB, SS = PIP_SUB * PIP_SUB;
     const int64_t t = (int64_t)blockIdx.x * blockDim.x + threadIdx.x;
     const int64_t item = t / SS;
@@ -580,9 +659,12 @@
     store_labels(rec, label);
 }
 __global__ void sub_commit_kernel(const int32_t* __restrict__ flag, const int32_t* __restrict__ pos, const int32_t* __restrict__ flag2,
-                                  const int32_t* __restrict__ pos2, int64_t n_cells, int route_logR, uint32_t* __restrict__ cell) {
+                                  const int32_t* __restrict__ pos2, int64_t n_cells, int route_logR, uint32_t* __restrict__ cell,
+                                  SpecCtl sc = SpecCtl{}) {
     const int64_t c = (int64_t)blockIdx.x * blockDim.x + threadIdx.x;
     if (c >= n_cells) return;
+    int64_t n_checked = 0;
+    if (!spec_enter(sc, n_checked)) return;
     const int64_t o = sub_slot(c, route_logR);
     if (flag[o])
         cell[c] = (CELL_TAG_SUB << 30) | (uint32_t)pos[o];
@@ -591,9 +673,11 @@
 }
 
 __global__ void lrec_count_kernel(const uint32_t* __restrict__ cell, const uint32_t* __restrict__ list, int64_t n_cells,
-                                  int32_t* __restrict__ cnt) {
+                                  int32_t* __restrict__ cnt, SpecCtl sc = SpecCtl{}) {
     const int64_t c = (int64_t)blockIdx.x * blockDim.x + threadIdx.x;
     if (c >= n_cells) return;
+    int64_t n_checked = 0;
+    if (!spec_enter(sc, n_checked)) return;
     const uint32_t w = cell[c];
     int n = 0;
     if ((w >> 30) == CELL_TAG_LIST) {
@@ -623,12 +707,13 @@
 __global__ __launch_bounds__(256) void half_chain_kernel(DevGeo a, PipView pv, FineGrid g, const int32_t* __restrict__ work_cell,
                                                          const uint32_t* __restrict__ work_part, int64_t n_work,
                                                          const int32_t* __restrict__ slab_vidx, const SubCell* __restrict__ sub,
-                                                         uint32_t* __restrict__ hword) {
+                                                         uint32_t* __restrict__ hword, SpecCtl sc = SpecCtl{}) {
     constexpr int S = PIP_SUB;
     static_assert(S == 8 && PIP_SLAB_MUL == 2, "a record is two halves of four sub-cell rows, one base slab row each");
     const int64_t t = (int64_t)blockIdx.x * blockDim.x + threadIdx.x;
     const int64_t item = t >> 1;
     const int half = (int)(t & 1);
+    if (!spec_enter(sc, n_work)) return;
     if (item >= n_work) return;
     const int64_t c = work_cell[item];
     const int part = (int)work_part[item];
@@ -733,8 +818,9 @@
     }
     hword[2 * item + half] = word;
 }
-__global__ void half_chain_commit_kernel(SubCell* __restrict__ sub, int64_t n_sub, const uint32_t* __restrict__ hword) {
+__global__ void half_chain_commit_kernel(SubCell* __restrict__ sub, int64_t n_sub, const uint32_t* __restrict__ hword, SpecCtl sc = SpecCtl{}) {
     const int64_t i = (int64_t)blockIdx.x * blockDim.x + threadIdx.x;
+    if (!spec_enter(sc, n_sub)) return;
     if (i >= n_sub) return;
     const SubCell rc = sub[i];
     HalfCell* h = reinterpret_cast<HalfCell*>(sub + i);
@@ -788,18 +874,24 @@
 }
 
 __global__ void sub_work_kernel(const uint32_t* __restrict__ cell, const int32_t* __restrict__ flag, const int32_t* __restrict__ pos,
-                                int64_t n_cells, int route_logR, int32_t* __restrict__ work_cell, uint32_t* __restrict__ work_part) {
+                                int64_t n_cells, int route_logR, int32_t* __restrict__ work_cell, uint32_t* __restrict__ work_part,
+                                SpecCtl sc = SpecCtl{}) {
     const int64_t c = (int64_t)blockIdx.x * blockDim.x + threadIdx.x;
     if (c >= n_cells) return;
+    int64_t n_checked = 0;
+    if (!spec_enter(sc, n_checked)) return;
     const int64_t o = sub_slot(c, route_logR);
     if (!flag[o]) return;
     work_cell[pos[o]] = (int32_t)c;
     work_part[pos[o]] = (cell[c] & 0x3FFFFFFFu) >> 1;
 }
 __global__ void lrec_assign_kernel(const uint32_t* __restrict__ cell, uint32_t* __restrict__ list, int64_t n_cells,
-                                   const int32_t* __restrict__ pos, int32_t* __restrict__ work_cell, uint32_t* __restrict__ work_part) {
+                                   const int32_t* __restrict__ pos, int32_t* __restrict__ work_cell, uint32_t* __restrict__ work_part,
+                                   SpecCtl sc = SpecCtl{}) {
     const int64_t c = (int64_t)blockIdx.x * blockDim.x + threadIdx.x;
     if (c >= n_cells) return;
+    int64_t n_checked = 0;
+    if (!spec_enter(sc, n_checked)) return;
     const uint32_t w = cell[c];
     if ((w >> 30) != CELL_TAG_LIST) return;
     const uint32_t off = w & 0x3FFFFFFFu, m = list[off];
@@ -812,6 +904,33 @@
         list[off + 1 + t] = ((uint32_t)o << 1) | 1u;
         ++o;
     }
+}
+
+__global__ void small_decide_kernel(const int32_t* __restrict__ list_len, const int32_t* __restrict__ n_sub,
+                                    const int32_t* __restrict__ n_refined, uint32_t* __restrict__ ctl) {
+    if (blockIdx.x != 0 || threadIdx.x != 0 || ctl[SC_STOP]) return;
+    const int64_t ll = *list_len, ns = *n_sub, ns2 = ctl[SC_N_FLAG2];
+    if (ns2 > 0 && ns2 >= 4 * ns) {
+        ctl[SC_STOP] = 2u;
+        return;
+    }
+    ctl[SC_GO_CHAIN] = (ll * 8 <= ns && *n_refined == 0 && ns > 0) ? 1u : 0u;
+}
+__global__ void small_collect_kernel(const int32_t* __restrict__ n_slabs, const int32_t* __restrict__ n_edges, const int32_t* __restrict__ n_marks_raw,
+                                     const int32_t* __restrict__ list_len, const int32_t* __restrict__ n_sub,
+                                     const int32_t* __restrict__ n_lrec, const int32_t* __restrict__ n_refined,
+                                     const uint32_t* __restrict__ route_counts, uint32_t* __restrict__ ctl) {
+    if (blockIdx.x != 0 || threadIdx.x != 0 || ctl[SC_STOP]) return;
+    ctl[SC_N_SLABS] = (uint32_t)*n_slabs;
+    ctl[SC_N_EDGES] = (uint32_t)*n_edges;
+    ctl[SC_N_MARKS_RAW] = (uint32_t)*n_marks_raw;
+    ctl[SC_LIST_LEN] = (uint32_t)*list_len;
+    ctl[SC_N_SUB] = (uint32_t)*n_sub;
+    ctl[SC_N_SUB2] = ctl[SC_N_FLAG2];
+    ctl[SC_N_LREC] = n_lrec ? (uint32_t)*n_lrec : 0u;
+    ctl[SC_N_REFINED] = (uint32_t)*n_refined;
+    ctl[SC_ROUTE_OWN] = route_counts ? route_counts[0] : 0u;
+    ctl[SC_ROUTE_SINGLE] = route_counts ? route_counts[1] : 0u;
 }
 
 }
@@ -853,8 +972,9 @@
 
 namespace gpk {
 
-int32_t build_pip_index(const gpk_geoarray* a, gpk_index* ix, hipStream_t s, int list_records_mode) {
+static int32_t build_pip_index_impl(const gpk_geoarray* a, gpk_index* ix, hipStream_t s, int list_records_mode, const bool small, bool* took) {
     memset(&ix->pip, 0, sizeof ix->pip);
+    *took = true;
     const DevGeo& d = a->d;
     if (!is_polygonal(d.type) || d.n_geoms == 0 || d.n_coords == 0 || d.n_rings == 0) return GPK_OK;
     const GridParams hg = ix->host_grid;
@@ -884,12 +1004,34 @@
     if (!(g.pad_x > ulp64) || !(g.pad_y > ulp64)) return GPK_OK;
 
     const int64_t n_rings = d.n_rings, n_parts = d.n_parts, n_cells = (int64_t)R * R;
+    const bool level2_ok = g.pad_x / PIP_SUB > ulp64 && g.pad_y / PIP_SUB > ulp64 && R * PIP_SUB <= 32768;
+    int64_t cap_slabs = 0, cap_edges = 0, cap_marks = 0, cap_list = 0, cap_sub = 0;
+    if (small) {
+        if (!level2_ok) {
+            *took = false;
+            return GPK_OK;
+        }
+        cap_slabs = 4 * d.n_coords + (int64_t)PIP_SLAB_MUL * R + 2 * n_rings;
+        cap_edges = 4 * d.n_coords + 1024;
+        cap_marks = 12 * d.n_coords + 4096;
+        cap_list = 4 * d.n_coords + 1024;
+        cap_sub = n_cells < cap_marks ? n_cells : cap_marks;
+    }
     {
         size_t est = (size_t)n_rings * 64 + (size_t)n_cells * 96 + (size_t)d.n_coords * 168 + (8u << 20);
+        if (small) est += (size_t)cap_marks * 40 + (size_t)cap_slabs * 12 + (size_t)cap_edges * 4 + (size_t)(cap_sub + cap_list) * 8;
         if (est > (size_t(256) << 20)) est = size_t(256) << 20;
         ScratchEstimate::reserve(workspace_aux(1), est);
     }
     Temps t;
+    uint32_t* ctl = nullptr;
+    if (small) {
+        GPK_TRY(t.alloc(&ctl, (size_t)SC_WORDS));
+        GPK_HIP(hipMemsetAsync(ctl, 0, sizeof(uint32_t) * SC_WORDS, s));
+    }
+    auto ctl64 = [&](const unsigned long long* n, int64_t cap) { return small ? SpecCtl{n, nullptr, cap, ctl + SC_STOP, nullptr} : SpecCtl{}; };
+    auto ctl32 = [&](const int32_t* n, int64_t cap) { return small ? SpecCtl{nullptr, n, cap, ctl + SC_STOP, nullptr} : SpecCtl{}; };
+    auto ctl_stop = [&]() { return small ? SpecCtl{nullptr, nullptr, 0, ctl + SC_STOP, nullptr} : SpecCtl{}; };
     const bool dbg_time = getenv("GPK_DEBUG_INDEX") != nullptr;
     auto t_last = std::chrono::steady_clock::now();
     auto stamp = [&](const char* what) {
@@ -945,6 +1087,25 @@
     const int slab_off_slot = slot++;
     int32_t n_refined = 0, *n_refined_dev;
     GPK_TRY(t.alloc(&n_refined_dev, 64));
+    if (small) {
+        if (cap_slabs > max_scan) max_scan = cap_slabs;
+        if (cap_marks > max_scan) max_scan = cap_marks;
+        GPK_TRY(t.alloc(&btot, (size_t)((max_scan + 255) / 256 + 4)));
+        GPK_HIP(hipMemsetAsync(n_refined_dev, 0, sizeof(int32_t), s));
+        GPK_LAUNCH("gpk_pipidx_ring_rows", ring_rows_kernel, blocks_for(n_rings), dim3(256), 0, s, ring_bbox, n_rings, d.ring_off, gs, PIP_FINE_LOG2,
+                   row0, nrows, n_refined_dev);
+        GPK_TRY(exclusive_scan_i32(nrows, n_rings, slab_base, nullptr, btot, s));
+        GPK_TRY(t.alloc(&slab_cnt, (size_t)cap_slabs + 1));
+        GPK_TRY(t.alloc(&cursor, (size_t)cap_slabs + 1));
+        GPK_HIP(cached_malloc((void**)&slab_off, sizeof(int32_t) * (size_t)(cap_slabs + 1)));
+        ix->owned[slab_off_slot] = slab_off;
+        GPK_HIP(hipMemsetAsync(slab_cnt, 0, sizeof(int32_t) * (size_t)(cap_slabs + 1), s));
+        GPK_LAUNCH("gpk_pipidx_slab_count", slab_register_kernel<false>, blocks_for(d.n_coords), dim3(256), 0, s, d, coord_ring, gs, row0, slab_base,
+                   slab_cnt, (double4*)nullptr, (int32_t*)nullptr, ctl64(btot + (n_rings + 255) / 256, cap_slabs));
+        GPK_TRY(exclusive_scan_i32(slab_cnt, cap_slabs, slab_off, cursor, btot, s));
+        n_slabs = (int32_t)cap_slabs;
+        n_edges = (int32_t)cap_edges;
+    } else
     for (int max_shift = PIP_FINE_LOG2;; max_shift = 0) {
         GPK_HIP(hipMemsetAsync(n_refined_dev, 0, sizeof(int32_t), s));
         GPK_LAUNCH("gpk_pipidx_ring_rows", ring_rows_kernel, blocks_for(n_rings), dim3(256), 0, s, ring_bbox, n_rings, d.ring_off, gs, max_shift,
@@ -988,7 +1149,7 @@
         keep(slab_vidx);
     }
     GPK_LAUNCH("gpk_pipidx_slab_fill", slab_register_kernel<true>, blocks_for(d.n_coords), dim3(256), 0, s, d, coord_ring, gs, row0, slab_base,
-               cursor, edges, slab_vidx);
+               cursor, edges, slab_vidx, ctl64(btot + (cap_slabs + 255) / 256, cap_edges));
 
     stamp("slab fill (+ edges malloc)");
     PartInfo* part_info = nullptr;
@@ -1022,18 +1183,41 @@
                (unsigned long long*)nullptr);
     GPK_TRY(exclusive_scan_i32(mark_cnt, d.n_coords, mark_off, nullptr, btot, s));
     unsigned long long n_marks_raw = 0;
-    GPK_HIP(d2h_small(&n_marks_raw, btot + (d.n_coords + 255) / 256, sizeof n_marks_raw, s));
-    GPK_HIP(sync_small(s));
+    if (small) {
+        n_marks_raw = (unsigned long long)cap_marks;
+    } else {
+        GPK_HIP(d2h_small(&n_marks_raw, btot + (d.n_coords + 255) / 256, sizeof n_marks_raw, s));
+        GPK_HIP(sync_small(s));
+    }
     if (n_marks_raw >= (1ull << 31))
         return GPK_OK;
     stamp("mark count + scan");
-    unsigned long long *keys, *sorted, *marks;
+    unsigned long long *keys, *sorted = nullptr, *marks;
     GPK_TRY(t.alloc(&keys, (size_t)n_marks_raw));
-    GPK_TRY(t.alloc(&sorted, (size_t)n_marks_raw));
+    if (!small) GPK_TRY(t.alloc(&sorted, (size_t)n_marks_raw));
     marks = keys;
-    int64_t n_marks = 0;
     int32_t* mark_start;
+    int32_t* mark_uniq = nullptr;
     GPK_TRY(t.alloc(&mark_start, (size_t)n_cells + 2));
+    if (small) {
+        const SpecCtl raw = ctl32(mark_off + d.n_coords, cap_marks);
+        int32_t *raw_cnt, *raw_cur;
+        unsigned long long* bucket;
+        GPK_TRY(t.alloc(&raw_cnt, (size_t)n_cells + 2));
+        GPK_TRY(t.alloc(&raw_cur, (size_t)n_cells + 2));
+        GPK_TRY(t.alloc(&mark_uniq, (size_t)n_cells + 2));
+        GPK_TRY(t.alloc(&bucket, (size_t)cap_marks));
+        GPK_HIP(hipMemsetAsync(raw_cnt, 0, sizeof(int32_t) * (size_t)(n_cells + 2), s));
+        GPK_LAUNCH("gpk_pipidx_mark_fill", mark_kernel<true>, blocks_for(d.n_coords), dim3(256), 0, s, d, coord_ring, g, ring_part, mark_off, keys,
+                   ctl64(btot + (d.n_coords + 255) / 256, cap_marks));
+        GPK_LAUNCH("gpk_pipidx_mark_hist", mark_hist_kernel, blocks_for(cap_marks), dim3(256), 0, s, (const unsigned long long*)keys, raw_cnt, raw);
+        GPK_TRY(exclusive_scan_i32(raw_cnt, n_cells, mark_start, raw_cur, btot, s));
+        GPK_LAUNCH("gpk_pipidx_mark_scatter", mark_scatter_kernel, blocks_for(cap_marks), dim3(256), 0, s, (const unsigned long long*)keys, raw_cur,
+                   bucket, raw);
+        GPK_LAUNCH("gpk_pipidx_mark_cellsort", cell_marks_sort_kernel, blocks_for(n_cells), dim3(256), 0, s, bucket, (const int32_t*)mark_start, n_cells,
+                   mark_uniq, ctl_stop());
+        marks = bucket;
+    } else {
     GPK_HIP(hipMemsetAsync(mark_start, 0, sizeof(int32_t) * (size_t)(n_cells + 2), s));
     if (n_marks_raw > 0) {
         GPK_LAUNCH("gpk_pipidx_mark_fill", mark_kernel<true>, blocks_for(d.n_coords), dim3(256), 0, s, d, coord_ring, g, ring_part, mark_off, keys);
@@ -1059,7 +1243,7 @@
         int32_t nu = 0;
         GPK_HIP(d2h_small(&nu, pos + n_marks_raw, sizeof nu, s));
         GPK_HIP(sync_small(s));
-        n_marks = nu;
+    }
     }
 
     stamp("mark fill + sort + unique");
@@ -1072,18 +1256,23 @@
     uint32_t* cell_scratch = nullptr;
     GPK_TRY(t.alloc(&cell_scratch, (size_t)n_cells * CELL_SCRATCH));
     GPK_LAUNCH("gpk_pipidx_cell_count", cell_build_kernel<false>, blocks_for(n_cells), dim3(256), 0, s, d, ix->v, pv, g, marks, mark_start,
-               need, (const int32_t*)nullptr, cell, (uint32_t*)nullptr, cell_scratch, (const double4*)ring_bbox);
+               need, (const int32_t*)nullptr, cell, (uint32_t*)nullptr, cell_scratch, (const double4*)ring_bbox, ctl_stop(), (const int32_t*)mark_uniq);
     GPK_TRY(exclusive_scan_i32(need, n_cells, list_off, nullptr, btot, s));
     int32_t list_len = 0;
-    GPK_HIP(d2h_small(&list_len, list_off + n_cells, sizeof list_len, s));
-    GPK_HIP(sync_small(s));
+    if (small) {
+        list_len = (int32_t)cap_list;
+    } else {
+        GPK_HIP(d2h_small(&list_len, list_off + n_cells, sizeof list_len, s));
+        GPK_HIP(sync_small(s));
+    }
     if ((unsigned)list_len >= (1u << 30)) return GPK_OK;
     uint32_t* list = nullptr;
     GPK_HIP(cached_malloc((void**)&list, sizeof(uint32_t) * (size_t)(list_len ? list_len : 1)));
     keep(list);
     GPK_LAUNCH("gpk_pipidx_cell_fill", cell_build_kernel<true>, blocks_for(n_cells), dim3(256), 0, s, d, ix->v, pv, g, marks, mark_start,
-               need, list_off, cell, list, cell_scratch, (const double4*)ring_bbox);
-    GPK_HIP(hipStreamSynchronize(s));
+               need, list_off, cell, list, cell_scratch, (const double4*)ring_bbox, ctl64(btot + (n_cells + 255) / 256, cap_list),
+               (const int32_t*)mark_uniq);
+    if (!small) GPK_HIP(hipStreamSynchronize(s));
     pv.cell = cell;
     pv.list = list;
     ix->pip_list_heavy = (int64_t)list_len * 4 > n_cells ? 1 : 0;
@@ -1099,8 +1288,39 @@
     int route_logR = 0;
     if (R <= PIP_ROUTE_RMAX)
         while ((1 << route_logR) < R) ++route_logR;
-    const bool level2_ok = g.pad_x / PIP_SUB > ulp64 && g.pad_y / PIP_SUB > ulp64 && R * PIP_SUB <= 32768;
-    if (level2_ok) {
+    int32_t *list_len_dev = list_off + n_cells, *n_sub_dev = nullptr;
+    if (small) {
+        int32_t *sflag, *spos;
+        GPK_TRY(t.alloc(&sflag, (size_t)n_cells + 1));
+        GPK_TRY(t.alloc(&spos, (size_t)n_cells + 1));
+        n_sub_dev = spos + n_cells;
+        GPK_LAUNCH("gpk_pipidx_sub_flag", sub_flag_kernel, blocks_for(n_cells), dim3(256), 0, s, cell, (const uint32_t*)list, n_cells, route_logR, sflag,
+                   (int32_t*)nullptr, ctl_stop(), ctl + SC_N_FLAG2);
+        GPK_TRY(exclusive_scan_i32(sflag, n_cells, spos, nullptr, btot, s));
+        GPK_LAUNCH("gpk_pipidx_small_decide", small_decide_kernel, dim3(1), dim3(64), 0, s, (const int32_t*)list_len_dev, (const int32_t*)n_sub_dev,
+                   (const int32_t*)n_refined_dev, ctl);
+        n_sub = (int32_t)cap_sub;
+        const SpecCtl recs = ctl32(n_sub_dev, cap_sub);
+        SpecCtl rest = recs;
+        rest.go = ctl + SC_GO_REST;
+        GPK_HIP(cached_malloc((void**)&sub, sizeof(SubCell) * (size_t)cap_sub));
+        keep(sub);
+        GPK_HIP(hipMemsetAsync(sub, 0, sizeof(SubCell) * (size_t)cap_sub, s));
+        GPK_TRY(t.alloc(&swork_cell, (size_t)cap_sub));
+        GPK_TRY(t.alloc(&swork_part, (size_t)cap_sub));
+        GPK_LAUNCH("gpk_pipidx_sub_work", sub_work_kernel, blocks_for(n_cells), dim3(256), 0, s, (const uint32_t*)cell, (const int32_t*)sflag,
+                   (const int32_t*)spos, n_cells, route_logR, swork_cell, swork_part, recs);
+        GPK_LAUNCH("gpk_pipidx_sub_head", sub_head_kernel, blocks_for(cap_sub), dim3(256), 0, s, pv, g, (const int32_t*)swork_cell,
+                   (const uint32_t*)swork_part, (int64_t)0, sub, recs, ctl + SC_GO_REST);
+        GPK_LAUNCH("gpk_pipidx_sub_build_fast", (sub_build_kernel<1, true, 1>), blocks_for(cap_sub * PIP_SUB * PIP_SUB), dim3(256), 0, s, d, pv, g,
+                   (const int32_t*)nullptr, (const int32_t*)nullptr, n_cells, (const uint32_t*)cell, (const uint32_t*)list, sub, (SubCell2*)nullptr,
+                   (const int32_t*)swork_cell, (const uint32_t*)swork_part, (int64_t)0, recs);
+        GPK_LAUNCH("gpk_pipidx_sub_build_rest", (sub_build_kernel<1, true, 2>), blocks_for(cap_sub * PIP_SUB * PIP_SUB), dim3(256), 0, s, d, pv, g,
+                   (const int32_t*)nullptr, (const int32_t*)nullptr, n_cells, (const uint32_t*)cell, (const uint32_t*)list, sub, (SubCell2*)nullptr,
+                   (const int32_t*)swork_cell, (const uint32_t*)swork_part, (int64_t)0, rest);
+        GPK_LAUNCH("gpk_pipidx_sub_commit", sub_commit_kernel, blocks_for(n_cells), dim3(256), 0, s, sflag, spos, (const int32_t*)nullptr,
+                   (const int32_t*)nullptr, n_cells, route_logR, cell, ctl_stop());
+    } else if (level2_ok) {
         int32_t *sflag, *spos, *sflag2, *spos2;
         GPK_TRY(t.alloc(&sflag, (size_t)n_cells + 1));
         GPK_TRY(t.alloc(&spos, (size_t)n_cells + 1));
@@ -1158,6 +1378,127 @@
     stamp("level-2 records");
     pv.sub = sub;
     pv.sub2 = sub2;
+    if (small) {
+        auto drop = [&](auto*& p) {
+            for (int i = 4; i < 24; ++i)
+                if (p && ix->owned[i] == (void*)p) ix->owned[i] = nullptr;
+            if (p) cached_free((void*)p);
+            p = nullptr;
+        };
+        int32_t* n_lrec_dev = nullptr;
+        SubCell* lrec = nullptr;
+        if (list_records) {
+            int32_t *lcnt, *lpos, *work_cell;
+            uint32_t* work_part;
+            GPK_TRY(t.alloc(&lcnt, (size_t)n_cells + 1));
+            GPK_TRY(t.alloc(&lpos, (size_t)n_cells + 1));
+            GPK_TRY(t.alloc(&work_cell, (size_t)cap_list));
+            GPK_TRY(t.alloc(&work_part, (size_t)cap_list));
+            n_lrec_dev = lpos + n_cells;
+            GPK_LAUNCH("gpk_pipidx_lrec_count", lrec_count_kernel, blocks_for(n_cells), dim3(256), 0, s, (const uint32_t*)cell, (const uint32_t*)list, n_cells,
+                       lcnt, ctl_stop());
+            GPK_TRY(exclusive_scan_i32(lcnt, n_cells, lpos, nullptr, btot, s));
+            const SpecCtl recs = ctl32(n_lrec_dev, cap_list);
+            SpecCtl rest = recs;
+            rest.go = ctl + SC_GO_REST;
+            GPK_HIP(cached_malloc((void**)&lrec, sizeof(SubCell) * (size_t)cap_list));
+            keep(lrec);
+            GPK_HIP(hipMemsetAsync(lrec, 0, sizeof(SubCell) * (size_t)cap_list, s));
+            GPK_LAUNCH("gpk_pipidx_lrec_assign", lrec_assign_kernel, blocks_for(n_cells), dim3(256), 0, s, (const uint32_t*)cell, list, n_cells,
+                       (const int32_t*)lpos, work_cell, work_part, recs);
+            GPK_LAUNCH("gpk_pipidx_lrec_head", sub_head_kernel, blocks_for(cap_list), dim3(256), 0, s, pv, g, (const int32_t*)work_cell,
+                       (const uint32_t*)work_part, (int64_t)0, lrec, recs, ctl + SC_GO_REST);
+            GPK_LAUNCH("gpk_pipidx_lrec_build", (sub_build_kernel<1, true, 1>), blocks_for(cap_list * PIP_SUB * PIP_SUB), dim3(256), 0, s, d, pv, g,
+                       (const int32_t*)nullptr, (const int32_t*)nullptr, n_cells, (const uint32_t*)cell, (const uint32_t*)list, lrec, (SubCell2*)nullptr,
+                       (const int32_t*)work_cell, (const uint32_t*)work_part, (int64_t)0, recs);
+            GPK_LAUNCH("gpk_pipidx_lrec_build", (sub_build_kernel<1, true, 2>), blocks_for(cap_list * PIP_SUB * PIP_SUB), dim3(256), 0, s, d, pv, g,
+                       (const int32_t*)nullptr, (const int32_t*)nullptr, n_cells, (const uint32_t*)cell, (const uint32_t*)list, lrec, (SubCell2*)nullptr,
+                       (const int32_t*)work_cell, (const uint32_t*)work_part, (int64_t)0, rest);
+        }
+        float4* part_box = nullptr;
+        GPK_HIP(cached_malloc((void**)&part_box, sizeof(float4) * (size_t)(n_parts ? n_parts : 1)));
+        keep(part_box);
+        GPK_LAUNCH("gpk_pipidx_part_box", part_box_kernel, blocks_for(n_parts), dim3(256), 0, s, d, n_parts, (const double4*)ring_bbox, part_box);
+        const int64_t n_ext = d.n_coords + d.n_rings * CHAIN_MAX;
+        const bool chains_fit = slab_vidx && n_ext < ((int64_t)1 << (32 - HCHAIN_START_SHIFT));
+        double2* cxy = nullptr;
+        RouteWord* route = nullptr;
+        uint32_t* route_counts = nullptr;
+        if (chains_fit) {
+            SpecCtl chain = ctl32(n_sub_dev, cap_sub);
+            chain.go = ctl + SC_GO_CHAIN;
+            GPK_HIP(cached_malloc((void**)&cxy, sizeof(double2) * (size_t)n_ext));
+            keep(cxy);
+            uint32_t* hword;
+            GPK_TRY(t.alloc(&hword, (size_t)cap_sub * 2 + 2));
+            GPK_LAUNCH("gpk_pipidx_chain_xy", chain_xy_kernel, blocks_for(n_ext), dim3(256), 0, s, d, cxy);
+            GPK_LAUNCH("gpk_pipidx_half_chain", half_chain_kernel, blocks_for(cap_sub * 2), dim3(256), 0, s, d, pv, g, (const int32_t*)swork_cell,
+                       (const uint32_t*)swork_part, (int64_t)0, (const int32_t*)slab_vidx, (const SubCell*)sub, hword, chain);
+            GPK_LAUNCH("gpk_pipidx_chain_commit", half_chain_commit_kernel, blocks_for(cap_sub), dim3(256), 0, s, sub, (int64_t)0, (const uint32_t*)hword, chain);
+            if (R <= PIP_ROUTE_RMAX) {
+                const int64_t n_words = n_cells / 32;
+                GPK_HIP(cached_malloc((void**)&route, sizeof(RouteWord) * (size_t)n_words));
+                keep(route);
+                GPK_TRY(t.alloc(&route_counts, 2));
+                GPK_HIP(hipMemsetAsync(route_counts, 0, 2 * sizeof(uint32_t), s));
+                GPK_LAUNCH("gpk_pipidx_route", route_build_kernel, blocks_for(n_words), dim3(256), 0, s, (const uint32_t*)cell, n_words, route_logR, route,
+                           route_counts);
+            }
+        }
+        GPK_LAUNCH("gpk_pipidx_small_collect", small_collect_kernel, dim3(1), dim3(64), 0, s, (const int32_t*)(slab_base + n_rings),
+                   (const int32_t*)(slab_off + cap_slabs), (const int32_t*)(mark_off + d.n_coords), (const int32_t*)list_len_dev, (const int32_t*)n_sub_dev,
+                   (const int32_t*)n_lrec_dev, (const int32_t*)n_refined_dev, (const uint32_t*)route_counts, ctl);
+        uint32_t hc[SC_WORDS];
+        GPK_HIP(d2h_small(hc, ctl, sizeof hc, s));
+        GPK_HIP(sync_small(s));
+        if (getenv("GPK_DEBUG_INDEX"))
+            fprintf(stderr, "[gpk] small build: stop %u; slabs %u / %lld, slab entries %u / %lld, raw marks %u / %lld, list %u / %lld, records %u / %lld\n", hc[SC_STOP],
+                    hc[SC_N_SLABS], (long long)cap_slabs, hc[SC_N_EDGES], (long long)cap_edges, hc[SC_N_MARKS_RAW], (long long)cap_marks, hc[SC_LIST_LEN],
+                    (long long)cap_list, hc[SC_N_SUB], (long long)cap_sub);
+        if (hc[SC_STOP]) {
+            *took = false;
+            return GPK_OK;
+        }
+        n_slabs = (int32_t)hc[SC_N_SLABS];
+        n_edges = (int32_t)hc[SC_N_EDGES];
+        list_len = (int32_t)hc[SC_LIST_LEN];
+        n_sub = (int32_t)hc[SC_N_SUB];
+        n_refined = (int32_t)hc[SC_N_REFINED];
+        const int32_t n_lrec = (int32_t)hc[SC_N_LREC];
+        if (n_sub == 0) drop(sub);
+        if (n_lrec == 0) drop(lrec);
+        pv.sub = sub;
+        pv.lrec = lrec;
+        ix->pip_list_heavy = (int64_t)list_len * 4 > n_cells ? 1 : 0;
+        if (list_len > 0 && !lrec) {
+            pv.part_box = part_box;
+            ix->nbytes += (int64_t)(sizeof(float4) * (size_t)n_parts);
+        } else {
+            drop(part_box);
+        }
+        ix->pip_lean = (int64_t)list_len * 8 <= (int64_t)n_sub && n_refined == 0 ? 1 : 0;
+        if (ix->pip_lean && n_sub > 0 && chains_fit) {
+            pv.chain_xy = cxy;
+            ix->nbytes += (int64_t)(sizeof(double2) * (size_t)n_ext);
+            if (route) {
+                pv.route = route;
+                ix->nbytes += (int64_t)(sizeof(RouteWord) * (size_t)(n_cells / 32));
+                ix->route_own = (int32_t)hc[SC_ROUTE_OWN];
+                ix->route_single = (int32_t)hc[SC_ROUTE_SINGLE];
+            }
+        } else {
+            drop(cxy);
+            drop(route);
+        }
+        ix->nbytes += (int64_t)(sizeof(SubCell) * (size_t)n_sub + sizeof(SubCell) * (size_t)n_lrec);
+        ix->pip = pv;
+        ix->nbytes += (int64_t)(sizeof(uint32_t) * (size_t)n_cells + sizeof(uint32_t) * (size_t)list_len + (pv.slab_edges ? sizeof(double4) : sizeof(int32_t)) * (size_t)n_edges +
+                                sizeof(int32_t) * (size_t)(n_slabs + 1) + sizeof(int32_t) * (size_t)(2 * n_rings + 1) +
+                                (part_geom ? sizeof(uint32_t) * (size_t)n_parts : 0) + sizeof(PartInfo) * (size_t)n_parts);
+        const int64_t counts[8] = {n_slabs, n_edges, list_len, n_sub, 0, n_lrec, pv.chain_xy ? n_ext : 0, n_parts};
+        memcpy(ix->pip_counts, counts, sizeof counts);
+        return GPK_OK;
+    }
     int32_t n_lrec = 0;
     SubCell* lrec = nullptr;
     if (level2_ok && list_len > 0 && list_records) {
@@ -1252,7 +1593,37 @@
     ix->nbytes += (int64_t)(sizeof(uint32_t) * (size_t)n_cells + sizeof(uint32_t) * (size_t)list_len + (pv.slab_edges ? sizeof(double4) : sizeof(int32_t)) * (size_t)n_edges +
                             sizeof(int32_t) * (size_t)(n_slabs + 1) + sizeof(int32_t) * (size_t)(2 * n_rings + 1) +
                             (part_geom ? sizeof(uint32_t) * (size_t)n_parts : 0) + sizeof(PartInfo) * (size_t)n_parts);
+    const int64_t counts[8] = {n_slabs, n_edges, list_len, n_sub, n_sub2, n_lrec, pv.chain_xy ? d.n_coords + d.n_rings * CHAIN_MAX : 0, n_parts};
+    memcpy(ix->pip_counts, counts, sizeof counts);
     return GPK_OK;
 }
 
-}
+constexpr int64_t PIP_SMALL_MAX_COORDS = 65536;
+constexpr int64_t PIP_SMALL_FORCE_MAX_COORDS = int64_t(1) << 22;
+
+int32_t build_pip_index(const gpk_geoarray* a, gpk_index* ix, hipStream_t s, int list_records_mode, int path_mode) {
+    ix->pip_build_path = 0;
+    memset(ix->pip_counts, 0, sizeof ix->pip_counts);
+    const int64_t n = a->d.n_coords;
+    if (path_mode != 1 && (n <= PIP_SMALL_MAX_COORDS || (path_mode == 2 && n <= PIP_SMALL_FORCE_MAX_COORDS))) {
+        const int64_t nbytes0 = ix->nbytes;
+        bool took = false;
+        const int32_t rc = build_pip_index_impl(a, ix, s, list_records_mode, true, &took);
+        if (rc != GPK_OK) return rc;
+        if (took) {
+            ix->pip_build_path = 1;
+            return GPK_OK;
+        }
+        for (int i = 4; i < 24; ++i) {
+            if (ix->owned[i]) cached_free(ix->owned[i]);
+            ix->owned[i] = nullptr;
+        }
+        ix->nbytes = nbytes0;
+        ix->pip_lean = ix->pip_list_heavy = ix->route_own = ix->route_single = 0;
+        ix->pip_build_path = 2;
+    }
+    bool took = true;
+    return build_pip_index_impl(a, ix, s, list_records_mode, false, &took);
+}
+
+}
diff --git a/geopolars_amd/spatial_index.py b/geopolars_amd/spatial_index.py
--- a/geopolars_amd/spatial_index.py
+++ b/geopolars_amd/spatial_index.py
@@ -30,10 +30,12 @@
     return t.data_ptr() if t is not None else None
 
 
-def _index_parts(for_points: bool, full: bool, light: bool) -> int:
+def _index_parts(for_points: bool, full: bool, light: bool, build: str | None = None) -> int:
     parts = _abi.INDEX_BBOX_GRID | (_abi.INDEX_PIP if for_points else 0) | (_abi.INDEX_PIP_FULL if for_points and full else 0)
     if for_points and light and not full:
         parts |= _abi.INDEX_PIP_LIGHT
+    if for_points and build is not None:
+        parts |= {"exact": _abi.INDEX_PIP_EXACT_BUILD, "small": _abi.INDEX_PIP_SMALL_BUILD}[build]
     return parts
 
 
@@ -47,12 +49,13 @@
         self._h = h
 
     @staticmethod
-    def from_device(dev: DeviceGeoArray, stream: int = 0, for_points: bool = True, bboxes=None, full: bool = False, light: bool = False) -> "SpatialIndex":
+    def from_device(dev: DeviceGeoArray, stream: int = 0, for_points: bool = True, bboxes=None, full: bool = False, light: bool = False,
+                    build: str | None = None) -> "SpatialIndex":
         self = SpatialIndex.__new__(SpatialIndex)
         self.series = None
         self._dev = dev
         h = C.c_void_p()
-        parts = _index_parts(for_points, full, light)
+        parts = _index_parts(for_points, full, light, build)
         _abi.check(_abi.lib().gpk_index_build_ex(dev.handle, parts, _ptr(bboxes), stream, C.byref(h)))
         self._h = h
         return self
@@ -70,6 +73,21 @@
         out = (C.c_int64 * 8)()
         _abi.check(_abi.lib().gpk_index_describe(self._h, out))
         return {"R": int(out[0]), "lean": bool(out[1]), "chains": bool(out[2]), "route": bool(out[3]), "list_heavy": bool(out[4])}
+
+    def build_path(self) -> str:
+        out = (C.c_int64 * 8)()
+        _abi.check(_abi.lib().gpk_index_describe(self._h, out))
+        return ("exact", "small", "fallback")[int(out[7])]
+
+    def table(self, name: str, stream: int = 0) -> np.ndarray:
+        import torch
+
+        lib, which, n = _abi.lib(), _abi.INDEX_TABLES[name], C.c_int64(0)
+        _abi.check(lib.gpk_index_debug_table(self._h, which, None, 0, C.byref(n), stream))
+        buf = torch.empty(max(int(n.value), 1), dtype=torch.uint8, device="cuda")
+        _abi.check(lib.gpk_index_debug_table(self._h, which, buf.data_ptr(), int(n.value), C.byref(n), stream))
+        torch.cuda.synchronize()
+        return buf[: int(n.value)].cpu().numpy()
 
     def query_envelopes(self, boxes, mode: str = "contained", stream: int = 0) -> tuple[np.ndarray, np.ndarray]:
         lib = _abi.lib()
diff --git a/include/geopolars_hip.h b/include/geopolars_hip.h
--- a/include/geopolars_hip.h
+++ b/include/geopolars_hip.h
@@ -183,6 +183,8 @@
 #define GPK_INDEX_PIP       2
 #define GPK_INDEX_PIP_LIGHT 4
 #define GPK_INDEX_PIP_FULL  8
+#define GPK_INDEX_PIP_EXACT_BUILD 16
+#define GPK_INDEX_PIP_SMALL_BUILD 32
 int32_t gpk_index_build_ex(const gpk_geoarray* a, int32_t parts, const double* bbox4_dev, void* stream,
                            gpk_index** out);
 int32_t gpk_index_free(gpk_index* idx);
@@ -193,6 +195,21 @@
                                  int32_t space, void* stream);
 int32_t gpk_index_nbytes(const gpk_index* idx, int64_t* out_bytes);
 int32_t gpk_index_describe(const gpk_index* idx, int64_t out[8]);
+#define GPK_INDEX_TABLE_CELL       0
+#define GPK_INDEX_TABLE_LIST       1
+#define GPK_INDEX_TABLE_SUB        2
+#define GPK_INDEX_TABLE_SUB2       3
+#define GPK_INDEX_TABLE_LREC       4
+#define GPK_INDEX_TABLE_CHAIN_XY   5
+#define GPK_INDEX_TABLE_ROUTE      6
+#define GPK_INDEX_TABLE_PART_INFO  7
+#define GPK_INDEX_TABLE_PART_BOX   8
+#define GPK_INDEX_TABLE_SLAB_OFF   9
+#define GPK_INDEX_TABLE_SLAB_EDGES 10
+#define GPK_INDEX_TABLE_RING_ROW0  11
+#define GPK_INDEX_TABLE_RING_SLAB  12
+#define GPK_INDEX_TABLE_PART_GEOM  13
+int32_t gpk_index_debug_table(const gpk_index* idx, int32_t which, void* dst_dev, int64_t capacity, int64_t* nbytes, void* stream);
 
 int32_t gpk_spatial_join(const gpk_geoarray* left, const gpk_geoarray* right,
                          const gpk_index* right_index, int32_t predicate, uint32_t left_row_base,
```

Result: no change. 126900 billion (-0.7%).
